# PTD504/handwritten-math-ocr-api

Hardware: NVIDIA B200
Metric: images_per_sec (higher is better)
Workload: dtype fp16

## Files before the change

handwritten_math_ocr_api_b200/_lib.py:

```python
from __future__ import annotations

import ctypes as C
import os

HERE = os.path.dirname(os.path.abspath(__file__))
LIB_PATH = os.path.join(HERE, "libhmocr.so")


class HmocrConfig(C.Structure):
    _fields_ = [(n, C.c_int32) for n in ("vocab_size", "d_model", "nhead", "dim_feedforward", "num_layers",
                                         "max_seq_len", "sos_id", "eos_id", "pad_id", "encoder_arch",
                                         "enc_num_layers")]


_p, _i, _i64p, _fp = C.c_void_p, C.c_int, C.POINTER(C.c_int64), C.c_void_p

SIGNATURES = {
    "hmocr_last_error": (C.c_char_p, []),
    "hmocr_version": (C.c_char_p, []),
    "hmocr_launch_count": (C.c_int64, []),
    "hmocr_create": (_i, [C.POINTER(HmocrConfig), C.POINTER(_p)]),
    "hmocr_destroy": (None, [_p]),
    "hmocr_load_weight": (_i, [_p, C.c_char_p, _p, _i64p, _i, _i]),
    "hmocr_finalize_weights": (_i, [_p]),
    "hmocr_set_option": (_i, [_p, C.c_char_p, _i]),
    "hmocr_decode_max_clusters": (_i, [C.POINTER(C.c_int)]),
    "hmocr_set_pos_table": (_i, [_p, _p, _i, _i, _p]),
    "hmocr_workspace_bytes": (_i, [_p, _i, _i, _i, C.POINTER(C.c_size_t)]),
    "hmocr_set_workspace": (_i, [_p, _p, C.c_size_t, _p]),
    "hmocr_read_trace": (_i, [_p, _i64p, _i]),
    "hmocr_encode": (_i, [_p, _p, _i, _p, _p]),
    "hmocr_decoder_forward": (_i, [_p, _p, _p, _i, _i, _p, _p]),
    "hmocr_generate": (_i, [_p, _p, _i, _i, _i, _p, _p, _p, _p, _p]),
    "hmocr_generate_from_memory": (_i, [_p, _p, _i, _i, _i, _p, _p, _p, _p, _p]),
    "hmocr_generate_nbest": (_i, [_p, _p, _i, _i, _i, _i, _i, _p, _p, _p, _p, _p]),
    "hmocr_generate_host": (_i, [_p, _p, _i, _i, _i, _p, _p, _p, _p, _p]),
    "hmocr_preprocess_u8": (_i, [_p, _p, _i, _p, _p]),
    "hmocr_pack_tokens": (_i, [_p, _p, _i, _i, _p, _p, _p]),
    "hmocr_preprocess_image_u8": (_i, [_p, _p, _i, _i, _i, _p, _p]),
    "hmocr_preprocess_cv2_u8": (_i, [_p, _p, _i, _i, _p, _p]),
    "hmocr_generate_host_u8": (_i, [_p, _p, _i, _i, _i, _p, _p, _p, _p, _p]),
    "hmocr_last_decode_steps": (_i, [_p, C.POINTER(C.c_int32)]),
    "hmocr_last_timings": (_i, [_p, C.POINTER(C.c_float), C.POINTER(C.c_float)]),
    "hmocr_gemm_f16": (_i, [_p, _i, _i, _i, _p, _i, _p, _i, _p, _i, _p, _i, _p, _i, _p, _p, _i, _p]),
    "hmocr_swin_mlp": (_i, [_p, _i, _i, _p, _p, _p, _p, _p, _p]),
    "hmocr_layernorm": (_i, [_p, _i, _i, _p, _p, _p, _p, _p]),
    "hmocr_patch_embed": (_i, [_p, _i, _p, _p, _p, _p, _p, _p]),
    "hmocr_patch_merge_ln": (_i, [_p, _i, _i, _i, _i, _p, _p, _p, _p]),
    "hmocr_window_attention": (_i, [_p, _p, _p, _i, _i, _i, _i, _i, _i, _p, _p]),
    "hmocr_self_attention": (_i, [_p, _i, _i, _i, _i, _p, _p]),
}

_lib = None


def load() -> C.CDLL:
    global _lib
    if _lib is None:
        if not os.path.exists(LIB_PATH):
            raise RuntimeError(
                f"{LIB_PATH} is missing: build it with `python -m handwritten_math_ocr_api_b200.build` "
                "(there is no CPU or PyTorch fallback)")
        lib = C.CDLL(LIB_PATH)
        for name, (res, args) in SIGNATURES.items():
            fn = getattr(lib, name)
            fn.restype, fn.argtypes = res, args
        _lib = lib
    return _lib


def check(rc: int, what: str) -> None:
    if rc != 0:
        msg = load().hmocr_last_error()
        raise RuntimeError(f"{what} failed ({rc}): {msg.decode() if msg else 'unknown error'}")
```

handwritten_math_ocr_api_b200/csrc/engine.cu:

```cuda
#include <stdarg.h>
#include <string.h>

#include <map>
#include <string>
#include <vector>

#include "decode_persistent.cuh"
#include "gemm.cuh"
#include "hmocr.h"
#include "kernels.cuh"

#include <nvtx3/nvToolsExt.h>

#define HM_API extern "C" __attribute__((visibility("default")))

namespace hmocr {

thread_local long g_launch_count = 0;
static thread_local char g_err[1024] = "";

void set_error(const char* fmt, ...) {
  va_list ap;
  va_start(ap, fmt);
  vsnprintf(g_err, sizeof(g_err), fmt, ap);
  va_end(ap);
}

namespace {

inline void nvtx_push(const char* name) { nvtxRangePushA(name); }
inline void nvtx_pop() { nvtxRangePop(); }

constexpr int IMG_H = 96, IMG_W = 320, SWIN_OUT = 768;
constexpr int RES18_MEM = 10, SWIN_MEM = 30;
constexpr int RES18_C[4] = {64, 128, 256, 512};
constexpr int RES18_STRIDE[4] = {1, 2, 2, 2};
constexpr int DEPTHS[4] = {2, 2, 6, 2};
constexpr int HEADS[4] = {3, 6, 12, 24};
constexpr int STEP_CHUNK = 8;

struct HostTensor {
  std::vector<float> f;
  std::vector<int64_t> i;
  std::vector<int64_t> shape;
};

struct Lin {
  h16* w = nullptr;
  float* b = nullptr;
  int n = 0, k = 0;
};
struct Norm { float* g = nullptr; float* b = nullptr; };
struct SwinBlock { Norm n1, n2; Lin qkv, proj, fc1, fc2; float* rel_bias = nullptr; };
struct Merge { Norm norm; Lin red; };
struct DecLayer { Lin sa_in, sa_out, ca_q, ca_out, l1, l2; Norm n1, n2, n3; };
struct EncLayer { Lin in_proj, out_proj, l1, l2; Norm n1, n2; };
struct ResBlock { Lin conv1, conv2, down; bool has_down = false; };

struct Buf {
  void* p = nullptr;
  size_t cap = 0;
};

}
}

using namespace hmocr;

struct hmocr_engine {
  hmocr_config cfg;
  int device = 0;
  int vpad = 0;
  std::map<std::string, HostTensor> host;
  bool finalized = false;

  uint8_t* arena = nullptr;
  size_t arena_cap = 0, arena_used = 0;
  float *pe_w = nullptr, *pe_b = nullptr;
  Norm pe_norm;
  SwinBlock blocks[12];
  Merge merges[3];
  Lin proj;
  float *emb = nullptr, *pos = nullptr;
  std::vector<DecLayer> layers;
  int mem_len = SWIN_MEM;
  float *r18_w1 = nullptr, *r18_b1 = nullptr;
  ResBlock r18_blocks[8];
  Lin r18_proj;
  std::vector<EncLayer> enc_layers;
  float* pos_table = nullptr;
  bool pos_table_set = false;
  Lin ca_kv;
  Lin fc;
  uint8_t* dp_wstream = nullptr;
  float* dp_lnparams = nullptr;
  int dp_fc_tiles = 0, dp_chunks_per_step = 0;
  int decode_impl = 0;
  int steps_per_launch = 0;
  int trace_step = -1;
  int conv_impl = 0;
  int mlp_fused = 1;

  std::map<std::string, Buf> ws;
  uint64_t ws_epoch = 0;
  uint8_t* ext_ws = nullptr;
  size_t ext_cap = 0, ext_used = 0;
  cudaStream_t cur_stream = nullptr;
  bool planning = false;
  std::map<std::string, size_t> plan;
  std::map<std::string, size_t> planned;

  struct StepGraph { cudaGraphExec_t exec = nullptr; uint64_t epoch = 0; };
  std::map<long long, StepGraph> graphs;
  struct EncGraph { cudaGraphExec_t exec = nullptr; uint64_t epoch = 0; bool warm = false; long launches = 0; };
  std::map<int, EncGraph> enc_graphs;
  int encoder_graph = 1;
  cudaStream_t cap_stream = nullptr;
  cudaEvent_t ev[4] = {nullptr, nullptr, nullptr, nullptr};
  cudaEvent_t poll_ev[2] = {nullptr, nullptr};
  DecodeState* pinned_state = nullptr;
  int last_poll_slot = -1;
  float last_enc_ms = 0.f, last_dec_ms = 0.f;
  bool timings_pending = false;
};

namespace hmocr {
namespace {

constexpr size_t WS_ALIGN = 256;
inline size_t ws_round(size_t b) { return (b + WS_ALIGN - 1) / WS_ALIGN * WS_ALIGN; }
inline bool ws_pool_exempt(const char* name) { return name[0] == 'p' && name[1] == 'p' && name[2] == '.'; }

template <class T>
int ws_get(hmocr_engine* e, const char* name, size_t count, T** out) {
  const size_t bytes = ws_round(count * sizeof(T) + 1);
  if (e->planning) {
    size_t& need = e->plan[name];
    if (need < bytes) need = bytes;
    *out = reinterpret_cast<T*>(WS_ALIGN);
    return 0;
  }
  Buf& b = e->ws[name];
  if (b.cap < bytes) {
    if (e->ext_ws != nullptr && !ws_pool_exempt(name)) {
      const size_t off = ws_round(e->ext_used);
      auto pl = e->planned.find(name);
      const size_t bytes_now = bytes;
      const size_t bytes = (pl != e->planned.end() && pl->second > bytes_now) ? pl->second : bytes_now;
      HM_CHECK(off + bytes <= e->ext_cap,
               "caller-owned workspace too small for '%s' (%zu + %zu > %zu bytes): size it with hmocr_workspace_bytes for "
               "the largest (batch, max_len, beam) you call with", name, off, bytes, e->ext_cap);
      b.p = e->ext_ws + off;
      b.cap = bytes;
      e->ext_used = off + bytes;
    } else {
      if (b.p != nullptr) {
        HM_CUDA(cudaFreeAsync(b.p, e->cur_stream));
        b.p = nullptr;
        b.cap = 0;
      }
      const size_t want = ws_round(bytes + bytes / 8);
      HM_CUDA(cudaMallocAsync(&b.p, want, e->cur_stream));
      b.cap = want;
    }
    ++e->ws_epoch;
  }
  *out = reinterpret_cast<T*>(b.p);
  return 0;
}

int arena_alloc(hmocr_engine* e, size_t bytes, void** out) {
  const size_t off = (e->arena_used + 255) & ~size_t(255);
  HM_CHECK(off + bytes <= e->arena_cap, "weight arena overflow (%zu + %zu > %zu)", off, bytes, e->arena_cap);
  *out = e->arena + off;
  e->arena_used = off + bytes;
  return 0;
}

const HostTensor* find(hmocr_engine* e, const std::string& key) {
  auto it = e->host.find(key);
  return it == e->host.end() ? nullptr : &it->second;
}

int need(hmocr_engine* e, const std::string& key, std::vector<int64_t> shape, const HostTensor** out) {
  const HostTensor* t = find(e, key);
  HM_CHECK(t != nullptr, "missing state-dict entry '%s'", key.c_str());
  HM_CHECK(t->shape == shape, "state-dict entry '%s' has the wrong shape", key.c_str());
  HM_CHECK(!t->f.empty(), "state-dict entry '%s' must be float32", key.c_str());
  *out = t;
  return 0;
}

inline h16 host_to_h16(float v) { return __float2half(v > 65504.f ? 65504.f : (v < -65504.f ? -65504.f : v)); }

int upload_f32(hmocr_engine* e, const float* src, size_t n, float** out) {
  void* p;
  HM_TRY(arena_alloc(e, n * sizeof(float), &p));
  HM_CUDA(cudaMemcpy(p, src, n * sizeof(float), cudaMemcpyHostToDevice));
  *out = reinterpret_cast<float*>(p);
  return 0;
}

int upload_vec(hmocr_engine* e, const std::string& key, int64_t n, float** out) {
  const HostTensor* t;
  HM_TRY(need(e, key, {n}, &t));
  return upload_f32(e, t->f.data(), (size_t)n, out);
}

int upload_norm(hmocr_engine* e, const std::string& prefix, int64_t n, Norm* out) {
  HM_TRY(upload_vec(e, prefix + ".weight", n, &out->g));
  return upload_vec(e, prefix + ".bias", n, &out->b);
}

int upload_lin_rows(hmocr_engine* e, const float* w, const float* b, int rows, int k, Lin* out) {
  const int npad = (rows + 31) / 32 * 32;
  std::vector<h16> tmp((size_t)npad * k, host_to_h16(0.f));
  for (size_t i = 0; i < (size_t)rows * k; ++i) tmp[i] = host_to_h16(w[i]);
  void* p;
  HM_TRY(arena_alloc(e, tmp.size() * 2, &p));
  HM_CUDA(cudaMemcpy(p, tmp.data(), tmp.size() * 2, cudaMemcpyHostToDevice));
  out->w = reinterpret_cast<h16*>(p);
  out->n = npad;
  out->k = k;
  out->b = nullptr;
  if (b != nullptr) {
    std::vector<float> bt(npad, 0.f);
    memcpy(bt.data(), b, sizeof(float) * rows);
    HM_TRY(upload_f32(e, bt.data(), npad, &out->b));
  }
  return 0;
}

int upload_lin(hmocr_engine* e, const std::string& prefix, int n, int k, bool bias, Lin* out) {
  const HostTensor *w, *b = nullptr;
  HM_TRY(need(e, prefix + ".weight", {n, k}, &w));
  if (bias) HM_TRY(need(e, prefix + ".bias", {n}, &b));
  return upload_lin_rows(e, w->f.data(), b ? b->f.data() : nullptr, n, k, out);
}

int fold_bn(hmocr_engine* e, const std::string& bn, int cout, std::vector<float>* scale, std::vector<float>* shift) {
  const HostTensor *g, *b, *m, *v;
  HM_TRY(need(e, bn + ".weight", {cout}, &g));
  HM_TRY(need(e, bn + ".bias", {cout}, &b));
  HM_TRY(need(e, bn + ".running_mean", {cout}, &m));
  HM_TRY(need(e, bn + ".running_var", {cout}, &v));
  scale->resize(cout); shift->resize(cout);
  for (int i = 0; i < cout; ++i) {
    const float sc = g->f[i] / sqrtf(v->f[i] + 1e-5f);
    (*scale)[i] = sc;
    (*shift)[i] = b->f[i] - m->f[i] * sc;
  }
  return 0;
}

int upload_conv(hmocr_engine* e, const std::string& conv, const std::string& bn, int cout, int cin, int k, Lin* out) {
  const HostTensor* w;
  HM_TRY(need(e, conv + ".weight", {cout, cin, k, k}, &w));
  std::vector<float> scale, shift;
  HM_TRY(fold_bn(e, bn, cout, &scale, &shift));
  std::vector<float> m((size_t)cout * k * k * cin);
  for (int o = 0; o < cout; ++o)
    for (int ci = 0; ci < cin; ++ci)
      for (int ky = 0; ky < k; ++ky)
        for (int kx = 0; kx < k; ++kx)
          m[(size_t)o * k * k * cin + (size_t)(ky * k + kx) * cin + ci] =
              w->f[(((size_t)o * cin + ci) * k + ky) * k + kx] * scale[o];
  return upload_lin_rows(e, m.data(), shift.data(), cout, k * k * cin, out);
}

int load_res18_weights(hmocr_engine* e) {
  const hmocr_config& c = e->cfg;
  const int d = c.d_model, ff = c.dim_feedforward;
  const std::string f = "encoder.features.";
  {
    const HostTensor* w;
    HM_TRY(need(e, f + "0.weight", {64, 1, 7, 7}, &w));
    std::vector<float> scale, shift;
    HM_TRY(fold_bn(e, f + "1", 64, &scale, &shift));
    std::vector<float> w1(64 * 49);
    for (int o = 0; o < 64; ++o)
      for (int i = 0; i < 49; ++i) w1[o * 49 + i] = w->f[o * 49 + i] * scale[o];
    HM_TRY(upload_f32(e, w1.data(), w1.size(), &e->r18_w1));
    HM_TRY(upload_f32(e, shift.data(), shift.size(), &e->r18_b1));
  }
  int cin = 64;
  for (int sidx = 0; sidx < 4; ++sidx) {
    const int cout = RES18_C[sidx];
    for (int j = 0; j < 2; ++j) {
      const std::string p = f + std::to_string(4 + sidx) + "." + std::to_string(j) + ".";
      ResBlock& rb = e->r18_blocks[sidx * 2 + j];
      HM_TRY(upload_conv(e, p + "conv1", p + "bn1", cout, j == 0 ? cin : cout, 3, &rb.conv1));
      HM_TRY(upload_conv(e, p + "conv2", p + "bn2", cout, cout, 3, &rb.conv2));
      rb.has_down = find(e, p + "downsample.0.weight") != nullptr;
      if (rb.has_down) HM_TRY(upload_conv(e, p + "downsample.0", p + "downsample.1", cout, cin, 1, &rb.down));
    }
    cin = cout;
  }
  HM_TRY(upload_lin(e, "encoder.projection", d, 512, true, &e->r18_proj));
  const int enc_layers = c.enc_num_layers > 0 ? c.enc_num_layers : c.num_layers;
  HM_CHECK(find(e, "encoder.transformer_encoder.layers." + std::to_string(enc_layers) + ".linear1.weight") == nullptr,
           "checkpoint has more than %d TransformerEncoder layers: set hmocr_config.enc_num_layers "
           "(config.res18trans_num_encoder_layers)", enc_layers);
  e->enc_layers.resize(enc_layers);
  for (int l = 0; l < enc_layers; ++l) {
    const std::string p = "encoder.transformer_encoder.layers." + std::to_string(l) + ".";
    EncLayer& L = e->enc_layers[l];
    const HostTensor *w, *b;
    HM_TRY(need(e, p + "self_attn.in_proj_weight", {3 * d, d}, &w));
    HM_TRY(need(e, p + "self_attn.in_proj_bias", {3 * d}, &b));
    HM_TRY(upload_lin_rows(e, w->f.data(), b->f.data(), 3 * d, d, &L.in_proj));
    HM_TRY(upload_lin(e, p + "self_attn.out_proj", d, d, true, &L.out_proj));
    HM_TRY(upload_lin(e, p + "linear1", ff, d, true, &L.l1));
    HM_TRY(upload_lin(e, p + "linear2", d, ff, true, &L.l2));
    HM_TRY(upload_norm(e, p + "norm1", d, &L.n1));
    HM_TRY(upload_norm(e, p + "norm2", d, &L.n2));
  }
  void* pt;
  HM_TRY(arena_alloc(e, sizeof(float) * RES18_MEM * d, &pt));
  e->pos_table = static_cast<float*>(pt);
  return 0;
}

int run_lin(cudaStream_t st, const h16* a, int lda, int M, const Lin& l, GemmEpilogue epi) {
  epi.bias = l.b;
  return gemm_f16(st, a, lda, M, l.k, l.w, l.n, epi);
}

int encode_impl(hmocr_engine* e, const float* images, int B, float* enc32, h16* enc16, cudaStream_t st) {
  const size_t tok1 = (size_t)B * 24 * 80;
  float *xa, *xb;
  h16 *xn, *qkv, *ctx, *hid;
  HM_TRY(ws_get(e, "enc.xa", tok1 * 96, &xa));
  HM_TRY(ws_get(e, "enc.xb", tok1 * 96 / 2, &xb));
  HM_TRY(ws_get(e, "enc.xn", tok1 * 96, &xn));
  HM_TRY(ws_get(e, "enc.qkv", tok1 * 288, &qkv));
  HM_TRY(ws_get(e, "enc.ctx", tok1 * 96, &ctx));
  HM_TRY(ws_get(e, "enc.hid", tok1 * 384, &hid));
  if (e->planning) return 0;

  HM_TRY(patch_embed(st, images, B, e->pe_w, e->pe_b, e->pe_norm.g, e->pe_norm.b, xa));
  int H = 24, W = 80, C = 96, blk = 0;
  float* x = xa;
  float* other = xb;
  for (int s = 0; s < 4; ++s) {
    const int rows = B * H * W;
    for (int j = 0; j < DEPTHS[s]; ++j, ++blk) {
      const SwinBlock& sb = e->blocks[blk];
      HM_TRY(layernorm(st, x, rows, C, sb.n1.g, sb.n1.b, xn, nullptr));
      GemmEpilogue eq;
      eq.out_f16 = qkv; eq.ld16 = 3 * C;
      HM_TRY(run_lin(st, xn, C, rows, sb.qkv, eq));
      HM_TRY(window_attention(st, qkv, sb.qkv.b, sb.rel_bias, B, H, W, C, HEADS[s], (j & 1) ? 3 : 0, ctx));
      GemmEpilogue ep;
      ep.residual = x; ep.ldr = C; ep.out_f32 = x; ep.ld32 = C;
      HM_TRY(run_lin(st, ctx, C, rows, sb.proj, ep));
      HM_TRY(layernorm(st, x, rows, C, sb.n2.g, sb.n2.b, xn, nullptr));
      if (e->mlp_fused && swin_mlp_supported(C)) {
        HM_TRY(swin_mlp(st, xn, rows, C, sb.fc1.w, sb.fc1.b, sb.fc2.w, sb.fc2.b, x));
      } else {
        GemmEpilogue e1;
        e1.act = 1; e1.out_f16 = hid; e1.ld16 = 4 * C;
        HM_TRY(run_lin(st, xn, C, rows, sb.fc1, e1));
        GemmEpilogue e2;
        e2.residual = x; e2.ldr = C; e2.out_f32 = x; e2.ld32 = C;
        HM_TRY(run_lin(st, hid, 4 * C, rows, sb.fc2, e2));
      }
    }
    if (s < 3) {
      const Merge& m = e->merges[s];
      HM_TRY(patch_merge_ln(st, x, B, H, W, C, m.norm.g, m.norm.b, xn));
      GemmEpilogue em;
      em.out_f32 = other; em.ld32 = 2 * C;
      HM_TRY(run_lin(st, xn, 4 * C, rows / 4, m.red, em));
      float* t = x; x = other; other = t;
      H /= 2; W /= 2; C *= 2;
    }
  }
  const int rows = B * e->mem_len;
  HM_TRY(f32_to_f16(st, x, (size_t)rows * SWIN_OUT, xn));
  GemmEpilogue eo;
  eo.out_f32 = enc32; eo.ld32 = e->cfg.d_model;
  eo.out_f16 = enc16; eo.ld16 = e->cfg.d_model;
  HM_TRY(run_lin(st, xn, SWIN_OUT, rows, e->proj, eo));
  return 0;
}

int conv_gemm(hmocr_engine* e, cudaStream_t st, const h16* x16, int B, int H, int W, int C, int k, int stride,
              const Lin& w, h16* col, GemmEpilogue epi) {
  const int pad = (k == 3) ? 1 : 0;
  const int Ho = (H + 2 * pad - k) / stride + 1, Wo = (W + 2 * pad - k) / stride + 1;
  int tw, th, tn;
  if (e->conv_impl == 0 && C % 64 == 0 && w.n % 64 == 0 && conv_tiling(Ho, Wo, &tw, &th, &tn)) {
    epi.bias = w.b;
    return gemm_conv_f16(st, x16, B, H, W, C, k, stride, pad, w.w, w.n, epi);
  }
  HM_TRY(im2col(st, x16, B, H, W, C, k, stride, pad, col));
  return run_lin(st, col, k * k * C, B * Ho * Wo, w, epi);
}

int encode_res18_impl(hmocr_engine* e, const float* images, int B, float* enc32, h16* enc16, cudaStream_t st) {
  const int d = e->cfg.d_model, ff = e->cfg.dim_feedforward, nh = e->cfg.nhead;
  HM_CHECK(e->planning || e->pos_table_set, "ResNet-18 variant: call hmocr_set_pos_table first - the reference draws a fresh "
                             "nn.Embedding(10, d_model) table on every encoder call (src/model_res18trans.py:57-59)");
  HM_CHECK(B <= 256, "ResNet-18 variant: the encoder attends ACROSS the batch (SURVEY.md D7); batch %d > 256 unsupported", B);
  const size_t m1 = (size_t)B * 24 * 80;
  h16 *stem, *xa16, *xb16, *h16b, *col;
  float *xa32, *xb32, *ds32;
  HM_TRY(ws_get(e, "r18.stem", (size_t)B * 48 * 160 * 64, &stem));
  HM_TRY(ws_get(e, "r18.xa16", m1 * 64, &xa16));
  HM_TRY(ws_get(e, "r18.xb16", m1 * 64, &xb16));
  HM_TRY(ws_get(e, "r18.h16", m1 * 64, &h16b));
  HM_TRY(ws_get(e, "r18.xa32", m1 * 64, &xa32));
  HM_TRY(ws_get(e, "r18.xb32", m1 * 64, &xb32));
  HM_TRY(ws_get(e, "r18.ds32", m1 * 64 / 2, &ds32));
  HM_TRY(ws_get(e, "r18.col", m1 * 576, &col));
  const int S = RES18_MEM, rows = B * S;
  h16 *pool16, *z16, *qkv, *ctx, *hid;
  float *q32, *z32;
  HM_TRY(ws_get(e, "r18.pool16", (size_t)rows * 512, &pool16));
  HM_TRY(ws_get(e, "r18.q32", (size_t)rows * d, &q32));
  HM_TRY(ws_get(e, "r18.z32", (size_t)rows * d, &z32));
  HM_TRY(ws_get(e, "r18.z16", (size_t)rows * d, &z16));
  HM_TRY(ws_get(e, "r18.qkv", (size_t)rows * 3 * d, &qkv));
  HM_TRY(ws_get(e, "r18.ctx", (size_t)rows * d, &ctx));
  HM_TRY(ws_get(e, "r18.hid", (size_t)rows * ff, &hid));
  if (e->planning) return 0;
  HM_TRY(conv7x7_bn_relu(st, images, B, e->r18_w1, e->r18_b1, stem));
  HM_TRY(maxpool3x3s2(st, stem, B, 48, 160, 64, xa16, xa32));
  int H = 24, W = 80, C = 64;
  h16 *x16 = xa16, *y16 = xb16;
  float *x32 = xa32, *y32 = xb32;
  for (int sidx = 0; sidx < 4; ++sidx) {
    for (int j = 0; j < 2; ++j) {
      const ResBlock& rb = e->r18_blocks[sidx * 2 + j];
      const int cout = RES18_C[sidx], stride = (j == 0) ? RES18_STRIDE[sidx] : 1;
      const int Ho = H / stride, Wo = W / stride, M = B * Ho * Wo;
      GemmEpilogue e1;
      e1.act = 2; e1.out_f16 = h16b; e1.ld16 = cout;
      HM_TRY(conv_gemm(e, st, x16, B, H, W, C, 3, stride, rb.conv1, col, e1));
      const float* identity = x32;
      if (rb.has_down) {
        GemmEpilogue ed;
        ed.out_f32 = ds32; ed.ld32 = cout;
        HM_TRY(conv_gemm(e, st, x16, B, H, W, C, 1, stride, rb.down, col, ed));
        identity = ds32;
      }
      GemmEpilogue e2;
      e2.act = 3; e2.residual = identity; e2.ldr = cout; e2.out_f32 = y32; e2.ld32 = cout; e2.out_f16 = y16; e2.ld16 = cout;
      HM_TRY(conv_gemm(e, st, h16b, B, Ho, Wo, cout, 3, 1, rb.conv2, col, e2));
      (void)M;
      h16* t16 = x16; x16 = y16; y16 = t16;
      float* t32 = x32; x32 = y32; y32 = t32;
      H = Ho; W = Wo; C = cout;
    }
  }
  HM_TRY(avgpool_h(st, x32, B, H, W, C, pool16));
  GemmEpilogue ep;
  ep.out_f32 = q32; ep.ld32 = d;
  HM_TRY(run_lin(st, pool16, 512, rows, e->r18_proj, ep));
  HM_TRY(add_pos_permute(st, q32, e->pos_table, B, S, d, z32, z16));
  for (size_t l = 0; l < e->enc_layers.size(); ++l) {
    const EncLayer& L = e->enc_layers[l];
    GemmEpilogue ei;
    ei.out_f16 = qkv; ei.ld16 = 3 * d;
    HM_TRY(run_lin(st, z16, d, rows, L.in_proj, ei));
    HM_TRY(mha_prefill_self(st, qkv, S, B, nh, ctx, false));
    GemmEpilogue e1;
    e1.residual = z32; e1.ldr = d; e1.out_f32 = z32; e1.ld32 = d; e1.out_f16 = z16; e1.ld16 = d;
    e1.ln_gamma = L.n1.g; e1.ln_beta = L.n1.b;
    HM_TRY(run_lin(st, ctx, d, rows, L.out_proj, e1));
    GemmEpilogue ef;
    ef.act = 2; ef.out_f16 = hid; ef.ld16 = ff;
    HM_TRY(run_lin(st, z16, d, rows, L.l1, ef));
    GemmEpilogue e2;
    e2.residual = z32; e2.ldr = d; e2.out_f32 = z32; e2.ld32 = d; e2.out_f16 = z16; e2.ld16 = d;
    e2.ln_gamma = L.n2.g; e2.ln_beta = L.n2.b;
    HM_TRY(run_lin(st, hid, ff, rows, L.l2, e2));
  }
  return permute_back(st, z32, B, S, d, enc32, enc16);
}

int project_memory(hmocr_engine* e, const h16* enc16, int B, h16* memkv, cudaStream_t st) {
  GemmEpilogue ek;
  ek.out_f16 = memkv; ek.ld16 = e->ca_kv.n;
  return run_lin(st, enc16, e->cfg.d_model, B * e->mem_len, e->ca_kv, ek);
}

struct DecBufs {
  float* x32;
  h16 *x16, *qkv, *q, *ctx, *hid;
  float* logits;
};

int dec_bufs(hmocr_engine* e, const char* tag, size_t rows, DecBufs* b) {
  const int d = e->cfg.d_model, ff = e->cfg.dim_feedforward;
  std::string t(tag);
  HM_TRY(ws_get(e, (t + ".x32").c_str(), rows * d, &b->x32));
  HM_TRY(ws_get(e, (t + ".x16").c_str(), rows * d, &b->x16));
  HM_TRY(ws_get(e, (t + ".qkv").c_str(), rows * 3 * d, &b->qkv));
  HM_TRY(ws_get(e, (t + ".q").c_str(), rows * d, &b->q));
  HM_TRY(ws_get(e, (t + ".ctx").c_str(), rows * d, &b->ctx));
  HM_TRY(ws_get(e, (t + ".hid").c_str(), rows * ff, &b->hid));
  HM_TRY(ws_get(e, (t + ".logits").c_str(), rows * e->vpad, &b->logits));
  return 0;
}

int layer_tail(hmocr_engine* e, const DecLayer& L, int l, const DecBufs& b, int rows, const h16* memkv,
               const int* mem_row, int T, cudaStream_t st) {
  const int d = e->cfg.d_model, ff = e->cfg.dim_feedforward, nh = e->cfg.nhead;
  GemmEpilogue e1;
  e1.residual = b.x32; e1.ldr = d; e1.out_f32 = b.x32; e1.ld32 = d; e1.out_f16 = b.x16; e1.ld16 = d;
  e1.ln_gamma = L.n1.g; e1.ln_beta = L.n1.b;
  HM_TRY(run_lin(st, b.ctx, d, rows, L.sa_out, e1));
  GemmEpilogue eq;
  eq.out_f16 = b.q; eq.ld16 = d;
  HM_TRY(run_lin(st, b.x16, d, rows, L.ca_q, eq));
  if (T > 0)
    HM_TRY(mha_prefill_cross(st, b.q, memkv, e->ca_kv.n, l * 2 * d, l * 2 * d + d, rows / T, T, e->mem_len, nh, b.ctx));
  else
    HM_TRY(cross_attn_step(st, b.q, memkv, e->ca_kv.n, l * 2 * d, l * 2 * d + d, mem_row, rows, e->mem_len, nh, b.ctx));
  GemmEpilogue e2;
  e2.residual = b.x32; e2.ldr = d; e2.out_f32 = b.x32; e2.ld32 = d; e2.out_f16 = b.x16; e2.ld16 = d;
  e2.ln_gamma = L.n2.g; e2.ln_beta = L.n2.b;
  HM_TRY(run_lin(st, b.ctx, d, rows, L.ca_out, e2));
  GemmEpilogue ef;
  ef.act = 2; ef.out_f16 = b.hid; ef.ld16 = ff;
  HM_TRY(run_lin(st, b.x16, d, rows, L.l1, ef));
  GemmEpilogue e3;
  e3.residual = b.x32; e3.ldr = d; e3.out_f32 = b.x32; e3.ld32 = d; e3.out_f16 = b.x16; e3.ld16 = d;
  e3.ln_gamma = L.n3.g; e3.ln_beta = L.n3.b;
  HM_TRY(run_lin(st, b.hid, ff, rows, L.l2, e3));
  return 0;
}

int decoder_forward_impl(hmocr_engine* e, const float* enc32, const int64_t* tgt, int B, int T, float* logits,
                         cudaStream_t st) {
  const int d = e->cfg.d_model, nh = e->cfg.nhead;
  const int rows = B * T;
  h16 *enc16, *memkv;
  HM_TRY(ws_get(e, "tf.enc16", (size_t)B * e->mem_len * d, &enc16));
  HM_TRY(ws_get(e, "tf.memkv", (size_t)B * e->mem_len * e->ca_kv.n, &memkv));
  DecBufs b;
  HM_TRY(dec_bufs(e, "tf", rows, &b));
  if (e->planning) return 0;
  HM_TRY(f32_to_f16(st, enc32, (size_t)B * e->mem_len * d, enc16));
  HM_TRY(project_memory(e, enc16, B, memkv, st));
  HM_TRY(embed_tokens(st, tgt, T, B, T, e->emb, e->pos, d, e->cfg.vocab_size, b.x32, b.x16));
  for (int l = 0; l < e->cfg.num_layers; ++l) {
    const DecLayer& L = e->layers[l];
    GemmEpilogue ei;
    ei.out_f16 = b.qkv; ei.ld16 = 3 * d;
    HM_TRY(run_lin(st, b.x16, d, rows, L.sa_in, ei));
    HM_TRY(mha_prefill_self(st, b.qkv, B, T, nh, b.ctx));
    HM_TRY(layer_tail(e, L, l, b, rows, memkv, nullptr, T, st));
  }
  GemmEpilogue eo;
  eo.out_f32 = b.logits; eo.ld32 = e->vpad;
  HM_TRY(run_lin(st, b.x16, d, rows, e->fc, eo));
  HM_TRY(copy_logits(st, b.logits, e->vpad, rows, e->cfg.vocab_size, logits));
  return 0;
}

struct GenBufs {
  DecBufs b;
  h16 *kcache, *vcache;
  DecodeState* state;
  uint8_t* finished;
  int tmax;
};

int enqueue_step(hmocr_engine* e, const GenBufs& g, int rows, const h16* memkv, int64_t* tokens,
                 float* logprob, int max_len, cudaStream_t st) {
  const int d = e->cfg.d_model, nh = e->cfg.nhead;
  const size_t layer_stride = (size_t)rows * nh * g.tmax * 32;
  for (int l = 0; l < e->cfg.num_layers; ++l) {
    const DecLayer& L = e->layers[l];
    GemmEpilogue ei;
    ei.out_f16 = g.b.qkv; ei.ld16 = 3 * d;
    HM_TRY(run_lin(st, g.b.x16, d, rows, L.sa_in, ei));
    HM_TRY(self_attn_step(st, g.state, g.b.qkv, g.kcache + l * layer_stride, g.vcache + l * layer_stride, rows, nh,
                          g.tmax, g.b.ctx));
    HM_TRY(layer_tail(e, L, l, g.b, rows, memkv, nullptr, 0, st));
  }
  GemmEpilogue eo;
  eo.out_f32 = g.b.logits; eo.ld32 = e->vpad;
  HM_TRY(run_lin(st, g.b.x16, d, rows, e->fc, eo));
  HM_TRY(greedy_select(st, g.state, g.b.logits, e->vpad, e->cfg.vocab_size, rows, tokens, max_len + 1, logprob,
                       max_len, e->cfg.eos_id, g.finished, e->emb, e->pos, d, e->cfg.max_seq_len, g.b.x32, g.b.x16));
  HM_TRY(advance_step(st, g.state));
  return 0;
}

int generate_persistent(hmocr_engine* e, const h16* enc16, int B, int max_len, int beam, int64_t* tokens,
                        float* logprob, int32_t* steps, float* score, cudaStream_t st, int n_best);

int generate_from_memory_impl(hmocr_engine* e, const h16* enc16, int B, int max_len, int beam,
                              int64_t* tokens, float* logprob, int32_t* steps, float* score, cudaStream_t st,
                              int n_best = 0) {
  HM_CHECK(max_len >= 1 && max_len <= e->cfg.max_seq_len,
           "max_len=%d outside [1, %d] (size of pos_encoder, src/model_swin.py:54)", max_len, e->cfg.max_seq_len);
  HM_CHECK(beam >= 1 && beam <= DP_MAX_BEAM, "beam=%d outside [1, %d]", beam, DP_MAX_BEAM);
  HM_CHECK(beam <= e->cfg.vocab_size, "beam=%d exceeds vocab_size=%d", beam, e->cfg.vocab_size);
  if (e->decode_impl == 0 || n_best > 0)
    return generate_persistent(e, enc16, B, max_len, beam, tokens, logprob, steps, score, st, n_best);
  HM_CHECK(beam == 1, "the step-graph decode (decode_impl=1) is greedy only; beam=%d needs decode_impl=0", beam);
  const int d = e->cfg.d_model, nh = e->cfg.nhead, L = e->cfg.num_layers;
  const int rows = B;
  h16* memkv;
  HM_TRY(ws_get(e, "gen.memkv", (size_t)B * e->mem_len * e->ca_kv.n, &memkv));
  GenBufs g;
  g.tmax = e->cfg.max_seq_len;
  HM_TRY(dec_bufs(e, "gen", rows, &g.b));
  const size_t cache_elems = (size_t)L * rows * nh * g.tmax * 32;
  HM_TRY(ws_get(e, "gen.kcache", cache_elems, &g.kcache));
  HM_TRY(ws_get(e, "gen.vcache", cache_elems, &g.vcache));
  HM_TRY(ws_get(e, "gen.state", 1, &g.state));
  HM_TRY(ws_get(e, "gen.finished", rows, &g.finished));
  int64_t* tok_ws;
  float* lp_ws;
  HM_TRY(ws_get(e, "gen.tokens", (size_t)rows * (g.tmax + 1), &tok_ws));
  HM_TRY(ws_get(e, "gen.logprob", (size_t)rows * g.tmax, &lp_ws));
  if (e->planning) return 0;

  HM_TRY(project_memory(e, enc16, B, memkv, st));
  HM_TRY(init_decode(st, g.state, tok_ws, max_len + 1, rows, e->cfg.sos_id, e->cfg.pad_id, g.finished, lp_ws, max_len));
  HM_TRY(embed_tokens(st, tok_ws, max_len + 1, rows, 1, e->emb, e->pos, d, e->cfg.vocab_size, g.b.x32, g.b.x16));

  const long long key = (long long)rows * 1024 + max_len;
  hmocr_engine::StepGraph& sg = e->graphs[key];
  if (sg.exec == nullptr || sg.epoch != e->ws_epoch) {
    if (sg.exec != nullptr) { cudaGraphExecDestroy(sg.exec); sg.exec = nullptr; }
    cudaGraph_t graph = nullptr;
    HM_CUDA(cudaStreamBeginCapture(e->cap_stream, cudaStreamCaptureModeThreadLocal));
    const long launches_before = g_launch_count;
    int rc = enqueue_step(e, g, rows, memkv, tok_ws, lp_ws, max_len, e->cap_stream);
    g_launch_count = launches_before;
    cudaError_t ce = cudaStreamEndCapture(e->cap_stream, &graph);
    if (rc != 0) { if (graph) cudaGraphDestroy(graph); return rc; }
    HM_CUDA(ce);
    ce = cudaGraphInstantiate(&sg.exec, graph, 0);
    cudaGraphDestroy(graph);
    HM_CUDA(ce);
    sg.epoch = e->ws_epoch;
  }
  size_t nodes_per_step = 8 * (size_t)L + 3;
  int launched_steps = 0, poll_idx = 0;
  bool done = false;
  for (int s0 = 0; s0 < max_len && !done; s0 += STEP_CHUNK, ++poll_idx) {
    const int n = (max_len - s0 < STEP_CHUNK) ? (max_len - s0) : STEP_CHUNK;
    for (int i = 0; i < n; ++i) {
      HM_CUDA(cudaGraphLaunch(sg.exec, st));
      g_launch_count += (long)nodes_per_step;
    }
    launched_steps += n;
    const int slot = poll_idx & 1;
    HM_CUDA(cudaMemcpyAsync(&e->pinned_state[slot], g.state, sizeof(DecodeState), cudaMemcpyDeviceToHost, st));
    HM_CUDA(cudaEventRecord(e->poll_ev[slot], st));
    if (poll_idx >= 1) {
      const int prev = (poll_idx - 1) & 1;
      HM_CUDA(cudaEventSynchronize(e->poll_ev[prev]));
      if (e->pinned_state[prev].steps_executed > 0) done = true;
    }
  }
  (void)launched_steps;
  HM_TRY(finalize_decode(st, g.state, tok_ws, max_len + 1, rows, max_len, e->cfg.pad_id, lp_ws, steps));
// ... 461 lines not shown
  }

  HM_TRY(need(e, "decoder.embedding.weight", {V, d}, &t));
  HM_TRY(upload_f32(e, t->f.data(), (size_t)V * d, &e->emb));
  HM_TRY(need(e, "decoder.pos_encoder.weight", {c.max_seq_len, d}, &t));
  HM_TRY(upload_f32(e, t->f.data(), (size_t)c.max_seq_len * d, &e->pos));
  std::vector<float> kvw((size_t)c.num_layers * 2 * d * d), kvb((size_t)c.num_layers * 2 * d);
  for (int l = 0; l < c.num_layers; ++l) {
    const std::string p = "decoder.decoder.layers." + std::to_string(l) + ".";
    DecLayer& L = e->layers[l];
    const HostTensor *w, *b;
    HM_TRY(need(e, p + "self_attn.in_proj_weight", {3 * d, d}, &w));
    HM_TRY(need(e, p + "self_attn.in_proj_bias", {3 * d}, &b));
    HM_TRY(upload_lin_rows(e, w->f.data(), b->f.data(), 3 * d, d, &L.sa_in));
    HM_TRY(upload_lin(e, p + "self_attn.out_proj", d, d, true, &L.sa_out));
    HM_TRY(need(e, p + "multihead_attn.in_proj_weight", {3 * d, d}, &w));
    HM_TRY(need(e, p + "multihead_attn.in_proj_bias", {3 * d}, &b));
    HM_TRY(upload_lin_rows(e, w->f.data(), b->f.data(), d, d, &L.ca_q));
    memcpy(&kvw[(size_t)l * 2 * d * d], w->f.data() + (size_t)d * d, sizeof(float) * 2 * d * d);
    memcpy(&kvb[(size_t)l * 2 * d], b->f.data() + d, sizeof(float) * 2 * d);
    HM_TRY(upload_lin(e, p + "multihead_attn.out_proj", d, d, true, &L.ca_out));
    HM_TRY(upload_lin(e, p + "linear1", ff, d, true, &L.l1));
    HM_TRY(upload_lin(e, p + "linear2", d, ff, true, &L.l2));
    HM_TRY(upload_norm(e, p + "norm1", d, &L.n1));
    HM_TRY(upload_norm(e, p + "norm2", d, &L.n2));
    HM_TRY(upload_norm(e, p + "norm3", d, &L.n3));
  }
  HM_TRY(upload_lin_rows(e, kvw.data(), kvb.data(), c.num_layers * 2 * d, d, &e->ca_kv));
  {
    const HostTensor *w, *b;
    HM_TRY(need(e, "decoder.fc_out.weight", {V, d}, &w));
    HM_TRY(need(e, "decoder.fc_out.bias", {V}, &b));
    std::vector<float> wp((size_t)e->vpad * d, 0.f), bp(e->vpad, 0.f);
    memcpy(wp.data(), w->f.data(), sizeof(float) * (size_t)V * d);
    memcpy(bp.data(), b->f.data(), sizeof(float) * V);
    HM_TRY(upload_lin_rows(e, wp.data(), bp.data(), e->vpad, d, &e->fc));
  }
  HM_TRY(pack_decode_operands(e));
  HM_TRY(decode_persistent_init());
  e->host.clear();
  e->finalized = true;
  return 0;
}

HM_API int hmocr_set_pos_table(hmocr_engine* e, const float* pos_host, int rows, int d, void* stream) {
  HM_CHECK(e != nullptr && pos_host != nullptr, "hmocr_set_pos_table: null argument");
  HM_CHECK(e->finalized && e->cfg.encoder_arch == 1, "hmocr_set_pos_table: only for a loaded ResNet-18 variant engine");
  HM_CHECK(rows == RES18_MEM && d == e->cfg.d_model, "positional table must be [%d, %d]", RES18_MEM, e->cfg.d_model);
  HM_CUDA(cudaSetDevice(e->device));
  HM_CUDA(cudaMemcpyAsync(e->pos_table, pos_host, sizeof(float) * rows * d, cudaMemcpyHostToDevice,
                          static_cast<cudaStream_t>(stream)));
  e->pos_table_set = true;
  return 0;
}

HM_API int hmocr_workspace_bytes(hmocr_engine* e, int batch, int max_len, int beam, size_t* bytes) {
  HM_CHECK(e != nullptr && bytes != nullptr, "hmocr_workspace_bytes: null argument");
  HM_CHECK(e->finalized, "hmocr_workspace_bytes: load the weights first (buffer sizes depend on the checkpoint's vocabulary)");
  HM_CHECK(batch >= 1 && max_len >= 1 && beam >= -DP_MAX_BEAM, "hmocr_workspace_bytes: bad shape batch=%d max_len=%d beam=%d", batch, max_len, beam);
  return plan_workspace(e, batch, max_len, beam, bytes);
}

HM_API int hmocr_set_workspace(hmocr_engine* e, void* workspace_dev, size_t bytes, void* stream) {
  HM_CHECK(e != nullptr, "hmocr_set_workspace: null engine");
  HM_CHECK(workspace_dev == nullptr || (reinterpret_cast<uintptr_t>(workspace_dev) % WS_ALIGN == 0 && bytes >= WS_ALIGN),
           "hmocr_set_workspace: the buffer must be %zu-byte aligned and non-empty", WS_ALIGN);
  HM_CUDA(cudaSetDevice(e->device));
  cudaStream_t st = static_cast<cudaStream_t>(stream);
  for (auto& kv : e->ws) {
    uint8_t* p = static_cast<uint8_t*>(kv.second.p);
    const bool in_pool = e->ext_ws != nullptr && p >= e->ext_ws && p < e->ext_ws + e->ext_cap;
    if (p != nullptr && !in_pool) HM_CUDA(cudaFreeAsync(p, st));
  }
  e->ws.clear();
  e->ext_ws = static_cast<uint8_t*>(workspace_dev);
  e->ext_cap = workspace_dev ? bytes : 0;
  e->ext_used = 0;
  ++e->ws_epoch;
  return 0;
}

HM_API int hmocr_decode_max_clusters(int* out) {
  HM_CHECK(out != nullptr, "null argument");
  return decode_persistent_max_clusters(out);
}

HM_API int hmocr_set_option(hmocr_engine* e, const char* name, int value) {
  HM_CHECK(e != nullptr && name != nullptr, "hmocr_set_option: null argument");
  const std::string n(name);
  if (n == "decode_impl") {
    HM_CHECK(value == 0 || value == 1, "decode_impl must be 0 (persistent cluster kernel) or 1 (step graph)");
    e->decode_impl = value;
  } else if (n == "steps_per_launch") {
    HM_CHECK(value >= 0 && value <= 256, "steps_per_launch must be in [0,256] (0 = automatic)");
    e->steps_per_launch = value;
  } else if (n == "trace_step") {
    e->trace_step = value;
  } else if (n == "encoder_graph") {
    HM_CHECK(value == 0 || value == 1, "encoder_graph must be 0 or 1");
    e->encoder_graph = value;
  } else if (n == "conv_impl") {
    HM_CHECK(value == 0 || value == 1, "conv_impl must be 0 (implicit GEMM) or 1 (im2col)");
    e->conv_impl = value;
  } else if (n == "gemm_dbg") {
    gemm_set_debug(value);
  } else if (n == "mlp_fused") {
    HM_CHECK(value == 0 || value == 1, "mlp_fused must be 0 (fc1 and fc2 as two GEMM launches) or 1 (one kernel)");
    if (e->mlp_fused != value) ++e->ws_epoch;
    e->mlp_fused = value;
  } else {
    HM_CHECK(false, "unknown option '%s'", name);
  }
  return 0;
}

HM_API int hmocr_read_trace(hmocr_engine* e, int64_t* out_host, int n) {
  HM_CHECK(e != nullptr && out_host != nullptr && n >= 1 && n <= 1024, "hmocr_read_trace: bad argument");
  auto it = e->ws.find("gen.trace");
  HM_CHECK(it != e->ws.end() && it->second.p != nullptr, "no trace recorded (set option trace_step first)");
  HM_CUDA(cudaMemcpy(out_host, it->second.p, sizeof(int64_t) * n, cudaMemcpyDeviceToHost));
  return 0;
}

HM_API int hmocr_encode(hmocr_engine* e, const float* images, int B, float* enc_out, void* stream) {
  HM_TRY(check_ready(e, B, stream));
  HM_CHECK(images != nullptr && enc_out != nullptr, "hmocr_encode: null buffer");
  h16* enc16;
  HM_TRY(ws_get(e, "enc.out16", (size_t)B * e->mem_len * e->cfg.d_model, &enc16));
  return e->cfg.encoder_arch == 1 ? encode_res18_impl(e, images, B, enc_out, enc16, static_cast<cudaStream_t>(stream))
                                  : encode_impl(e, images, B, enc_out, enc16, static_cast<cudaStream_t>(stream));
}

HM_API int hmocr_decoder_forward(hmocr_engine* e, const float* enc_out, const int64_t* tgt, int B, int T,
                                 float* logits, void* stream) {
  HM_TRY(check_ready(e, B, stream));
  HM_CHECK(enc_out != nullptr && tgt != nullptr && logits != nullptr, "hmocr_decoder_forward: null buffer");
  HM_CHECK(T >= 1 && T <= e->cfg.max_seq_len, "T=%d outside [1,%d] (tgt_mask / pos_encoder size)", T,
           e->cfg.max_seq_len);
  return decoder_forward_impl(e, enc_out, tgt, B, T, logits, static_cast<cudaStream_t>(stream));
}

HM_API int hmocr_generate(hmocr_engine* e, const float* images, int B, int max_len, int beam, int64_t* tokens,
                          float* logprob, int32_t* steps, float* score, void* stream) {
  HM_TRY(check_ready(e, B, stream));
  HM_CHECK(images != nullptr && tokens != nullptr, "hmocr_generate: null buffer");
  return generate_impl(e, images, B, max_len, beam, tokens, logprob, steps, score, static_cast<cudaStream_t>(stream));
}

HM_API int hmocr_generate_from_memory(hmocr_engine* e, const float* enc_out, int B, int max_len, int beam,
                                      int64_t* tokens, float* logprob, int32_t* steps, float* score, void* stream) {
  HM_TRY(check_ready(e, B, stream));
  HM_CHECK(enc_out != nullptr && tokens != nullptr, "hmocr_generate_from_memory: null buffer");
  return generate_from_enc32(e, enc_out, B, max_len, beam, tokens, logprob, steps, score,
                             static_cast<cudaStream_t>(stream), 0);
}

HM_API int hmocr_generate_nbest(hmocr_engine* e, const float* input, int input_is_memory, int B, int max_len, int beam,
                                int n_best, int64_t* tokens, float* logprob, float* score, int32_t* steps, void* stream) {
  HM_TRY(check_ready(e, B, stream));
  HM_CHECK(beam >= 1 && beam <= DP_MAX_BEAM, "hmocr_generate_nbest: beam=%d outside [1, %d]", beam, DP_MAX_BEAM);
  HM_CHECK(n_best >= 1 && n_best <= beam, "hmocr_generate_nbest: n_best=%d outside [1, beam=%d]", n_best, beam);
  HM_CHECK(input != nullptr && tokens != nullptr, "hmocr_generate_nbest: null buffer");
  cudaStream_t st = static_cast<cudaStream_t>(stream);
  if (input_is_memory) return generate_from_enc32(e, input, B, max_len, beam, tokens, logprob, steps, score, st, n_best);
  return generate_impl(e, input, B, max_len, beam, tokens, logprob, steps, score, st, n_best);
}

HM_API int hmocr_generate_host(hmocr_engine* e, const float* images_host, int B, int max_len, int beam,
                               int64_t* tokens_host, float* logprob_host, int32_t* steps_host, float* score_host,
                               void* stream) {
  HM_TRY(check_ready(e, B, stream));
  HM_CHECK(images_host != nullptr && tokens_host != nullptr, "hmocr_generate_host: null buffer");
  cudaStream_t st = static_cast<cudaStream_t>(stream);
  float *img_d, *lp_d, *score_d;
  int64_t* tok_d;
  int32_t* steps_d;
  const size_t img_n = (size_t)B * IMG_H * IMG_W;
  HM_TRY(ws_get(e, "host.images", img_n, &img_d));
  HM_TRY(ws_get(e, "host.tokens", (size_t)B * (max_len + 1), &tok_d));
  HM_TRY(ws_get(e, "host.logprob", (size_t)B * max_len, &lp_d));
  HM_TRY(ws_get(e, "host.steps", 1, &steps_d));
  HM_TRY(ws_get(e, "host.score", B, &score_d));
  HM_CUDA(cudaMemcpyAsync(img_d, images_host, img_n * sizeof(float), cudaMemcpyHostToDevice, st));
  HM_TRY(generate_impl(e, img_d, B, max_len, beam, tok_d, logprob_host ? lp_d : nullptr, steps_d,
                       score_host ? score_d : nullptr, st));
  HM_CUDA(cudaMemcpyAsync(tokens_host, tok_d, sizeof(int64_t) * B * (max_len + 1), cudaMemcpyDeviceToHost, st));
  if (logprob_host) HM_CUDA(cudaMemcpyAsync(logprob_host, lp_d, sizeof(float) * B * max_len, cudaMemcpyDeviceToHost, st));
  if (steps_host) HM_CUDA(cudaMemcpyAsync(steps_host, steps_d, sizeof(int32_t), cudaMemcpyDeviceToHost, st));
  if (score_host) HM_CUDA(cudaMemcpyAsync(score_host, score_d, sizeof(float) * B, cudaMemcpyDeviceToHost, st));
  HM_CUDA(cudaStreamSynchronize(st));
  return 0;
}

HM_API int hmocr_preprocess_image_u8(hmocr_engine* e, const uint8_t* image_host, int channels, int height, int width,
                                     float* image_dev, void* stream) {
  HM_CHECK(e != nullptr && image_host != nullptr && image_dev != nullptr, "hmocr_preprocess_image_u8: null argument");
  HM_CHECK(channels == 1 || channels == 3, "hmocr_preprocess_image_u8: channels must be 1 (mode L) or 3 (mode RGB), got %d", channels);
  HM_CHECK(height >= 1 && width >= 1 && height <= 16384 && width <= 16384, "hmocr_preprocess_image_u8: bad size %dx%d", height, width);
  HM_CUDA(cudaSetDevice(e->device));
  cudaStream_t st = static_cast<cudaStream_t>(stream);
  e->cur_stream = st;
  uint8_t *src, *mid;
  int* tables;
  const size_t bytes = (size_t)height * width * channels;
  HM_TRY(ws_get(e, "pp.src", bytes, &src));
  HM_TRY(ws_get(e, "pp.mid", (size_t)height * IMG_W, &mid));
  HM_TRY(ws_get(e, "pp.tables", preprocess_table_ints(height, width, IMG_H, IMG_W), &tables));
  HM_CUDA(cudaMemcpyAsync(src, image_host, bytes, cudaMemcpyHostToDevice, st));
  return preprocess_image(st, src, channels, height, width, IMG_H, IMG_W, tables, mid, image_dev);
}

HM_API int hmocr_preprocess_cv2_u8(hmocr_engine* e, const uint8_t* gray_host, int height, int width, float* image_dev,
                                   void* stream) {
  HM_CHECK(e != nullptr && gray_host != nullptr && image_dev != nullptr, "hmocr_preprocess_cv2_u8: null argument");
  HM_CHECK(height >= 1 && width >= 1 && height <= 16384 && width <= 16384, "hmocr_preprocess_cv2_u8: bad size %dx%d", height, width);
  HM_CUDA(cudaSetDevice(e->device));
  cudaStream_t st = static_cast<cudaStream_t>(stream);
  e->cur_stream = st;
  uint8_t* src;
  int* tables;
  const size_t bytes = (size_t)height * width;
  HM_TRY(ws_get(e, "pp.src", bytes, &src));
  HM_TRY(ws_get(e, "pp.tables", (size_t)4 * (IMG_H + IMG_W) + preprocess_table_ints(height, width, IMG_H, IMG_W), &tables));
  HM_CUDA(cudaMemcpyAsync(src, gray_host, bytes, cudaMemcpyHostToDevice, st));
  return preprocess_gray_cv2(st, src, height, width, IMG_H, IMG_W, tables, image_dev);
}

HM_API int hmocr_pack_tokens(hmocr_engine* e, const int64_t* tokens_dev, int rows, int ld_tok, int32_t* lengths_dev,
                             int32_t* packed_dev, void* stream) {
  HM_CHECK(e != nullptr && tokens_dev != nullptr && lengths_dev != nullptr && packed_dev != nullptr, "hmocr_pack_tokens: null argument");
  HM_CHECK(rows >= 1 && ld_tok >= 1, "hmocr_pack_tokens: bad shape rows=%d ld=%d", rows, ld_tok);
  HM_CUDA(cudaSetDevice(e->device));
  return pack_tokens(static_cast<cudaStream_t>(stream), tokens_dev, rows, ld_tok, e->cfg.sos_id, e->cfg.eos_id, e->cfg.pad_id,
                     lengths_dev, packed_dev);
}

HM_API int hmocr_preprocess_u8(hmocr_engine* e, const uint8_t* images_u8_dev, int B, float* images_dev, void* stream) {
  HM_CHECK(e != nullptr && images_u8_dev != nullptr && images_dev != nullptr && B >= 1, "hmocr_preprocess_u8: bad argument");
  HM_CUDA(cudaSetDevice(e->device));
  return preprocess_u8(static_cast<cudaStream_t>(stream), images_u8_dev, (size_t)B * IMG_H * IMG_W, images_dev);
}

HM_API int hmocr_generate_host_u8(hmocr_engine* e, const uint8_t* images_u8_host, int B, int max_len, int beam,
                                  int64_t* tokens_host, float* logprob_host, int32_t* steps_host, float* score_host,
                                  void* stream) {
  HM_TRY(check_ready(e, B, stream));
  HM_CHECK(images_u8_host != nullptr && tokens_host != nullptr, "hmocr_generate_host_u8: null buffer");
  cudaStream_t st = static_cast<cudaStream_t>(stream);
  uint8_t* u8_d;
  float *img_d, *lp_d, *score_d;
  int64_t* tok_d;
  int32_t* steps_d;
  const size_t img_n = (size_t)B * IMG_H * IMG_W;
  HM_TRY(ws_get(e, "host.images_u8", img_n, &u8_d));
  HM_TRY(ws_get(e, "host.images", img_n, &img_d));
  HM_TRY(ws_get(e, "host.tokens", (size_t)B * (max_len + 1), &tok_d));
  HM_TRY(ws_get(e, "host.logprob", (size_t)B * max_len, &lp_d));
  HM_TRY(ws_get(e, "host.steps", 1, &steps_d));
  HM_TRY(ws_get(e, "host.score", B, &score_d));
  HM_CUDA(cudaMemcpyAsync(u8_d, images_u8_host, img_n, cudaMemcpyHostToDevice, st));
  HM_TRY(preprocess_u8(st, u8_d, img_n, img_d));
  HM_TRY(generate_impl(e, img_d, B, max_len, beam, tok_d, logprob_host ? lp_d : nullptr, steps_d,
                       score_host ? score_d : nullptr, st));
  HM_CUDA(cudaMemcpyAsync(tokens_host, tok_d, sizeof(int64_t) * B * (max_len + 1), cudaMemcpyDeviceToHost, st));
  if (logprob_host) HM_CUDA(cudaMemcpyAsync(logprob_host, lp_d, sizeof(float) * B * max_len, cudaMemcpyDeviceToHost, st));
  if (steps_host) HM_CUDA(cudaMemcpyAsync(steps_host, steps_d, sizeof(int32_t), cudaMemcpyDeviceToHost, st));
  if (score_host) HM_CUDA(cudaMemcpyAsync(score_host, score_d, sizeof(float) * B, cudaMemcpyDeviceToHost, st));
  HM_CUDA(cudaStreamSynchronize(st));
  return 0;
}

HM_API int hmocr_last_decode_steps(hmocr_engine* e, int32_t* steps_run) {
  HM_CHECK(e != nullptr && steps_run != nullptr, "hmocr_last_decode_steps: null argument");
  HM_CHECK(e->last_poll_slot >= 0 && e->pinned_state != nullptr, "no persistent-kernel decode has run on this engine");
  *steps_run = e->pinned_state[e->last_poll_slot].step;
  return 0;
}

HM_API int hmocr_last_timings(hmocr_engine* e, float* encoder_ms, float* decode_ms) {
  HM_CHECK(e != nullptr, "null engine");
  if (e->timings_pending) {
    HM_CUDA(cudaEventSynchronize(e->ev[2]));
    HM_CUDA(cudaEventElapsedTime(&e->last_enc_ms, e->ev[0], e->ev[1]));
    HM_CUDA(cudaEventElapsedTime(&e->last_dec_ms, e->ev[1], e->ev[2]));
    e->timings_pending = false;
  }
  if (encoder_ms) *encoder_ms = e->last_enc_ms;
  if (decode_ms) *decode_ms = e->last_dec_ms;
  return 0;
}

HM_API int hmocr_gemm_f16(const void* a, int lda, int M, int K, const void* w, int N, const float* bias, int act,
                           const float* residual, int ldr, float* out_f32, int ld32, void* out_f16, int ld16,
                           const float* ln_gamma, const float* ln_beta, int force_bn, void* stream) {
  GemmEpilogue epi;
  epi.bias = bias; epi.act = act; epi.residual = residual; epi.ldr = ldr;
  epi.out_f32 = out_f32; epi.ld32 = ld32;
  epi.out_f16 = static_cast<h16*>(out_f16); epi.ld16 = ld16;
  epi.ln_gamma = ln_gamma; epi.ln_beta = ln_beta;
  return gemm_f16(static_cast<cudaStream_t>(stream), static_cast<const h16*>(a), lda, M, K,
                   static_cast<const h16*>(w), N, epi, force_bn);
}

HM_API int hmocr_swin_mlp(const void* xn, int M, int C, const void* w1, const float* b1, const void* w2, const float* b2,
                          float* x, void* stream) {
  HM_CHECK(xn != nullptr && w1 != nullptr && w2 != nullptr && x != nullptr, "null buffer");
  return swin_mlp(static_cast<cudaStream_t>(stream), static_cast<const h16*>(xn), M, C, static_cast<const h16*>(w1), b1,
                  static_cast<const h16*>(w2), b2, x);
}

HM_API int hmocr_layernorm(const float* x, int rows, int C, const float* gamma, const float* beta, void* out_f16,
                           float* out_f32, void* stream) {
  return layernorm(static_cast<cudaStream_t>(stream), x, rows, C, gamma, beta, static_cast<h16*>(out_f16),
                   out_f32);
}

HM_API int hmocr_patch_embed(const float* images, int B, const float* w, const float* b, const float* g,
                             const float* beta, float* x, void* stream) {
  return patch_embed(static_cast<cudaStream_t>(stream), images, B, w, b, g, beta, x);
}

HM_API int hmocr_patch_merge_ln(const float* x, int B, int H, int W, int C, const float* gamma, const float* beta,
                                void* out_f16, void* stream) {
  return patch_merge_ln(static_cast<cudaStream_t>(stream), x, B, H, W, C, gamma, beta,
                        static_cast<h16*>(out_f16));
}

HM_API int hmocr_self_attention(const void* qkv, int B, int T, int nhead, int causal, void* ctx, void* stream) {
  HM_CHECK(qkv != nullptr && ctx != nullptr, "null buffer");
  HM_CHECK(B >= 1 && T >= 1 && nhead >= 1, "bad shape B=%d T=%d nhead=%d", B, T, nhead);
  return mha_prefill_self(static_cast<cudaStream_t>(stream), static_cast<const h16*>(qkv), B, T, nhead,
                          static_cast<h16*>(ctx), causal != 0);
}

HM_API int hmocr_window_attention(const void* qkv, const float* qkv_bias, const float* rel_bias, int B, int H, int W,
                                  int C, int heads, int shift, void* ctx, void* stream) {
  return window_attention(static_cast<cudaStream_t>(stream), static_cast<const h16*>(qkv), qkv_bias,
                          rel_bias, B, H, W, C, heads, shift, static_cast<h16*>(ctx));
}
```

handwritten_math_ocr_api_b200/csrc/gemm.cu:

```cuda
#include "gemm.cuh"

#include <map>
#include <mutex>
#include <tuple>

namespace hmocr {
namespace {

constexpr int BM = 128;
constexpr int BK = 64;
constexpr int EPI_WARPS = 16;
constexpr int GROUP_WARPS = 8;
constexpr int NUM_THREADS = 32 * (2 + EPI_WARPS);
constexpr int EPI_WARP_BYTES = 4096 + 128;

template <int BN>
struct Cfg {
  static constexpr int A_BYTES = BM * BK * 2;
  static constexpr int B_BYTES = BN * BK * 2;
  static constexpr int STAGE_BYTES = A_BYTES + B_BYTES;
  static constexpr int EPI_STAGE_BYTES = EPI_WARPS * EPI_WARP_BYTES;
  static constexpr int STAGES_RAW = (156 * 1024) / STAGE_BYTES;
  static constexpr int STAGES = STAGES_RAW > 8 ? 8 : STAGES_RAW;
  static constexpr int TMEM_COLS = (2 * BN <= 128) ? 128 : ((2 * BN <= 256) ? 256 : 512);
  static constexpr int BAR_BYTES = 256;
  static constexpr int SMEM_BYTES = STAGES * STAGE_BYTES + 1024 + BAR_BYTES + EPI_STAGE_BYTES;
};

enum EpiMode { EPI_GENERAL = 0, EPI_F16 = 1, EPI_LN = 2 };

struct ConvGeom {
  int tw, th, tn, tiles_w, tiles_h, Ho, Wo, B, stride, pad, ksize, cin_blocks, rows_valid;
};
__device__ __forceinline__ int conv_pixel(const ConvGeom& g, int mi, int r) {
  if (r >= g.rows_valid) return -1;
  const int tile_w = mi % g.tiles_w, t2 = mi / g.tiles_w, tile_h = t2 % g.tiles_h, tile_n = t2 / g.tiles_h;
  const int w = r % g.tw, r2 = r / g.tw, h = r2 % g.th, n = tile_n * g.tn + r2 / g.th;
  if (n >= g.B) return -1;
  return (n * g.Ho + tile_h * g.th + h) * g.Wo + tile_w * g.tw + w;
}

struct GemmParams {
  int M, N, K;
  int num_n_tiles, num_tiles;
  int mode;
  ConvGeom cg;
  int dbg;
  GemmEpilogue epi;
};
int g_gemm_dbg = 0;

__device__ __forceinline__ uint64_t make_smem_desc(uint32_t saddr) {
  uint64_t d = 0;
  d |= static_cast<uint64_t>((saddr & 0x3FFFF) >> 4);
  d |= static_cast<uint64_t>(1) << 16;
  d |= static_cast<uint64_t>(1024 >> 4) << 32;
  d |= static_cast<uint64_t>(1) << 46;
  d |= static_cast<uint64_t>(2) << 61;
  return d;
}

template <int BN>
__device__ __forceinline__ constexpr uint32_t make_idesc() {
  return (1u << 4)
         | (0u << 7)
         | (0u << 10)
         | (uint32_t(BN >> 3) << 17)
         | (uint32_t(BM >> 4) << 24);
}

__device__ __forceinline__ void release_accumulator(bool last_chunk, uint32_t release_bar) {
  tc_fence_before();
  __syncwarp();
  if (last_chunk && (threadIdx.x & 31) == 0) mbar_arrive_cluster(release_bar);
}

template <int BN, int ACT, bool CONV>
__device__ __forceinline__ void epilogue_f16(const GemmEpilogue& e, uint32_t taddr, uint32_t st_addr, int m_base,
                                             int M, int n0, int c_first, int dbg, uint32_t release_bar,
                                             const ConvGeom& cg, int mi, int rq) {
  const int lane = threadIdx.x & 31;
  const uint32_t bias_addr = st_addr + 4096;
  const int srow = lane >> 2, sq = lane & 3;
  const uint32_t wr_addr = st_addr + lane * 64, wr_sw = (lane >> 1) & 3;
  const uint32_t rd_addr = st_addr + srow * 64 + ((sq ^ ((srow >> 1) & 3)) << 4);
  h16* out = e.out_f16 + (size_t)(m_base + srow) * e.ld16 + n0 + sq * 8;
  const size_t out_step = (size_t)8 * e.ld16;
  const int rows_left = (dbg & 1) ? 0 : M - m_base - srow;
  int pix[4];
  if (CONV) {
#pragma unroll
    for (int it = 0; it < 4; ++it) pix[it] = (dbg & 1) ? -1 : conv_pixel(cg, mi, rq + it * 8 + srow);
  }
#pragma unroll 1
  for (int c = c_first; c < BN / 32; c += 2) {
    const float b = e.bias != nullptr ? __ldg(e.bias + n0 + c * 32 + lane) : 0.0f;
    __syncwarp();
    asm volatile("st.shared.f32 [%0], %1;" ::"r"(bias_addr + lane * 4), "f"(b) : "memory");
    uint32_t r[32];
    tmem_ld32(taddr + c * 32, r);
    release_accumulator(c + 2 >= BN / 32, release_bar);
    if ((dbg & 4) && r[0] != 0x12345678u) continue;
    uint32_t h[16];
#pragma unroll
    for (int q = 0; q < 8; ++q) {
      uint64_t b01, b23;
      asm volatile("ld.shared.v2.b64 {%0, %1}, [%2];" : "=l"(b01), "=l"(b23) : "r"(bias_addr + q * 16));
      float v0, v1, v2, v3;
      upk2(add2(pk2(__uint_as_float(r[4 * q]), __uint_as_float(r[4 * q + 1])), b01), v0, v1);
      upk2(add2(pk2(__uint_as_float(r[4 * q + 2]), __uint_as_float(r[4 * q + 3])), b23), v2, v3);
      if (ACT == 1) { gelu_erf2(v0, v1); gelu_erf2(v2, v3); }
      if (ACT == 2) { v0 = fmaxf(v0, 0.f); v1 = fmaxf(v1, 0.f); v2 = fmaxf(v2, 0.f); v3 = fmaxf(v3, 0.f); }
      h[2 * q] = pack16(v0, v1);
      h[2 * q + 1] = pack16(v2, v3);
    }
#pragma unroll
    for (int q = 0; q < 4; ++q)
      asm volatile("st.shared.v4.b32 [%0], {%1, %2, %3, %4};" ::"r"(wr_addr + ((q ^ wr_sw) << 4)), "r"(h[4 * q]),
                   "r"(h[4 * q + 1]), "r"(h[4 * q + 2]), "r"(h[4 * q + 3])
                   : "memory");
    __syncwarp();
#pragma unroll
    for (int it = 0; it < 4; ++it) {
      uint4 v;
      asm volatile("ld.shared.v4.b32 {%0, %1, %2, %3}, [%4];"
                   : "=r"(v.x), "=r"(v.y), "=r"(v.z), "=r"(v.w)
                   : "r"(rd_addr + it * 512));
      if (CONV) {
        if (pix[it] >= 0) *reinterpret_cast<uint4*>(e.out_f16 + (size_t)pix[it] * e.ld16 + n0 + sq * 8 + c * 32) = v;
      } else {
        if (it * 8 < rows_left) *reinterpret_cast<uint4*>(out + it * out_step + c * 32) = v;
      }
    }
  }
}

template <int BN, bool RES, bool CONV>
__device__ __forceinline__ void epilogue_general(const GemmEpilogue& e, uint32_t taddr, uint32_t st_addr, int m_base,
                                                 int M, int n0, int c_first, int dbg, uint32_t release_bar,
                                                 const ConvGeom& cg, int mi, int rq) {
  const int lane = threadIdx.x & 31;
  const int rr = lane >> 3, cg4 = lane & 7;
  const float lo_pre = e.act == 2 ? 0.0f : -INFINITY, lo_post = e.act == 3 ? 0.0f : -INFINITY;
  const int rows_left = M - m_base - rr;
  const int rows_store = (dbg & 1) ? 0 : rows_left;
  const uint32_t wr_addr = st_addr + lane * 128, wr_sw = lane & 7;
  const uint32_t rd_addr = st_addr + rr * 128;
  int pix[8];
  if (CONV) {
#pragma unroll
    for (int it = 0; it < 8; ++it) pix[it] = conv_pixel(cg, mi, rq + it * 4 + rr);
  }
#pragma unroll 1
  for (int c = c_first; c < BN / 32; c += 2) {
    const int col = n0 + c * 32 + cg4 * 4;
    float4 res[8];
    if (RES) {
      const float* rp = e.residual + (size_t)(m_base + rr) * e.ldr + col;
#pragma unroll
      for (int it = 0; it < 8; ++it) {
        if (CONV)
          res[it] = pix[it] >= 0 ? __ldcs(reinterpret_cast<const float4*>(e.residual + (size_t)pix[it] * e.ldr + col))
                                 : make_float4(0.f, 0.f, 0.f, 0.f);
        else
          res[it] = (it * 4 < rows_left) ? __ldcs(reinterpret_cast<const float4*>(rp + (size_t)it * 4 * e.ldr))
                                         : make_float4(0.f, 0.f, 0.f, 0.f);
      }
    }
    float4 bias = make_float4(0.f, 0.f, 0.f, 0.f);
    if (e.bias != nullptr) bias = __ldg(reinterpret_cast<const float4*>(e.bias + col));
    uint32_t r[32];
    tmem_ld32(taddr + c * 32, r);
    release_accumulator(c + 2 >= BN / 32, release_bar);
    if ((dbg & 4) && r[0] != 0x12345678u) continue;
#pragma unroll
    for (int q = 0; q < 8; ++q)
      asm volatile("st.shared.v4.b32 [%0], {%1, %2, %3, %4};" ::"r"(wr_addr + ((q ^ wr_sw) << 4)), "r"(r[4 * q]),
                   "r"(r[4 * q + 1]), "r"(r[4 * q + 2]), "r"(r[4 * q + 3])
                   : "memory");
    __syncwarp();
    float* o32 = e.out_f32 != nullptr ? e.out_f32 + (size_t)(m_base + rr) * e.ld32 + col : nullptr;
    h16* o16 = e.out_f16 != nullptr ? e.out_f16 + (size_t)(m_base + rr) * e.ld16 + col : nullptr;
#pragma unroll
    for (int it = 0; it < 8; ++it) {
      float4 v;
      asm volatile("ld.shared.v4.f32 {%0, %1, %2, %3}, [%4];"
                   : "=f"(v.x), "=f"(v.y), "=f"(v.z), "=f"(v.w)
                   : "r"(rd_addr + it * 512 + ((cg4 ^ ((it * 4 + rr) & 7)) << 4)));
      v.x += bias.x; v.y += bias.y; v.z += bias.z; v.w += bias.w;
      if (e.act == 1) { v.x = gelu_erf(v.x); v.y = gelu_erf(v.y); v.z = gelu_erf(v.z); v.w = gelu_erf(v.w); }
      v.x = fmaxf(v.x, lo_pre); v.y = fmaxf(v.y, lo_pre); v.z = fmaxf(v.z, lo_pre); v.w = fmaxf(v.w, lo_pre);
      if (RES) { v.x += res[it].x; v.y += res[it].y; v.z += res[it].z; v.w += res[it].w; }
      v.x = fmaxf(v.x, lo_post); v.y = fmaxf(v.y, lo_post); v.z = fmaxf(v.z, lo_post); v.w = fmaxf(v.w, lo_post);
      if (CONV) {
        if (pix[it] >= 0 && !(dbg & 1)) {
          if (e.out_f32 != nullptr) *reinterpret_cast<float4*>(e.out_f32 + (size_t)pix[it] * e.ld32 + col) = v;
          if (e.out_f16 != nullptr)
            *reinterpret_cast<uint2*>(e.out_f16 + (size_t)pix[it] * e.ld16 + col) = make_uint2(pack16(v.x, v.y), pack16(v.z, v.w));
        }
      } else if (it * 4 < rows_store) {
        if (o32 != nullptr) *reinterpret_cast<float4*>(o32 + (size_t)it * 4 * e.ld32) = v;
        if (o16 != nullptr)
          *reinterpret_cast<uint2*>(o16 + (size_t)it * 4 * e.ld16) = make_uint2(pack16(v.x, v.y), pack16(v.z, v.w));
      }
    }
  }
}

template <int BN>
__device__ __forceinline__ void epilogue_ln(const GemmEpilogue& e, uint32_t taddr, int row, bool row_ok, int n0) {
  float sum = 0.0f;
#pragma unroll 1
  for (int c = 0; c < BN / 32; ++c) {
    uint32_t r[32];
    tmem_ld32(taddr + c * 32, r);
    const int col = n0 + c * 32;
    float v[32];
#pragma unroll
    for (int j = 0; j < 32; ++j) v[j] = __uint_as_float(r[j]);
    if (e.bias != nullptr) {
#pragma unroll
      for (int j = 0; j < 32; ++j) v[j] += __ldg(e.bias + col + j);
    }
    if (e.act == 1) {
#pragma unroll
      for (int j = 0; j < 32; ++j) v[j] = gelu_erf(v[j]);
    } else if (e.act == 2) {
#pragma unroll
      for (int j = 0; j < 32; ++j) v[j] = fmaxf(v[j], 0.0f);
    }
    if (row_ok && e.residual != nullptr) {
      const float4* r4 = reinterpret_cast<const float4*>(e.residual + (size_t)row * e.ldr + col);
#pragma unroll
      for (int q = 0; q < 8; ++q) {
        float4 x = r4[q];
        v[4 * q + 0] += x.x; v[4 * q + 1] += x.y; v[4 * q + 2] += x.z; v[4 * q + 3] += x.w;
      }
    }
#pragma unroll
    for (int j = 0; j < 32; ++j) { sum += v[j]; r[j] = __float_as_uint(v[j]); }
    tmem_st32(taddr + c * 32, r);
  }
  const float mean = sum * (1.0f / BN);
  float sq = 0.0f;
#pragma unroll 1
  for (int c = 0; c < BN / 32; ++c) {
    uint32_t r[32];
    tmem_ld32(taddr + c * 32, r);
#pragma unroll
    for (int j = 0; j < 32; ++j) { float d = __uint_as_float(r[j]) - mean; sq += d * d; }
  }
  const float rstd = rsqrtf(sq * (1.0f / BN) + 1e-5f);
#pragma unroll 1
  for (int c = 0; c < BN / 32; ++c) {
    uint32_t r[32];
    tmem_ld32(taddr + c * 32, r);
    const int col = n0 + c * 32;
    float v[32];
#pragma unroll
    for (int j = 0; j < 32; ++j)
      v[j] = (__uint_as_float(r[j]) - mean) * rstd * __ldg(e.ln_gamma + col + j) + __ldg(e.ln_beta + col + j);
    if (row_ok) {
      if (e.out_f32 != nullptr) {
        float4* o = reinterpret_cast<float4*>(e.out_f32 + (size_t)row * e.ld32 + col);
#pragma unroll
        for (int q = 0; q < 8; ++q) o[q] = make_float4(v[4 * q], v[4 * q + 1], v[4 * q + 2], v[4 * q + 3]);
      }
      if (e.out_f16 != nullptr) {
        uint4* o = reinterpret_cast<uint4*>(e.out_f16 + (size_t)row * e.ld16 + col);
#pragma unroll
        for (int q = 0; q < 4; ++q)
          o[q] = make_uint4(pack16(v[8 * q], v[8 * q + 1]), pack16(v[8 * q + 2], v[8 * q + 3]),
                            pack16(v[8 * q + 4], v[8 * q + 5]), pack16(v[8 * q + 6], v[8 * q + 7]));
      }
    }
  }
}

template <int BN, bool CONV>
__global__ void __launch_bounds__(NUM_THREADS, 1)
gemm_tcgen05_kernel(const __grid_constant__ CUtensorMap tmA, const __grid_constant__ CUtensorMap tmB,
                    const GemmParams p) {
  using C = Cfg<BN>;
  extern __shared__ uint8_t smem_raw[];
  const uint32_t raw_addr = smem_u32(smem_raw);
  uint8_t* smem = smem_raw + ((1024u - (raw_addr & 1023u)) & 1023u);

  uint64_t* full_bar = reinterpret_cast<uint64_t*>(smem + C::STAGES * C::STAGE_BYTES);
  uint64_t* empty_bar = full_bar + C::STAGES;
  uint64_t* tfull_bar = empty_bar + C::STAGES;
  uint64_t* tempty_bar = tfull_bar + 2;
  uint32_t* tmem_slot = reinterpret_cast<uint32_t*>(tempty_bar + 2);
  const uint32_t epi_stage = smem_u32(smem + C::STAGES * C::STAGE_BYTES + C::BAR_BYTES);

  const int warp = threadIdx.x >> 5;
  const int lane = threadIdx.x & 31;
  pdl_launch_dependents();

  if (warp == 0 && lane == 0) {
    tma_prefetch_desc(&tmA);
    tma_prefetch_desc(&tmB);
    for (int s = 0; s < C::STAGES; ++s) {
      mbar_init(&full_bar[s], 1);
      mbar_init(&empty_bar[s], 1);
    }
    for (int a = 0; a < 2; ++a) {
      mbar_init(&tfull_bar[a], 1);
      mbar_init(&tempty_bar[a], GROUP_WARPS);
    }
    fence_barrier_init();
  }
  if (warp == 1) tmem_alloc(tmem_slot, C::TMEM_COLS);
  tc_fence_before();
  __syncthreads();
  tc_fence_after();
  const uint32_t tmem_base = *tmem_slot;
  const int num_kb = (p.K + BK - 1) / BK;
  pdl_wait();

  if (warp == 0) {
    if (lane == 0) {
      int s = 0;
      uint32_t ph = 0;
      for (int t = blockIdx.x; t < p.num_tiles; t += gridDim.x) {
        const int m0 = (t / p.num_n_tiles) * BM;
        const int n0 = (t % p.num_n_tiles) * BN;
        int cw = 0, chh = 0, cn = 0;
        if (CONV) {
          const int mi = t / p.num_n_tiles;
          const int tile_w = mi % p.cg.tiles_w, t2 = mi / p.cg.tiles_w;
          cw = tile_w * p.cg.tw * p.cg.stride - p.cg.pad;
          chh = (t2 % p.cg.tiles_h) * p.cg.th * p.cg.stride - p.cg.pad;
          cn = (t2 / p.cg.tiles_h) * p.cg.tn;
        }
        for (int kb = 0; kb < num_kb; ++kb) {
          mbar_wait(&empty_bar[s], ph ^ 1u);
          uint8_t* st = smem + s * C::STAGE_BYTES;
          if (CONV) {
            mbar_expect_tx(&full_bar[s], p.cg.rows_valid * (BK * 2) + C::B_BYTES);
            const int tap = kb / p.cg.cin_blocks, cb = kb - tap * p.cg.cin_blocks;
            const int kh = tap / p.cg.ksize, kw = tap - kh * p.cg.ksize;
            tma_load_4d(st, &tmA, &full_bar[s], cb * BK, cw + kw, chh + kh, cn);
          } else {
            mbar_expect_tx(&full_bar[s], C::STAGE_BYTES);
            tma_load_2d(st, &tmA, &full_bar[s], kb * BK, m0);
          }
          tma_load_2d(st + C::A_BYTES, &tmB, &full_bar[s], kb * BK, n0);
          if (++s == C::STAGES) { s = 0; ph ^= 1u; }
        }
      }
    }
  } else if (warp == 1) {
    if (lane == 0) {
      constexpr uint32_t idesc = make_idesc<BN>();
      int s = 0;
      uint32_t ph = 0;
      int it = 0;
      for (int t = blockIdx.x; t < p.num_tiles; t += gridDim.x, ++it) {
        const int a = it & 1;
        const uint32_t aph = (it >> 1) & 1;
        mbar_wait_backoff(&tempty_bar[a], aph ^ 1u);
        tc_fence_after();
        const uint32_t d_tmem = tmem_base + a * BN;
        for (int kb = 0; kb < num_kb; ++kb) {
          mbar_wait(&full_bar[s], ph);
          tc_fence_after();
          const uint32_t abase = smem_u32(smem + s * C::STAGE_BYTES);
          const uint32_t bbase = abase + C::A_BYTES;
#pragma unroll
          for (int k = 0; k < BK / 16; ++k) {
            umma_f16(d_tmem, make_smem_desc(abase + k * 32), make_smem_desc(bbase + k * 32), idesc,
                      (kb | k) != 0 ? 1u : 0u);
          }
          umma_commit(&empty_bar[s]);
          if (++s == C::STAGES) { s = 0; ph ^= 1u; }
        }
        umma_commit(&tfull_bar[a]);
      }
    }
  } else {
    const int quarter = warp & 3;
    const int ew = warp - 2;
    const int group = ew >> 3;
    const int half = (ew >> 2) & 1;
    const uint32_t st_addr = epi_stage + ew * EPI_WARP_BYTES;
    const uint32_t taddr = tmem_base + (uint32_t(quarter * 32) << 16) + group * BN;
    const bool has_res = p.epi.residual != nullptr && !(p.dbg & 2);
    int it = group;
    for (int t = blockIdx.x + group * gridDim.x; t < p.num_tiles; t += 2 * gridDim.x, it += 2) {
      const uint32_t aph = (it >> 1) & 1;
      const int m0 = (t / p.num_n_tiles) * BM;
      const int n0 = (t % p.num_n_tiles) * BN;
      mbar_wait_backoff(&tfull_bar[group], aph);
      tc_fence_after();
      const int mb = m0 + quarter * 32;
      const int mi = t / p.num_n_tiles, rq = quarter * 32;
      if (p.mode == EPI_LN) {
        const int row = mb + lane;
        if (half == 0) epilogue_ln<BN>(p.epi, taddr, row, row < p.M, n0);
      } else if (p.mode == EPI_F16) {
        if (p.epi.act == 1) epilogue_f16<BN, 1, CONV>(p.epi, taddr, st_addr, mb, p.M, n0, half, p.dbg, smem_u32(&tempty_bar[group]), p.cg, mi, rq);
        else if (p.epi.act == 2) epilogue_f16<BN, 2, CONV>(p.epi, taddr, st_addr, mb, p.M, n0, half, p.dbg, smem_u32(&tempty_bar[group]), p.cg, mi, rq);
        else epilogue_f16<BN, 0, CONV>(p.epi, taddr, st_addr, mb, p.M, n0, half, p.dbg, smem_u32(&tempty_bar[group]), p.cg, mi, rq);
      } else {
        if (has_res) epilogue_general<BN, true, CONV>(p.epi, taddr, st_addr, mb, p.M, n0, half, p.dbg, smem_u32(&tempty_bar[group]), p.cg, mi, rq);
        else epilogue_general<BN, false, CONV>(p.epi, taddr, st_addr, mb, p.M, n0, half, p.dbg, smem_u32(&tempty_bar[group]), p.cg, mi, rq);
      }
      if (p.mode == EPI_LN) {
        tc_fence_before();
        __syncwarp();
        if (lane == 0) mbar_arrive(&tempty_bar[group]);
      }
    }
  }

  tc_fence_before();
  __syncthreads();
  if (warp == 1) {
    __syncwarp();
    tmem_dealloc(tmem_base, C::TMEM_COLS);
  }
}

template <int BN>
struct Cfg2 {
  static constexpr int A_BYTES = BM * BK * 2;
  static constexpr int B_BYTES = (BN / 2) * BK * 2;
  static constexpr int STAGE_BYTES = A_BYTES + B_BYTES;
  static constexpr int EPI_STAGE_BYTES = EPI_WARPS * EPI_WARP_BYTES;
  static constexpr int STAGES_RAW = (156 * 1024) / STAGE_BYTES;
  static constexpr int STAGES = STAGES_RAW > 8 ? 8 : STAGES_RAW;
  static constexpr int TMEM_COLS = (2 * BN <= 128) ? 128 : ((2 * BN <= 256) ? 256 : 512);
  static constexpr int BAR_BYTES = 256;
  static constexpr int SMEM_BYTES = STAGES * STAGE_BYTES + 1024 + BAR_BYTES + EPI_STAGE_BYTES;
};

template <int BN>
__global__ void __launch_bounds__(NUM_THREADS, 1)
gemm2_tcgen05_kernel(const __grid_constant__ CUtensorMap tmA, const __grid_constant__ CUtensorMap tmB,
                     const GemmParams p) {
  using C = Cfg2<BN>;
  extern __shared__ uint8_t smem_raw[];
  const uint32_t raw_addr = smem_u32(smem_raw);
  uint8_t* smem = smem_raw + ((1024u - (raw_addr & 1023u)) & 1023u);

  uint64_t* full_bar = reinterpret_cast<uint64_t*>(smem + C::STAGES * C::STAGE_BYTES);
  uint64_t* empty_bar = full_bar + C::STAGES;
  uint64_t* tfull_bar = empty_bar + C::STAGES;
  uint64_t* tempty_bar = tfull_bar + 2;
  uint32_t* tmem_slot = reinterpret_cast<uint32_t*>(tempty_bar + 2);
  const uint32_t epi_stage = smem_u32(smem + C::STAGES * C::STAGE_BYTES + C::BAR_BYTES);

  const int warp = threadIdx.x >> 5;
  const int lane = threadIdx.x & 31;
  const uint32_t rank = cta_rank_in_cluster();
  const int pair = blockIdx.x >> 1, npairs = gridDim.x >> 1;
  pdl_launch_dependents();

  if (warp == 0 && lane == 0) {
    tma_prefetch_desc(&tmA);
    tma_prefetch_desc(&tmB);
    for (int s = 0; s < C::STAGES; ++s) {
      mbar_init(&full_bar[s], 1);
      mbar_init(&empty_bar[s], 1);
    }
    for (int a = 0; a < 2; ++a) {
      mbar_init(&tfull_bar[a], 1);
      mbar_init(&tempty_bar[a], 2 * GROUP_WARPS);
    }
    fence_barrier_init();
  }
  cluster_barrier();
  if (warp == 1) tmem_alloc2(tmem_slot, C::TMEM_COLS);
  tc_fence_before();
  __syncthreads();
  cluster_barrier();
  tc_fence_after();
  const uint32_t tmem_base = *tmem_slot;
  const int num_kb = (p.K + BK - 1) / BK;
  pdl_wait();

  if (warp == 0) {
    if (lane == 0) {
      int s = 0;
      uint32_t ph = 0;
      for (int t = pair; t < p.num_tiles; t += npairs) {
        const int m0 = (t / p.num_n_tiles) * (2 * BM) + rank * BM;
        const int n0 = (t % p.num_n_tiles) * BN + rank * (BN / 2);
        for (int kb = 0; kb < num_kb; ++kb) {
          mbar_wait(&empty_bar[s], ph ^ 1u);
          if (rank == 0) mbar_expect_tx(&full_bar[s], 2 * C::STAGE_BYTES);
          uint8_t* st = smem + s * C::STAGE_BYTES;
          tma2_load_2d(st, &tmA, &full_bar[s], kb * BK, m0);
          tma2_load_2d(st + C::A_BYTES, &tmB, &full_bar[s], kb * BK, n0);
          if (++s == C::STAGES) { s = 0; ph ^= 1u; }
        }
      }
    }
  } else if (warp == 1) {
    if (lane == 0 && rank == 0) {
      constexpr uint32_t idesc = (1u << 4) | (uint32_t(BN >> 3) << 17) | (uint32_t((2 * BM) >> 4) << 24);
      int s = 0;
      uint32_t ph = 0;
      int it = 0;
      for (int t = pair; t < p.num_tiles; t += npairs, ++it) {
        const int a = it & 1;
        const uint32_t aph = (it >> 1) & 1;
        mbar_wait_backoff(&tempty_bar[a], aph ^ 1u);
        tc_fence_after();
        const uint32_t d_tmem = tmem_base + a * BN;
        for (int kb = 0; kb < num_kb; ++kb) {
          mbar_wait(&full_bar[s], ph);
          tc_fence_after();
          const uint32_t abase = smem_u32(smem + s * C::STAGE_BYTES);
          const uint32_t bbase = abase + C::A_BYTES;
#pragma unroll
          for (int k = 0; k < BK / 16; ++k) {
            umma2_f16(d_tmem, make_smem_desc(abase + k * 32), make_smem_desc(bbase + k * 32), idesc,
                      (kb | k) != 0 ? 1u : 0u);
          }
          umma2_commit(&empty_bar[s]);
          if (++s == C::STAGES) { s = 0; ph ^= 1u; }
        }
        umma2_commit(&tfull_bar[a]);
      }
    }
  } else {
    const int quarter = warp & 3;
    const int ew = warp - 2;
    const int group = ew >> 3;
    const int half = (ew >> 2) & 1;
    const uint32_t st_addr = epi_stage + ew * EPI_WARP_BYTES;
    const uint32_t taddr = tmem_base + (uint32_t(quarter * 32) << 16) + group * BN;
    const bool has_res = p.epi.residual != nullptr && !(p.dbg & 2);
    const uint32_t release = smem_u32(&tempty_bar[group]) & PEER_BIT_MASK;
    int it = group;
    for (int t = pair + group * npairs; t < p.num_tiles; t += 2 * npairs, it += 2) {
      const uint32_t aph = (it >> 1) & 1;
      const int m0 = (t / p.num_n_tiles) * (2 * BM) + rank * BM;
      const int n0 = (t % p.num_n_tiles) * BN;
      mbar_wait_backoff(&tfull_bar[group], aph);
      tc_fence_after();
      const int mb = m0 + quarter * 32;
      if (p.mode == EPI_F16) {
        if (p.epi.act == 1) epilogue_f16<BN, 1, false>(p.epi, taddr, st_addr, mb, p.M, n0, half, p.dbg, release, p.cg, 0, 0);
        else if (p.epi.act == 2) epilogue_f16<BN, 2, false>(p.epi, taddr, st_addr, mb, p.M, n0, half, p.dbg, release, p.cg, 0, 0);
        else epilogue_f16<BN, 0, false>(p.epi, taddr, st_addr, mb, p.M, n0, half, p.dbg, release, p.cg, 0, 0);
      } else {
        if (has_res) epilogue_general<BN, true, false>(p.epi, taddr, st_addr, mb, p.M, n0, half, p.dbg, release, p.cg, 0, 0);
        else epilogue_general<BN, false, false>(p.epi, taddr, st_addr, mb, p.M, n0, half, p.dbg, release, p.cg, 0, 0);
      }
    }
  }

  tc_fence_before();
  __syncthreads();
  cluster_barrier();
  if (warp == 1) {
    __syncwarp();
    tmem_dealloc2(tmem_base, C::TMEM_COLS);
  }
}

typedef CUresult (*EncodeTiledFn)(CUtensorMap*, CUtensorMapDataType, cuuint32_t, void*, const cuuint64_t*,
                                  const cuuint64_t*, const cuuint32_t*, const cuuint32_t*, CUtensorMapInterleave,
                                  CUtensorMapSwizzle, CUtensorMapL2promotion, CUtensorMapFloatOOBfill);
EncodeTiledFn g_encode = nullptr;
int g_sms[HM_MAX_DEVICES] = {};
int num_sms() {
  int dev = 0;
  cudaGetDevice(&dev);
  return (dev >= 0 && dev < HM_MAX_DEVICES && g_sms[dev] > 0) ? g_sms[dev] : 148;
}
std::mutex g_mu;
std::map<std::tuple<const void*, int, int, int, int>, CUtensorMap> g_maps;

int get_tensor_map(const void* ptr, int rows, int cols, int ld, int box_rows, CUtensorMap* out) {
  auto key = std::make_tuple(ptr, rows, cols, ld, box_rows);
  std::lock_guard<std::mutex> lk(g_mu);
  auto it = g_maps.find(key);
  if (it != g_maps.end()) {
    *out = it->second;
    return 0;
  }
  alignas(64) CUtensorMap m;
  cuuint64_t dims[2] = {(cuuint64_t)cols, (cuuint64_t)rows};
  cuuint64_t strides[1] = {(cuuint64_t)ld * 2};
  cuuint32_t box[2] = {(cuuint32_t)BK, (cuuint32_t)box_rows};
  cuuint32_t estr[2] = {1, 1};
  CUresult r = g_encode(&m, CU_TENSOR_MAP_DATA_TYPE_FLOAT16, 2, const_cast<void*>(ptr), dims, strides, box, estr,
                        CU_TENSOR_MAP_INTERLEAVE_NONE, CU_TENSOR_MAP_SWIZZLE_128B, CU_TENSOR_MAP_L2_PROMOTION_L2_256B,
                        CU_TENSOR_MAP_FLOAT_OOB_FILL_NONE);
  HM_CHECK(r == CUDA_SUCCESS, "cuTensorMapEncodeTiled failed (%d) ptr=%p rows=%d cols=%d ld=%d box_rows=%d", (int)r,
           ptr, rows, cols, ld, box_rows);
  if (g_maps.size() > 4096) g_maps.clear();
  g_maps[key] = m;
  *out = m;
  return 0;
}

template <int BN>
int launch(cudaStream_t stream, const h16* A, int lda, int M, int K, const h16* W, int N,
           const GemmEpilogue& epi) {
  using C = Cfg<BN>;
  alignas(64) CUtensorMap tmA, tmB;
  HM_TRY(get_tensor_map(A, M, K, lda, BM, &tmA));
  HM_TRY(get_tensor_map(W, N, K, K, BN, &tmB));
  GemmParams p;
  p.M = M; p.N = N; p.K = K;
  p.num_n_tiles = N / BN;
  p.num_tiles = ceil_div(M, BM) * p.num_n_tiles;
  p.epi = epi;
  p.dbg = g_gemm_dbg;
  p.mode = epi.ln_gamma != nullptr ? EPI_LN
           : (epi.out_f32 == nullptr && epi.residual == nullptr && epi.act != 3) ? EPI_F16 : EPI_GENERAL;
  const int grid = p.num_tiles < num_sms() ? p.num_tiles : num_sms();
  HM_CUDA(launch_pdl(gemm_tcgen05_kernel<BN, false>, dim3(grid), dim3(NUM_THREADS), C::SMEM_BYTES, stream, tmA, tmB, p));
  HM_LAUNCHED();
  return 0;
}

std::map<std::tuple<const void*, int, int, int, int, int, int, int, int>, CUtensorMap> g_maps4;
int get_tensor_map_nhwc(const void* ptr, int B, int H, int W, int C, int tw, int th, int tn, int stride, CUtensorMap* out) {
  auto key = std::make_tuple(ptr, B, H, W, C, tw, th, tn, stride);
  std::lock_guard<std::mutex> lk(g_mu);
  auto it = g_maps4.find(key);
  if (it != g_maps4.end()) {
    *out = it->second;
    return 0;
  }
  alignas(64) CUtensorMap m;
  cuuint64_t dims[4] = {(cuuint64_t)C, (cuuint64_t)W, (cuuint64_t)H, (cuuint64_t)B};
  cuuint64_t strides[3] = {(cuuint64_t)C * 2, (cuuint64_t)W * C * 2, (cuuint64_t)H * W * C * 2};
  cuuint32_t box[4] = {(cuuint32_t)BK, (cuuint32_t)(tw * stride), (cuuint32_t)(th * stride), (cuuint32_t)tn};
  cuuint32_t estr[4] = {1, (cuuint32_t)stride, (cuuint32_t)stride, 1};
  CUresult r = g_encode(&m, CU_TENSOR_MAP_DATA_TYPE_FLOAT16, 4, const_cast<void*>(ptr), dims, strides, box, estr,
                        CU_TENSOR_MAP_INTERLEAVE_NONE, CU_TENSOR_MAP_SWIZZLE_128B, CU_TENSOR_MAP_L2_PROMOTION_L2_256B,
                        CU_TENSOR_MAP_FLOAT_OOB_FILL_NONE);
  HM_CHECK(r == CUDA_SUCCESS, "cuTensorMapEncodeTiled (NHWC) failed (%d) B=%d H=%d W=%d C=%d box=%dx%dx%d stride=%d", (int)r,
           B, H, W, C, tw, th, tn, stride);
  if (g_maps4.size() > 1024) g_maps4.clear();
  g_maps4[key] = m;
  *out = m;
  return 0;
}

template <int BN>
int launch_conv(cudaStream_t stream, const CUtensorMap& tmA, const h16* Wt, int N, int K, const ConvGeom& cg, int m_tiles,
                const GemmEpilogue& epi) {
  using C = Cfg<BN>;
  alignas(64) CUtensorMap tmB;
  HM_TRY(get_tensor_map(Wt, N, K, K, BN, &tmB));
  GemmParams p;
  p.M = m_tiles * BM; p.N = N; p.K = K;
  p.num_n_tiles = N / BN;
  p.num_tiles = m_tiles * p.num_n_tiles;
  p.epi = epi;
  p.dbg = g_gemm_dbg;
  p.mode = (epi.out_f32 == nullptr && epi.residual == nullptr && epi.act != 3) ? EPI_F16 : EPI_GENERAL;
  p.cg = cg;
  const int grid = p.num_tiles < num_sms() ? p.num_tiles : num_sms();
  HM_CUDA(launch_pdl(gemm_tcgen05_kernel<BN, true>, dim3(grid), dim3(NUM_THREADS), C::SMEM_BYTES, stream, tmA, tmB, p));
  HM_LAUNCHED();
  return 0;
}

template <int BN>
int launch2(cudaStream_t stream, const h16* A, int lda, int M, int K, const h16* W, int N, const GemmEpilogue& epi) {
  using C = Cfg2<BN>;
  alignas(64) CUtensorMap tmA, tmB;
  HM_TRY(get_tensor_map(A, M, K, lda, BM, &tmA));
  HM_TRY(get_tensor_map(W, N, K, K, BN / 2, &tmB));
  GemmParams p;
  p.M = M; p.N = N; p.K = K;
  p.num_n_tiles = N / BN;
  p.num_tiles = ceil_div(M, 2 * BM) * p.num_n_tiles;
  p.epi = epi;
  p.dbg = g_gemm_dbg;
  p.mode = (epi.out_f32 == nullptr && epi.residual == nullptr && epi.act != 3) ? EPI_F16 : EPI_GENERAL;
  p.cg = ConvGeom{};
  int pairs = num_sms() / 2;
  if (p.num_tiles < pairs) pairs = p.num_tiles;
  cudaLaunchConfig_t cfg = {};
  cfg.gridDim = dim3(2 * pairs);
  cfg.blockDim = dim3(NUM_THREADS);
  cfg.dynamicSmemBytes = C::SMEM_BYTES;
  cfg.stream = stream;
  cudaLaunchAttribute attr[2];
  attr[0].id = cudaLaunchAttributeClusterDimension;
  attr[0].val.clusterDim.x = 2; attr[0].val.clusterDim.y = 1; attr[0].val.clusterDim.z = 1;
  attr[1].id = cudaLaunchAttributeProgrammaticStreamSerialization;
  attr[1].val.programmaticStreamSerializationAllowed = 1;
  cfg.attrs = attr;
  cfg.numAttrs = 2;
  HM_CUDA(cudaLaunchKernelEx(&cfg, gemm2_tcgen05_kernel<BN>, tmA, tmB, p));
  HM_LAUNCHED();
  return 0;
}

}

bool conv_tiling(int Ho, int Wo, int* tw, int* th, int* tn) {
  if (Ho * Wo <= BM) {
    *tw = Wo; *th = Ho; *tn = BM / (Ho * Wo);
    if (*tn > 256) *tn = 256;
    return (*tw) * (*th) * (*tn) * 4 >= BM * 3;
  }
  *tn = 1;
  int best_tw = 0, best_th = 0;
  for (int w = 1; w <= Wo && w <= BM; ++w) {
    if (Wo % w != 0) continue;
    for (int h = 1; h <= Ho && w * h <= BM; ++h) {
      if (Ho % h != 0) continue;
      if (w * h > best_tw * best_th) { best_tw = w; best_th = h; }
    }
  }
  *tw = best_tw; *th = best_th;
  return best_tw * best_th * 4 >= BM * 3 && best_tw <= 256 && best_th <= 256;
}

int gemm_conv_f16(cudaStream_t stream, const h16* x, int B, int H, int W, int Cin, int ksize, int stride, int pad,
                  const h16* Wt, int N, const GemmEpilogue& epi) {
  HM_TRY(gemm_init());
  const int Ho = (H + 2 * pad - ksize) / stride + 1, Wo = (W + 2 * pad - ksize) / stride + 1;
  ConvGeom cg;
  HM_CHECK(conv_tiling(Ho, Wo, &cg.tw, &cg.th, &cg.tn), "conv: no tile box for a %dx%d output", Ho, Wo);
  HM_CHECK(Cin % BK == 0, "conv: input channels %d must be a multiple of %d", Cin, BK);
  HM_CHECK(cg.tw * stride <= 256 && cg.th * stride <= 256, "conv: tile box too large for TMA");
  HM_CHECK(epi.ln_gamma == nullptr, "conv: fused LayerNorm is not supported");
  HM_CHECK(epi.out_f32 != nullptr || epi.out_f16 != nullptr, "conv: no output");
  cg.tiles_w = Wo / cg.tw; cg.tiles_h = Ho / cg.th;
  cg.Ho = Ho; cg.Wo = Wo; cg.B = B; cg.stride = stride; cg.pad = pad; cg.ksize = ksize;
  cg.cin_blocks = Cin / BK; cg.rows_valid = cg.tw * cg.th * cg.tn;
  const int m_tiles = cg.tiles_w * cg.tiles_h * ceil_div(B, cg.tn);
  const int K = ksize * ksize * Cin;
  alignas(64) CUtensorMap tmA;
  HM_TRY(get_tensor_map_nhwc(x, B, H, W, Cin, cg.tw, cg.th, cg.tn, stride, &tmA));
  int bn = 0;
  const int cands[3] = {256, 128, 64};
  for (int i = 0; i < 3; ++i) {
    if (N % cands[i] != 0) continue;
    bn = cands[i];
    if (m_tiles * (N / cands[i]) >= num_sms()) break;
  }
  HM_CHECK(bn != 0, "conv: output channels %d must be a multiple of 64", N);
  switch (bn) {
    case 64: return launch_conv<64>(stream, tmA, Wt, N, K, cg, m_tiles, epi);
    case 128: return launch_conv<128>(stream, tmA, Wt, N, K, cg, m_tiles, epi);
    default: return launch_conv<256>(stream, tmA, Wt, N, K, cg, m_tiles, epi);
  }
}

void gemm_set_debug(int v) { g_gemm_dbg = v; }
int gemm_tensor_map(const void* ptr, int rows, int cols, int ld, int box_rows, CUtensorMap* out) {
  return get_tensor_map(ptr, rows, cols, ld, box_rows, out);
}
int gemm_num_sms() { return num_sms(); }

int gemm_init() {
  std::lock_guard<std::mutex> lk(g_mu);
  int cur = 0;
  HM_CUDA(cudaGetDevice(&cur));
  HM_CHECK(cur >= 0 && cur < HM_MAX_DEVICES, "device index %d", cur);
  if (g_sms[cur] > 0) return 0;
  void* fn = nullptr;
  cudaDriverEntryPointQueryResult q;
  HM_CUDA(cudaGetDriverEntryPoint("cuTensorMapEncodeTiled", &fn, cudaEnableDefault, &q));
  HM_CHECK(fn != nullptr && q == cudaDriverEntryPointSuccess, "cuTensorMapEncodeTiled not available in this driver");
  const int dev = cur;
  cudaDeviceProp prop;
  HM_CUDA(cudaGetDeviceProperties(&prop, dev));
  HM_CHECK(prop.major == 10, "libhmocr is built for sm_100a only; device is sm_%d%d (no fallback path)", prop.major,
           prop.minor);
  HM_CUDA(cudaFuncSetAttribute(gemm_tcgen05_kernel<64, false>, cudaFuncAttributeMaxDynamicSharedMemorySize, Cfg<64>::SMEM_BYTES));
  HM_CUDA(cudaFuncSetAttribute(gemm_tcgen05_kernel<96, false>, cudaFuncAttributeMaxDynamicSharedMemorySize, Cfg<96>::SMEM_BYTES));
  HM_CUDA(cudaFuncSetAttribute(gemm_tcgen05_kernel<128, false>, cudaFuncAttributeMaxDynamicSharedMemorySize, Cfg<128>::SMEM_BYTES));
  HM_CUDA(cudaFuncSetAttribute(gemm_tcgen05_kernel<192, false>, cudaFuncAttributeMaxDynamicSharedMemorySize, Cfg<192>::SMEM_BYTES));
  HM_CUDA(cudaFuncSetAttribute(gemm_tcgen05_kernel<256, false>, cudaFuncAttributeMaxDynamicSharedMemorySize, Cfg<256>::SMEM_BYTES));
  HM_CUDA(cudaFuncSetAttribute(gemm2_tcgen05_kernel<192>, cudaFuncAttributeMaxDynamicSharedMemorySize, Cfg2<192>::SMEM_BYTES));
  HM_CUDA(cudaFuncSetAttribute(gemm2_tcgen05_kernel<256>, cudaFuncAttributeMaxDynamicSharedMemorySize, Cfg2<256>::SMEM_BYTES));
  HM_CUDA(cudaFuncSetAttribute(gemm_tcgen05_kernel<64, true>, cudaFuncAttributeMaxDynamicSharedMemorySize, Cfg<64>::SMEM_BYTES));
  HM_CUDA(cudaFuncSetAttribute(gemm_tcgen05_kernel<128, true>, cudaFuncAttributeMaxDynamicSharedMemorySize, Cfg<128>::SMEM_BYTES));
  HM_CUDA(cudaFuncSetAttribute(gemm_tcgen05_kernel<256, true>, cudaFuncAttributeMaxDynamicSharedMemorySize, Cfg<256>::SMEM_BYTES));
  g_encode = reinterpret_cast<EncodeTiledFn>(fn);
  g_sms[dev] = prop.multiProcessorCount;
  return 0;
}

int gemm_f16(cudaStream_t stream, const h16* A, int lda, int M, int K, const h16* W, int N,
              const GemmEpilogue& epi, int force_bn) {
  HM_TRY(gemm_init());
  HM_CHECK(M > 0 && N > 0 && K > 0, "gemm: empty problem M=%d N=%d K=%d", M, N, K);
  HM_CHECK(N % 32 == 0, "gemm: N=%d must be a multiple of 32 (pad the weight)", N);
  HM_CHECK(K % 8 == 0 && lda % 8 == 0, "gemm: K=%d and lda=%d must be multiples of 8", K, lda);
  HM_CHECK((reinterpret_cast<uintptr_t>(A) & 15) == 0 && (reinterpret_cast<uintptr_t>(W) & 15) == 0,
           "gemm: operands must be 16-byte aligned");
  HM_CHECK(epi.out_f32 != nullptr || epi.out_f16 != nullptr, "gemm: no output");
  HM_CHECK(epi.out_f32 == nullptr || epi.ld32 % 4 == 0, "gemm: ld32 must be a multiple of 4");
  HM_CHECK(epi.out_f16 == nullptr || epi.ld16 % 8 == 0, "gemm: ld16 must be a multiple of 8");
  HM_CHECK(epi.residual == nullptr || epi.ldr % 4 == 0, "gemm: ldr must be a multiple of 4");
  int bn = force_bn;
  if (epi.ln_gamma != nullptr) {
    HM_CHECK(N == 64 || N == 96 || N == 128 || N == 192 || N == 256,
             "gemm: fused LayerNorm needs N in {64,96,128,192,256}, got %d", N);
    HM_CHECK(epi.ln_beta != nullptr, "gemm: ln_beta missing");
    bn = N;
  }
  if (bn == 0) {
    const int cands[5] = {256, 192, 128, 96, 64};
    const int mt = ceil_div(M, BM);
    int smallest = 0;
    for (int i = 0; i < 5; ++i) {
      if (N % cands[i] != 0) continue;
      smallest = cands[i];
      if (bn == 0 && mt * (N / cands[i]) >= num_sms()) bn = cands[i];
    }
    if (bn == 0) bn = smallest;
    HM_CHECK(bn != 0, "gemm: N=%d is not a multiple of 64 or 96", N);
  }
  if (force_bn == 0 && epi.ln_gamma == nullptr && K >= 1024 && N % 192 == 0 && M >= 4 * BM)
    return launch2<192>(stream, A, lda, M, K, W, N, epi);
  if (force_bn == 2192 || force_bn == 2256) {
    bn = force_bn - 2000;
    HM_CHECK(N % bn == 0 && epi.ln_gamma == nullptr, "gemm: pair kernel needs N %% %d == 0 and no fused LayerNorm", bn);
    return bn == 192 ? launch2<192>(stream, A, lda, M, K, W, N, epi) : launch2<256>(stream, A, lda, M, K, W, N, epi);
  }
  HM_CHECK(N % bn == 0, "gemm: N=%d not divisible by tile width %d", N, bn);
  switch (bn) {
    case 64: return launch<64>(stream, A, lda, M, K, W, N, epi);
    case 96: return launch<96>(stream, A, lda, M, K, W, N, epi);
    case 128: return launch<128>(stream, A, lda, M, K, W, N, epi);
    case 192: return launch<192>(stream, A, lda, M, K, W, N, epi);
    case 256: return launch<256>(stream, A, lda, M, K, W, N, epi);
  }
  HM_CHECK(false, "gemm: unsupported tile width %d", bn);
  return -2;
}

}
```

handwritten_math_ocr_api_b200/csrc/gemm.cuh:

```cuda
#pragma once
#include "common.cuh"

namespace hmocr {

struct GemmEpilogue {
  const float* bias = nullptr;
  int act = 0;
  const float* residual = nullptr;
  int ldr = 0;
  float* out_f32 = nullptr;
  int ld32 = 0;
  h16* out_f16 = nullptr;
  int ld16 = 0;
  const float* ln_gamma = nullptr;
  const float* ln_beta = nullptr;
};

int gemm_f16(cudaStream_t stream, const h16* A, int lda, int M, int K, const h16* W,
              int N, const GemmEpilogue& epi, int force_bn = 0);

bool conv_tiling(int Ho, int Wo, int* tw, int* th, int* tn);
int gemm_conv_f16(cudaStream_t stream, const h16* x, int B, int H, int W, int Cin, int ksize, int stride, int pad,
                  const h16* Wt, int N, const GemmEpilogue& epi);

int gemm_init();
int gemm_tensor_map(const void* ptr, int rows, int cols, int ld, int box_rows, CUtensorMap* out);
int gemm_num_sms();
void gemm_set_debug(int v);

}
```

handwritten_math_ocr_api_b200/csrc/kernels.cuh:

```cuda
#pragma once
#include "common.cuh"

namespace hmocr {

int layernorm(cudaStream_t st, const float* x, int rows, int C, const float* gamma, const float* beta,
              h16* out16, float* out32);
int patch_merge_ln(cudaStream_t st, const float* x, int B, int H, int W, int Cin, const float* gamma,
                   const float* beta, h16* out16);
int patch_embed(cudaStream_t st, const float* images, int B, const float* w, const float* b, const float* g,
                const float* beta, float* x);
int window_attention(cudaStream_t st, const h16* qkv, const float* qkv_bias, const float* rel_bias, int B,
                     int H, int W, int C, int heads, int shift, h16* ctx);

bool swin_mlp_supported(int C);
int swin_mlp(cudaStream_t st, const h16* xn, int M, int C, const h16* w1, const float* b1, const h16* w2,
             const float* b2, float* x);

struct DecodeState {
  int step;
  int finished_count;
  int steps_executed;
  int last_eos;
};

int embed_tokens(cudaStream_t st, const int64_t* tok, int ld_tok, int B, int T, const float* emb, const float* pos,
                 int d, int vocab, float* x32, h16* x16);

int mha_prefill_self(cudaStream_t st, const h16* qkv16, int B, int T, int nhead, h16* ctx16, bool causal = true);
int mha_full_mma(cudaStream_t st, const h16* qkv, int B, int T, int nhead, h16* ctx);
int mha_prefill_cross(cudaStream_t st, const h16* q16, const h16* memkv, int ld_mem, int koff,
                      int voff, int B, int T, int S, int nhead, h16* ctx16);

int self_attn_step(cudaStream_t st, const DecodeState* state, const h16* qkv16, h16* kcache,
                   h16* vcache, int rows, int nhead, int tmax, h16* ctx16);
int cross_attn_step(cudaStream_t st, const h16* q16, const h16* memkv, int ld_mem, int koff,
                    int voff, const int* mem_row, int rows, int S, int nhead, h16* ctx16);

int greedy_select(cudaStream_t st, DecodeState* state, const float* logits, int ld, int n_valid, int rows,
                  int64_t* tokens, int ld_tok, float* logprob, int max_len, int eos, uint8_t* finished,
                  const float* emb, const float* pos, int d, int max_pos, float* x32, h16* x16);
int advance_step(cudaStream_t st, DecodeState* state);
int pack_tokens(cudaStream_t st, const int64_t* tokens, int rows, int ld_tok, int sos, int eos, int pad, int32_t* lengths,
                int32_t* packed);
int init_decode(cudaStream_t st, DecodeState* state, int64_t* tokens, int ld_tok, int rows, int sos, int pad,
                uint8_t* finished, float* logprob, int max_len);
int finalize_decode(cudaStream_t st, const DecodeState* state, int64_t* tokens, int ld_tok, int rows, int max_len,
                    int pad, float* logprob, int32_t* steps_out);

int conv7x7_bn_relu(cudaStream_t st, const float* images, int B, const float* w, const float* bias, h16* out);
int maxpool3x3s2(cudaStream_t st, const h16* in, int B, int H, int W, int C, h16* out16, float* out32);
int im2col(cudaStream_t st, const h16* in, int B, int H, int W, int C, int k, int stride, int pad, h16* out);
int avgpool_h(cudaStream_t st, const float* in, int B, int H, int W, int C, h16* out);
int add_pos_permute(cudaStream_t st, const float* x, const float* pos, int B, int S, int d, float* o32, h16* o16);
int permute_back(cudaStream_t st, const float* x, int B, int S, int d, float* o32, h16* o16);

int preprocess_u8(cudaStream_t st, const uint8_t* in, size_t pixels, float* out);
int preprocess_gray_cv2(cudaStream_t st, const uint8_t* src_dev, int H, int W, int out_h, int out_w, int* tables_dev,
                        float* out_dev);
size_t preprocess_table_ints(int H, int W, int out_h, int out_w);
int preprocess_image(cudaStream_t st, const uint8_t* src_dev, int channels, int H, int W, int out_h, int out_w,
                     int* tables_dev, uint8_t* mid_dev, float* out_dev);

int copy_logits(cudaStream_t st, const float* src, int ld, int rows, int n_valid, float* dst);
int f32_to_f16(cudaStream_t st, const float* src, size_t n, h16* dst);

}
```

handwritten_math_ocr_api_b200/csrc/swin_kernels.cu:

```cuda
#include "kernels.cuh"

namespace hmocr {
namespace {

constexpr float LN_EPS = 1e-5f;

constexpr int LN_MAXV = 12;

struct RowSrc {
  const float* x;
  int C;
  __device__ __forceinline__ const float4* vec(int row, int idx) const {
    return reinterpret_cast<const float4*>(x + (size_t)row * C) + idx;
  }
};

struct MergeSrc {
  const float* x;
  int H, W, Cin;
  __device__ __forceinline__ const float4* vec(int row, int idx) const {
    const int Ho = H >> 1, Wo = W >> 1;
    const int j = row % Wo, i = (row / Wo) % Ho, b = row / (Wo * Ho);
    const int per = Cin >> 2;
    const int seg = idx / per, within = idx - seg * per;
    const int r = 2 * i + (seg & 1), c = 2 * j + (seg >> 1);
    return reinterpret_cast<const float4*>(x + ((size_t)(b * H + r) * W + c) * Cin) + within;
  }
};

template <class Src>
__global__ void __launch_bounds__(256) layernorm_kernel(Src src, int rows, int C, const float* __restrict__ gamma,
                                                        const float* __restrict__ beta,
                                                        h16* __restrict__ out16, float* __restrict__ out32) {
  const int lane = threadIdx.x & 31;
  const int row = blockIdx.x * (blockDim.x >> 5) + (threadIdx.x >> 5);
  if (row >= rows) return;
  const int nvec = C >> 2;
  float4 v[LN_MAXV];
  float sum = 0.f;
#pragma unroll
  for (int i = 0; i < LN_MAXV; ++i) {
    const int idx = lane + 32 * i;
    if (idx < nvec) {
      v[i] = *src.vec(row, idx);
      sum += v[i].x + v[i].y + v[i].z + v[i].w;
    }
  }
  const float mean = warp_sum(sum) / C;
  float sq = 0.f;
#pragma unroll
  for (int i = 0; i < LN_MAXV; ++i) {
    const int idx = lane + 32 * i;
    if (idx < nvec) {
      float a = v[i].x - mean, b = v[i].y - mean, c = v[i].z - mean, d = v[i].w - mean;
      sq += a * a + b * b + c * c + d * d;
    }
  }
  const float rstd = rsqrtf(warp_sum(sq) / C + LN_EPS);
#pragma unroll
  for (int i = 0; i < LN_MAXV; ++i) {
    const int idx = lane + 32 * i;
    if (idx < nvec) {
      const float4 g = __ldg(reinterpret_cast<const float4*>(gamma) + idx);
      const float4 b = __ldg(reinterpret_cast<const float4*>(beta) + idx);
      float4 y;
      y.x = (v[i].x - mean) * rstd * g.x + b.x;
      y.y = (v[i].y - mean) * rstd * g.y + b.y;
      y.z = (v[i].z - mean) * rstd * g.z + b.z;
      y.w = (v[i].w - mean) * rstd * g.w + b.w;
      if (out16 != nullptr)
        reinterpret_cast<uint2*>(out16 + (size_t)row * C)[idx] = make_uint2(pack16(y.x, y.y), pack16(y.z, y.w));
      if (out32 != nullptr) reinterpret_cast<float4*>(out32 + (size_t)row * C)[idx] = y;
    }
  }
}

template <int C, int V, bool MERGE>
__global__ void __launch_bounds__(256) layernorm_c_kernel(const float* __restrict__ x, int rows, int H, int W,
                                                          const float* __restrict__ gamma, const float* __restrict__ beta,
                                                          h16* __restrict__ out16, float* __restrict__ out32) {
  constexpr int G = C / (4 * V), RPW = 32 / G;
  static_assert(G >= 1 && G <= 32 && (G & (G - 1)) == 0 && G * 4 * V == C, "bad LayerNorm geometry");
  constexpr bool PARAMS_IN_REGS = V <= 3;
  const int lane = threadIdx.x & 31, g = lane % G, sub = lane / G;
  const int warps_total = gridDim.x * (blockDim.x >> 5);
  pdl_launch_dependents();
  float4 gr[PARAMS_IN_REGS ? V : 1], br[PARAMS_IN_REGS ? V : 1];
  if (PARAMS_IN_REGS) {
#pragma unroll
    for (int i = 0; i < V; ++i) {
      gr[i] = __ldg(reinterpret_cast<const float4*>(gamma) + g + G * i);
      br[i] = __ldg(reinterpret_cast<const float4*>(beta) + g + G * i);
    }
  }
  pdl_wait();
  for (int row0 = (blockIdx.x * (blockDim.x >> 5) + (threadIdx.x >> 5)) * RPW; row0 < rows; row0 += warps_total * RPW) {
    const int row = row0 + sub;
    const bool ok = row < rows;
    float4 v[V];
    float sum = 0.f;
    size_t base00 = 0;
    if (MERGE) {
      const int Ho = H >> 1, Wo = W >> 1, rr = ok ? row : 0;
      const int j = rr % Wo, i = (rr / Wo) % Ho, b = rr / (Wo * Ho);
      base00 = ((size_t)(b * H + 2 * i) * W + 2 * j) * (C / 4);
    }
#pragma unroll
    for (int i = 0; i < V; ++i) {
      const int idx = g + G * i;
      const float4* p;
      if (MERGE) {
        constexpr int per = C / 16;
        const int sgm = idx / per;
        p = reinterpret_cast<const float4*>(x + base00 + (size_t)((sgm & 1) * W + (sgm >> 1)) * (C / 4)) + (idx - sgm * per);
      } else {
        p = reinterpret_cast<const float4*>(x + (size_t)row * C) + idx;
      }
      v[i] = ok ? __ldcs(p) : make_float4(0.f, 0.f, 0.f, 0.f);
      sum += (v[i].x + v[i].y) + (v[i].z + v[i].w);
    }
#pragma unroll
    for (int o = G / 2; o > 0; o >>= 1) sum += __shfl_xor_sync(0xffffffffu, sum, o);
    const float mean = sum * (1.0f / C);
    float sq = 0.f;
#pragma unroll
    for (int i = 0; i < V; ++i) {
      v[i].x -= mean; v[i].y -= mean; v[i].z -= mean; v[i].w -= mean;
      sq += (v[i].x * v[i].x + v[i].y * v[i].y) + (v[i].z * v[i].z + v[i].w * v[i].w);
    }
#pragma unroll
    for (int o = G / 2; o > 0; o >>= 1) sq += __shfl_xor_sync(0xffffffffu, sq, o);
    const float rstd = rsqrtf(sq * (1.0f / C) + LN_EPS);
    if (!ok) continue;
#pragma unroll
    for (int i = 0; i < V; ++i) {
      const int idx = g + G * i;
      float4 gg, bb;
      if (PARAMS_IN_REGS) { gg = gr[i]; bb = br[i]; }
      else {
        gg = __ldg(reinterpret_cast<const float4*>(gamma) + idx);
        bb = __ldg(reinterpret_cast<const float4*>(beta) + idx);
      }
      float4 y;
      y.x = v[i].x * rstd * gg.x + bb.x; y.y = v[i].y * rstd * gg.y + bb.y;
      y.z = v[i].z * rstd * gg.z + bb.z; y.w = v[i].w * rstd * gg.w + bb.w;
      if (out16 != nullptr)
        reinterpret_cast<uint2*>(out16 + (size_t)row * C)[idx] = make_uint2(pack16(y.x, y.y), pack16(y.z, y.w));
      if (out32 != nullptr) reinterpret_cast<float4*>(out32 + (size_t)row * C)[idx] = y;
    }
  }
}

template <int C, int V, bool MERGE>
int launch_ln_c(cudaStream_t st, const float* x, int rows, int H, int W, const float* gamma, const float* beta,
                h16* out16, float* out32) {
  constexpr int RPW = 32 / (C / (4 * V));
  int blocks = ceil_div(rows, 8 * RPW);
  if (blocks > 148 * 8) blocks = 148 * 8;
  HM_CUDA(launch_pdl(layernorm_c_kernel<C, V, MERGE>, dim3(blocks), dim3(256), 0, st, x, rows, H, W, gamma, beta, out16, out32));
  HM_LAUNCHED();
  return 0;
}

constexpr int PE_WARPS = 4, PE_PITCH = 100;
struct PatchSmem {
  float wT[16][96];
  float bias[96], g[96], beta[96];
  float tile[PE_WARPS][32][PE_PITCH];
};

__global__ void __launch_bounds__(PE_WARPS * 32, 3) patch_embed_kernel(const float* __restrict__ img, int ntok,
                                                                      const float* __restrict__ w,
                                                                      const float* __restrict__ bias,
                                                                      const float* __restrict__ g,
                                                                      const float* __restrict__ beta,
                                                                      float* __restrict__ x) {
  extern __shared__ __align__(16) uint8_t pe_raw[];
  PatchSmem& s = *reinterpret_cast<PatchSmem*>(pe_raw);
  const int lane = threadIdx.x & 31, warp = threadIdx.x >> 5;
  pdl_launch_dependents();
  for (int i = threadIdx.x; i < 96 * 16; i += PE_WARPS * 32) s.wT[i & 15][i >> 4] = __ldg(w + i);
  for (int i = threadIdx.x; i < 96; i += PE_WARPS * 32) {
    s.bias[i] = __ldg(bias + i);
    s.g[i] = __ldg(g + i);
    s.beta[i] = __ldg(beta + i);
  }
  __syncthreads();
  pdl_wait();
  const uint32_t w_addr = smem_u32(&s.wT[0][0]), b_addr = smem_u32(&s.bias[0]);
  float(*tile)[PE_PITCH] = s.tile[warp];
  const int groups = ntok >> 5;
  for (int grp = blockIdx.x * PE_WARPS + warp; grp < groups; grp += gridDim.x * PE_WARPS) {
    const int tok = grp * 32 + lane;
    const int b = tok / 1920, rem = tok - b * 1920, ty = rem / 80, tx = rem - ty * 80;
    const float* base = img + ((size_t)b * 96 + ty * 4) * 320 + tx * 4;
    float px[16];
#pragma unroll
    for (int r = 0; r < 4; ++r) {
      const float4 v = __ldg(reinterpret_cast<const float4*>(base + r * 320));
      px[4 * r] = v.x; px[4 * r + 1] = v.y; px[4 * r + 2] = v.z; px[4 * r + 3] = v.w;
    }
    uint64_t acc[48];
#pragma unroll
    for (int c = 0; c < 24; ++c)
      asm volatile("ld.shared.v2.b64 {%0, %1}, [%2];" : "=l"(acc[2 * c]), "=l"(acc[2 * c + 1]) : "r"(b_addr + c * 16));
#pragma unroll
    for (int k = 0; k < 16; ++k) {
      const uint64_t pk = pk2(px[k], px[k]);
#pragma unroll
      for (int c = 0; c < 24; ++c) {
        uint64_t w0, w1;
        asm volatile("ld.shared.v2.b64 {%0, %1}, [%2];" : "=l"(w0), "=l"(w1) : "r"(w_addr + (k * 96 + c * 4) * 4));
        acc[2 * c] = fma2(pk, w0, acc[2 * c]);
        acc[2 * c + 1] = fma2(pk, w1, acc[2 * c + 1]);
      }
    }
    float o[96];
#pragma unroll
    for (int c = 0; c < 48; ++c) upk2(acc[c], o[2 * c], o[2 * c + 1]);
    float sum = 0.f;
#pragma unroll
    for (int c = 0; c < 96; ++c) sum += o[c];
    const float mean = sum * (1.0f / 96.0f);
    float sq = 0.f;
#pragma unroll
    for (int c = 0; c < 96; ++c) { o[c] -= mean; sq = fmaf(o[c], o[c], sq); }
    const float rstd = rsqrtf(sq * (1.0f / 96.0f) + LN_EPS);
    __syncwarp();
#pragma unroll
    for (int c = 0; c < 24; ++c) {
      const float4 gg = *reinterpret_cast<const float4*>(&s.g[4 * c]);
      const float4 bb = *reinterpret_cast<const float4*>(&s.beta[4 * c]);
      *reinterpret_cast<float4*>(&tile[lane][4 * c]) =
          make_float4(fmaf(o[4 * c] * rstd, gg.x, bb.x), fmaf(o[4 * c + 1] * rstd, gg.y, bb.y),
                      fmaf(o[4 * c + 2] * rstd, gg.z, bb.z), fmaf(o[4 * c + 3] * rstd, gg.w, bb.w));
    }
    __syncwarp();
    float* xo = x + (size_t)grp * 32 * 96;
#pragma unroll
    for (int it = 0; it < 24; ++it) {
      const int f = it * 128 + lane * 4, tk = f / 96, ch = f - tk * 96;
      *reinterpret_cast<float4*>(xo + f) = *reinterpret_cast<const float4*>(&tile[tk][ch]);
    }
  }
}

}

int layernorm(cudaStream_t st, const float* x, int rows, int C, const float* gamma, const float* beta,
              h16* out16, float* out32) {
  HM_CHECK(C % 4 == 0 && C <= LN_MAXV * 128, "layernorm: C=%d unsupported (multiple of 4, <= %d)", C, LN_MAXV * 128);
  HM_CHECK(rows > 0, "layernorm: empty input");
  switch (C) {
    case 96: return launch_ln_c<96, 3, false>(st, x, rows, 0, 0, gamma, beta, out16, out32);
    case 192: return launch_ln_c<192, 3, false>(st, x, rows, 0, 0, gamma, beta, out16, out32);
    case 384: return launch_ln_c<384, 3, false>(st, x, rows, 0, 0, gamma, beta, out16, out32);
    case 768: return launch_ln_c<768, 6, false>(st, x, rows, 0, 0, gamma, beta, out16, out32);
    default: break;
  }
  RowSrc src{x, C};
  layernorm_kernel<RowSrc><<<ceil_div(rows, 8), 256, 0, st>>>(src, rows, C, gamma, beta, out16, out32);
  HM_LAUNCHED();
  return 0;
}

int patch_merge_ln(cudaStream_t st, const float* x, int B, int H, int W, int Cin, const float* gamma,
                   const float* beta, h16* out16) {
  HM_CHECK(H % 2 == 0 && W % 2 == 0, "patch_merge: odd grid %dx%d (the reference pads; never hit at 96x320)", H, W);
  HM_CHECK(Cin % 4 == 0 && 4 * Cin <= LN_MAXV * 128, "patch_merge: C=%d unsupported", Cin);
  const int rows = B * (H / 2) * (W / 2);
  switch (Cin) {
    case 96: return launch_ln_c<384, 3, true>(st, x, rows, H, W, gamma, beta, out16, nullptr);
    case 192: return launch_ln_c<768, 6, true>(st, x, rows, H, W, gamma, beta, out16, nullptr);
    case 384: return launch_ln_c<1536, 12, true>(st, x, rows, H, W, gamma, beta, out16, nullptr);
    default: break;
  }
  MergeSrc src{x, H, W, Cin};
  layernorm_kernel<MergeSrc><<<ceil_div(rows, 8), 256, 0, st>>>(src, rows, 4 * Cin, gamma, beta, out16, nullptr);
  HM_LAUNCHED();
  return 0;
}

int patch_embed(cudaStream_t st, const float* images, int B, const float* w, const float* b, const float* g,
                const float* beta, float* x) {
  const int ntok = B * 24 * 80;
  HM_DEVICE_ONCE(HM_CUDA(cudaFuncSetAttribute(patch_embed_kernel, cudaFuncAttributeMaxDynamicSharedMemorySize, (int)sizeof(PatchSmem))));
  int blocks = ceil_div(ntok / 32, PE_WARPS);
  if (blocks > 148 * 3) blocks = 148 * 3;
  HM_CUDA(launch_pdl(patch_embed_kernel, dim3(blocks), dim3(PE_WARPS * 32), sizeof(PatchSmem), st, images, ntok, w, b, g, beta, x));
  HM_LAUNCHED();
  return 0;
}

}
```

handwritten_math_ocr_api_b200/csrc/swin_mlp.cu:

```cuda
#include "gemm.cuh"
#include "kernels.cuh"

namespace hmocr {
namespace {

constexpr int BM = 128, BK = 64, HC = 128;
constexpr int EPI_WARPS = 16;
constexpr int NUM_THREADS = 32 * (2 + EPI_WARPS);

template <int C>
struct MlpCfg {
  static constexpr int KB_A = (C + BK - 1) / BK;
  static constexpr int A_BYTES = KB_A * BM * BK * 2;
  static constexpr int NCH = 4 * C / HC;
  static constexpr int KB_H = HC / BK;
  static constexpr int H_BYTES = BM * HC * 2;
  static constexpr int W1_BOX = HC * BK * 2;
  static constexpr int W2_BOX = C * BK * 2;
  static constexpr int STAGE_BYTES = W1_BOX > W2_BOX ? W1_BOX : W2_BOX;
  static constexpr int STAGES = C == 96 ? 8 : (96 * 1024) / STAGE_BYTES;
  static constexpr int BAR_BYTES = 256;
  static constexpr int BIAS_BYTES = 4 * C * 4;
  static constexpr int SMEM_BYTES = A_BYTES + 2 * H_BYTES + STAGES * STAGE_BYTES + BAR_BYTES + BIAS_BYTES + 1024;
  static constexpr uint32_t ACC2_COL = 2 * HC;
  static_assert(C % 32 == 0 && C <= 256 && (4 * C) % HC == 0, "fused MLP: unsupported width");
  static_assert(ACC2_COL + C <= 512, "TMEM columns");
  static_assert(EPI_WARPS * 4096 <= 2 * H_BYTES, "the final epilogue's staging tiles alias the hidden buffers");
  static_assert(SMEM_BYTES <= 227 * 1024, "shared memory");
};

struct MlpParams {
  int M, num_tiles;
  const float* b1;
  const float* b2;
  float* x;
};

__device__ __forceinline__ uint64_t smem_desc(uint32_t saddr) {
  uint64_t d = 0;
  d |= static_cast<uint64_t>((saddr & 0x3FFFF) >> 4);
  d |= static_cast<uint64_t>(1) << 16;
  d |= static_cast<uint64_t>(1024 >> 4) << 32;
  d |= static_cast<uint64_t>(1) << 46;
  d |= static_cast<uint64_t>(2) << 61;
  return d;
}
__device__ __forceinline__ constexpr uint32_t idesc_f16(int n) {
  return (1u << 4) | (uint32_t(n >> 3) << 17) | (uint32_t(BM >> 4) << 24);
}

template <int C>
__global__ void __launch_bounds__(NUM_THREADS, 1)
swin_mlp_kernel(const __grid_constant__ CUtensorMap tmA, const __grid_constant__ CUtensorMap tmW1,
                const __grid_constant__ CUtensorMap tmW2, const MlpParams p) {
  using G = MlpCfg<C>;
  extern __shared__ uint8_t smem_raw[];
  const uint32_t raw_addr = smem_u32(smem_raw);
  uint8_t* smem = smem_raw + ((1024u - (raw_addr & 1023u)) & 1023u);
  uint8_t* sA = smem;
  uint8_t* sH = sA + G::A_BYTES;
  uint8_t* sW = sH + 2 * G::H_BYTES;
  uint64_t* bars = reinterpret_cast<uint64_t*>(sW + G::STAGES * G::STAGE_BYTES);
  uint64_t* w_full = bars;
  uint64_t* w_empty = w_full + G::STAGES;
  uint64_t* a_full = w_empty + G::STAGES;
  uint64_t* a_empty = a_full + 1;
  uint64_t* acc1_full = a_empty + 1;
  uint64_t* acc1_empty = acc1_full + 2;
  uint64_t* h_ready = acc1_empty + 2;
  uint64_t* h_free = h_ready + 2;
  uint64_t* acc2_full = h_free + 2;
  uint64_t* acc2_empty = acc2_full + 1;
  uint64_t* stg_free = acc2_empty + 1;
  uint32_t* tmem_slot = reinterpret_cast<uint32_t*>(stg_free + 1);
  float* s_b1 = reinterpret_cast<float*>(sW + G::STAGES * G::STAGE_BYTES + G::BAR_BYTES);

  const int warp = threadIdx.x >> 5, lane = threadIdx.x & 31;
  pdl_launch_dependents();
  if (warp == 0 && lane == 0) {
    tma_prefetch_desc(&tmA);
    tma_prefetch_desc(&tmW1);
    tma_prefetch_desc(&tmW2);
    for (int s = 0; s < G::STAGES; ++s) { mbar_init(&w_full[s], 1); mbar_init(&w_empty[s], 1); }
    mbar_init(a_full, 1);
    mbar_init(a_empty, 1);
    for (int b = 0; b < 2; ++b) {
      mbar_init(&acc1_full[b], 1);
      mbar_init(&acc1_empty[b], EPI_WARPS);
      mbar_init(&h_ready[b], EPI_WARPS);
      mbar_init(&h_free[b], 1);
    }
    mbar_init(acc2_full, 1);
    mbar_init(acc2_empty, EPI_WARPS);
    mbar_init(stg_free, EPI_WARPS);
    fence_barrier_init();
  }
  for (int i = threadIdx.x; i < 4 * C; i += NUM_THREADS) s_b1[i] = __ldg(p.b1 + i);
  if (warp == 1) tmem_alloc(tmem_slot, 512);
  tc_fence_before();
  __syncthreads();
  tc_fence_after();
  const uint32_t tmem_base = *tmem_slot;
  pdl_wait();

  if (warp == 0) {
    if (lane == 0) {
      int s = 0;
      uint32_t ph = 0;
      auto push_w1 = [&](int j) {
        for (int kb = 0; kb < G::KB_A; ++kb) {
          mbar_wait(&w_empty[s], ph ^ 1u);
          mbar_expect_tx(&w_full[s], G::W1_BOX);
          tma_load_2d(sW + s * G::STAGE_BYTES, &tmW1, &w_full[s], kb * BK, j * HC);
          if (++s == G::STAGES) { s = 0; ph ^= 1u; }
        }
      };
      auto push_w2 = [&](int j) {
        for (int kb = 0; kb < G::KB_H; ++kb) {
          mbar_wait(&w_empty[s], ph ^ 1u);
          mbar_expect_tx(&w_full[s], G::W2_BOX);
          tma_load_2d(sW + s * G::STAGE_BYTES, &tmW2, &w_full[s], j * HC + kb * BK, 0);
          if (++s == G::STAGES) { s = 0; ph ^= 1u; }
        }
      };
      uint32_t it = 0;
      for (int t = blockIdx.x; t < p.num_tiles; t += gridDim.x, ++it) {
        {
          const int rows = p.M - t * BM < BM ? p.M - t * BM : BM;
          asm volatile("cp.async.bulk.prefetch.L2.global [%0], %1;" ::"l"(reinterpret_cast<uint64_t>(p.x + (size_t)t * BM * C)),
                       "r"(rows * C * 4)
                       : "memory");
        }
        mbar_wait(a_empty, (it & 1u) ^ 1u);
        mbar_expect_tx(a_full, G::A_BYTES);
        for (int kb = 0; kb < G::KB_A; ++kb) tma_load_2d(sA + kb * (BM * BK * 2), &tmA, a_full, kb * BK, t * BM);
        for (int j = 0; j <= G::NCH; ++j) {
          if (j < G::NCH) push_w1(j);
          if (j >= 1) push_w2(j - 1);
        }
      }
    }
  } else if (warp == 1) {
    if (lane == 0) {
      constexpr uint32_t idesc1 = idesc_f16(HC), idesc2 = idesc_f16(C);
      int s = 0;
      uint32_t ph = 0;
      uint32_t n_acc1[2] = {0u, 0u}, n_h[2] = {0u, 0u};
      uint32_t it = 0;
      const uint32_t a_base = smem_u32(sA), h_base = smem_u32(sH);
      for (int t = blockIdx.x; t < p.num_tiles; t += gridDim.x, ++it) {
        mbar_wait_backoff(a_full, it & 1u);
        for (int j = 0; j <= G::NCH; ++j) {
          if (j < G::NCH) {
            const int b = j & 1;
            mbar_wait_backoff(&acc1_empty[b], (n_acc1[b] & 1u) ^ 1u);
            ++n_acc1[b];
            tc_fence_after();
            const uint32_t d_tmem = tmem_base + b * HC;
            for (int kb = 0; kb < G::KB_A; ++kb) {
              mbar_wait(&w_full[s], ph);
              tc_fence_after();
              const uint32_t wb = smem_u32(sW + s * G::STAGE_BYTES);
              const int nks = (C - kb * BK) >= BK ? BK / 16 : (C - kb * BK) / 16;
              for (int k = 0; k < nks; ++k)
                umma_f16(d_tmem, smem_desc(a_base + kb * (BM * BK * 2) + k * 32), smem_desc(wb + k * 32), idesc1,
                         (kb | k) != 0 ? 1u : 0u);
              umma_commit(&w_empty[s]);
              if (++s == G::STAGES) { s = 0; ph ^= 1u; }
            }
            umma_commit(&acc1_full[b]);
            if (j == G::NCH - 1) umma_commit(a_empty);
          }
          if (j >= 1) {
            const int jj = j - 1, b = jj & 1;
            if (jj == 0) mbar_wait_backoff(acc2_empty, (it & 1u) ^ 1u);
            mbar_wait_backoff(&h_ready[b], n_h[b] & 1u);
            ++n_h[b];
            tc_fence_after();
            const uint32_t d_tmem = tmem_base + G::ACC2_COL;
            for (int kb = 0; kb < G::KB_H; ++kb) {
              mbar_wait(&w_full[s], ph);
              tc_fence_after();
              const uint32_t wb = smem_u32(sW + s * G::STAGE_BYTES);
              const uint32_t hb = h_base + b * G::H_BYTES + kb * (BM * BK * 2);
#pragma unroll
              for (int k = 0; k < BK / 16; ++k)
                umma_f16(d_tmem, smem_desc(hb + k * 32), smem_desc(wb + k * 32), idesc2, (jj | kb | k) != 0 ? 1u : 0u);
              umma_commit(&w_empty[s]);
              if (++s == G::STAGES) { s = 0; ph ^= 1u; }
            }
            umma_commit(&h_free[b]);
            if (jj == G::NCH - 1) umma_commit(acc2_full);
          }
        }
      }
    }
  } else {
    const int ew = warp - 2;
    const int quarter = warp & 3;
    const int cgrp = ew >> 2;
    const uint32_t lane_base = tmem_base + (uint32_t(quarter * 32) << 16);
    const int row_in_tile = quarter * 32 + lane;
    uint32_t n_acc1[2] = {0u, 0u}, n_h[2] = {0u, 0u};
    uint32_t it = 0;
    const uint32_t h_row = smem_u32(sH) + (cgrp >> 1) * (BM * BK * 2) + row_in_tile * 128;
    const uint32_t h_sw = row_in_tile & 7, h_c0 = (cgrp & 1) * 4;
    const uint32_t st_addr = smem_u32(sH) + ew * 4096;
    const int rr = lane >> 3, cg4 = lane & 7;
    for (int t = blockIdx.x; t < p.num_tiles; t += gridDim.x, ++it) {
      const int m0 = t * BM;
      for (int j = 0; j < G::NCH; ++j) {
        const int b = j & 1;
        mbar_wait_backoff(&acc1_full[b], n_acc1[b] & 1u);
        ++n_acc1[b];
        tc_fence_after();
        uint32_t r[32];
        tmem_ld32(lane_base + b * HC + cgrp * 32, r);
        tc_fence_before();
        __syncwarp();
        if (lane == 0) mbar_arrive(&acc1_empty[b]);
        const float4* bp = reinterpret_cast<const float4*>(s_b1 + j * HC + cgrp * 32);
        uint32_t h[16];
#pragma unroll
        for (int q = 0; q < 8; ++q) {
          const float4 bb = bp[q];
          float v0, v1, v2, v3;
          upk2(add2(pk2(__uint_as_float(r[4 * q]), __uint_as_float(r[4 * q + 1])), pk2(bb.x, bb.y)), v0, v1);
          upk2(add2(pk2(__uint_as_float(r[4 * q + 2]), __uint_as_float(r[4 * q + 3])), pk2(bb.z, bb.w)), v2, v3);
          gelu_erf2(v0, v1);
          gelu_erf2(v2, v3);
          h[2 * q] = pack16(v0, v1);
          h[2 * q + 1] = pack16(v2, v3);
        }
        mbar_wait_backoff(&h_free[b], (n_h[b] & 1u) ^ 1u);
        ++n_h[b];
        if (j < 2) mbar_wait_backoff(stg_free, (it & 1u) ^ 1u);
        const uint32_t dst = h_row + b * G::H_BYTES;
#pragma unroll
        for (int q = 0; q < 4; ++q)
          asm volatile("st.shared.v4.b32 [%0], {%1, %2, %3, %4};" ::"r"(dst + (((h_c0 + q) ^ h_sw) << 4)), "r"(h[4 * q]),
                       "r"(h[4 * q + 1]), "r"(h[4 * q + 2]), "r"(h[4 * q + 3])
                       : "memory");
        fence_proxy_async();
        __syncwarp();
        if (lane == 0) mbar_arrive(&h_ready[b]);
      }
      const int mb = m0 + quarter * 32;
      const int rows_left = p.M - mb - rr;
      bool first = true;
      for (int c = cgrp; c < C / 32; c += 4) {
        const int col = c * 32 + cg4 * 4;
        float* xp = p.x + (size_t)(mb + rr) * C + col;
        float4 res[8];
#pragma unroll
        for (int i4 = 0; i4 < 8; ++i4)
          res[i4] = (i4 * 4 < rows_left) ? __ldcs(reinterpret_cast<const float4*>(xp + (size_t)i4 * 4 * C))
                                         : make_float4(0.f, 0.f, 0.f, 0.f);
        const float4 bias = __ldg(reinterpret_cast<const float4*>(p.b2 + col));
        if (first) {
          mbar_wait_backoff(acc2_full, it & 1u);
          tc_fence_after();
          first = false;
        }
        uint32_t r[32];
        tmem_ld32(lane_base + G::ACC2_COL + c * 32, r);
#pragma unroll
        for (int q = 0; q < 8; ++q)
          asm volatile("st.shared.v4.b32 [%0], {%1, %2, %3, %4};" ::"r"(st_addr + lane * 128 + ((q ^ (lane & 7)) << 4)),
                       "r"(r[4 * q]), "r"(r[4 * q + 1]), "r"(r[4 * q + 2]), "r"(r[4 * q + 3])
                       : "memory");
        __syncwarp();
#pragma unroll
        for (int i4 = 0; i4 < 8; ++i4) {
          float4 v;
          asm volatile("ld.shared.v4.f32 {%0, %1, %2, %3}, [%4];"
                       : "=f"(v.x), "=f"(v.y), "=f"(v.z), "=f"(v.w)
                       : "r"(st_addr + rr * 128 + i4 * 512 + ((cg4 ^ ((i4 * 4 + rr) & 7)) << 4)));
          v.x += bias.x + res[i4].x; v.y += bias.y + res[i4].y; v.z += bias.z + res[i4].z; v.w += bias.w + res[i4].w;
          if (i4 * 4 < rows_left) *reinterpret_cast<float4*>(xp + (size_t)i4 * 4 * C) = v;
        }
        __syncwarp();
      }
      if (first) {
        mbar_wait_backoff(acc2_full, it & 1u);
        tc_fence_after();
      }
      tc_fence_before();
      __syncwarp();
      if (lane == 0) {
        mbar_arrive(acc2_empty);
        mbar_arrive(stg_free);
      }
    }
  }

  tc_fence_before();
  __syncthreads();
  if (warp == 1) {
    __syncwarp();
    tmem_dealloc(tmem_base, 512);
  }
}

template <int C>
int launch_mlp(cudaStream_t st, const h16* xn, int M, const h16* w1, const float* b1, const h16* w2, const float* b2,
               float* x) {
  using G = MlpCfg<C>;
  HM_DEVICE_ONCE(HM_CUDA(cudaFuncSetAttribute(swin_mlp_kernel<C>, cudaFuncAttributeMaxDynamicSharedMemorySize, G::SMEM_BYTES)));
  alignas(64) CUtensorMap tmA, tmW1, tmW2;
  HM_TRY(gemm_tensor_map(xn, M, C, C, BM, &tmA));
  HM_TRY(gemm_tensor_map(w1, 4 * C, C, C, HC, &tmW1));
  HM_TRY(gemm_tensor_map(w2, C, 4 * C, 4 * C, C, &tmW2));
  MlpParams p;
  p.M = M;
  p.num_tiles = ceil_div(M, BM);
  p.b1 = b1; p.b2 = b2; p.x = x;
  const int sms = gemm_num_sms();
  const int grid = p.num_tiles < sms ? p.num_tiles : sms;
  HM_CUDA(launch_pdl(swin_mlp_kernel<C>, dim3(grid), dim3(NUM_THREADS), G::SMEM_BYTES, st, tmA, tmW1, tmW2, p));
  HM_LAUNCHED();
  return 0;
}

}

bool swin_mlp_supported(int C) { return C == 96 || C == 192; }

int swin_mlp(cudaStream_t st, const h16* xn, int M, int C, const h16* w1, const float* b1, const h16* w2,
             const float* b2, float* x) {
  HM_TRY(gemm_init());
  HM_CHECK(M > 0, "swin_mlp: empty input");
  HM_CHECK(b1 != nullptr && b2 != nullptr, "swin_mlp: biases missing");
  HM_CHECK((reinterpret_cast<uintptr_t>(xn) & 15) == 0 && (reinterpret_cast<uintptr_t>(x) & 15) == 0, "swin_mlp: unaligned operands");
  switch (C) {
    case 96: return launch_mlp<96>(st, xn, M, w1, b1, w2, b2, x);
    case 192: return launch_mlp<192>(st, xn, M, w1, b1, w2, b2, x);
    default: break;
  }
  HM_CHECK(false, "swin_mlp: C=%d unsupported (96, 192)", C);
  return -2;
}

}
```

include/hmocr.h:

```cpp
#ifndef HMOCR_H_
#define HMOCR_H_

#include <stddef.h>
#include <stdint.h>

#ifdef __cplusplus
extern "C" {
#endif

typedef struct hmocr_engine hmocr_engine;

typedef struct hmocr_config {
  int32_t vocab_size;
  int32_t d_model;
  int32_t nhead;
  int32_t dim_feedforward;
  int32_t num_layers;
  int32_t max_seq_len;
  int32_t sos_id, eos_id, pad_id;
  int32_t encoder_arch;
  int32_t enc_num_layers;
} hmocr_config;

enum { HMOCR_F32 = 0, HMOCR_I64 = 1 };

const char* hmocr_last_error(void);
const char* hmocr_version(void);
int64_t hmocr_launch_count(void);

int hmocr_create(const hmocr_config* cfg, hmocr_engine** out);
void hmocr_destroy(hmocr_engine* e);

int hmocr_load_weight(hmocr_engine* e, const char* key, const void* data_host, const int64_t* shape, int ndim,
                      int dtype);
int hmocr_finalize_weights(hmocr_engine* e);

int hmocr_set_option(hmocr_engine* e, const char* name, int value);
int hmocr_read_trace(hmocr_engine* e, int64_t* out_host, int n);

int hmocr_set_pos_table(hmocr_engine* e, const float* pos_host, int rows, int d, void* stream);

int hmocr_workspace_bytes(hmocr_engine* e, int batch, int max_len, int beam, size_t* bytes);
int hmocr_set_workspace(hmocr_engine* e, void* workspace_dev, size_t bytes, void* stream);

int hmocr_decode_max_clusters(int* out);

int hmocr_encode(hmocr_engine* e, const float* images_dev, int batch, float* enc_out_dev, void* stream);

int hmocr_decoder_forward(hmocr_engine* e, const float* enc_out_dev, const int64_t* tgt_dev, int batch, int T,
                          float* logits_dev, void* stream);

int hmocr_generate(hmocr_engine* e, const float* images_dev, int batch, int max_len, int beam, int64_t* tokens_dev,
                   float* logprob_dev, int32_t* steps_dev, float* score_dev, void* stream);

int hmocr_generate_from_memory(hmocr_engine* e, const float* enc_out_dev, int batch, int max_len, int beam,
                               int64_t* tokens_dev, float* logprob_dev, int32_t* steps_dev, float* score_dev,
                               void* stream);

int hmocr_generate_nbest(hmocr_engine* e, const float* input_dev, int input_is_memory, int batch, int max_len, int beam,
                         int n_best, int64_t* tokens_dev, float* logprob_dev, float* score_dev, int32_t* steps_dev,
                         void* stream);

int hmocr_generate_host(hmocr_engine* e, const float* images_host, int batch, int max_len, int beam,
                        int64_t* tokens_host, float* logprob_host, int32_t* steps_host, float* score_host,
                        void* stream);

int hmocr_preprocess_image_u8(hmocr_engine* e, const uint8_t* image_host, int channels, int height, int width,
                              float* image_dev, void* stream);

int hmocr_preprocess_cv2_u8(hmocr_engine* e, const uint8_t* gray_host, int height, int width, float* image_dev,
                            void* stream);

int hmocr_pack_tokens(hmocr_engine* e, const int64_t* tokens_dev, int rows, int ld_tok, int32_t* lengths_dev,
                      int32_t* packed_dev, void* stream);

int hmocr_preprocess_u8(hmocr_engine* e, const uint8_t* images_u8_dev, int batch, float* images_dev, void* stream);

int hmocr_generate_host_u8(hmocr_engine* e, const uint8_t* images_u8_host, int batch, int max_len, int beam,
                           int64_t* tokens_host, float* logprob_host, int32_t* steps_host, float* score_host,
                           void* stream);

int hmocr_last_decode_steps(hmocr_engine* e, int32_t* steps_run);

int hmocr_last_timings(hmocr_engine* e, float* encoder_ms, float* decode_ms);


int hmocr_gemm_f16(const void* a_dev, int lda, int M, int K, const void* w_dev, int N, const float* bias_dev,
                    int act, const float* residual_dev, int ldr, float* out_f32_dev, int ld32, void* out_f16_dev,
                    int ld16, const float* ln_gamma_dev, const float* ln_beta_dev, int force_bn, void* stream);

int hmocr_swin_mlp(const void* xn_dev, int M, int C, const void* w1_dev, const float* b1_dev, const void* w2_dev,
                   const float* b2_dev, float* x_dev, void* stream);

int hmocr_layernorm(const float* x_dev, int rows, int C, const float* gamma_dev, const float* beta_dev,
                    void* out_f16_dev, float* out_f32_dev, void* stream);

int hmocr_patch_embed(const float* images_dev, int batch, const float* conv_w_dev, const float* conv_b_dev,
                      const float* ln_g_dev, const float* ln_b_dev, float* x_dev, void* stream);

int hmocr_patch_merge_ln(const float* x_dev, int batch, int H, int W, int C, const float* gamma_dev,
                         const float* beta_dev, void* out_f16_dev, void* stream);

int hmocr_self_attention(const void* qkv_dev, int B, int T, int nhead, int causal, void* ctx_f16_dev, void* stream);

int hmocr_window_attention(const void* qkv_dev, const float* qkv_bias_dev, const float* rel_bias_dev, int batch,
                           int H, int W, int C, int heads, int shift, void* ctx_f16_dev, void* stream);

#ifdef __cplusplus
}
#endif
#endif
```

Baseline: 13870.

## Fold LayerNorm into QKV GEMM and Swin MLP A-operand producers

Adds a LayerNorm-fused variant of the tcgen05 GEMM. Extra producer warps normalize fp32 rows straight into shared-memory A tiles, double-buffered, with an L2 bulk prefetch and a remapped tile schedule. The swin_mlp kernel gets the same in-kernel LayerNorm path. The encoder's norm1+qkv and norm2+mlp stages now skip the separate layernorm launch and the fp16 xn round trip through global memory. The cost is higher shared-memory use, fewer pipeline stages, and LN work repeated across N-tile splits, which could lower GEMM throughput.

```diff
diff --git a/handwritten_math_ocr_api_b200/_lib.py b/handwritten_math_ocr_api_b200/_lib.py
--- a/handwritten_math_ocr_api_b200/_lib.py
+++ b/handwritten_math_ocr_api_b200/_lib.py
@@ -43,7 +43,9 @@
     "hmocr_last_decode_steps": (_i, [_p, C.POINTER(C.c_int32)]),
     "hmocr_last_timings": (_i, [_p, C.POINTER(C.c_float), C.POINTER(C.c_float)]),
     "hmocr_gemm_f16": (_i, [_p, _i, _i, _i, _p, _i, _p, _i, _p, _i, _p, _i, _p, _i, _p, _p, _i, _p]),
+    "hmocr_gemm_ln_f16": (_i, [_p, _p, _p, _i, _i, _p, _i, _p, _i, _p, _i, _p]),
     "hmocr_swin_mlp": (_i, [_p, _i, _i, _p, _p, _p, _p, _p, _p]),
+    "hmocr_swin_mlp_ln": (_i, [_p, _p, _i, _i, _p, _p, _p, _p, _p, _p]),
     "hmocr_layernorm": (_i, [_p, _i, _i, _p, _p, _p, _p, _p]),
     "hmocr_patch_embed": (_i, [_p, _i, _p, _p, _p, _p, _p, _p]),
     "hmocr_patch_merge_ln": (_i, [_p, _i, _i, _i, _i, _p, _p, _p, _p]),
diff --git a/handwritten_math_ocr_api_b200/csrc/engine.cu b/handwritten_math_ocr_api_b200/csrc/engine.cu
--- a/handwritten_math_ocr_api_b200/csrc/engine.cu
+++ b/handwritten_math_ocr_api_b200/csrc/engine.cu
@@ -326,6 +326,15 @@
   return gemm_f16(st, a, lda, M, l.k, l.w, l.n, epi);
 }
 
+int run_lin_ln(cudaStream_t st, const float* x, const Norm& n, h16* xn, int M, const Lin& l, GemmEpilogue epi) {
+  if (l.k <= 192) {
+    epi.bias = l.b;
+    return gemm_ln_f16(st, x, n.g, n.b, M, l.k, l.w, l.n, epi);
+  }
+  HM_TRY(layernorm(st, x, M, l.k, n.g, n.b, xn, nullptr));
+  return run_lin(st, xn, l.k, M, l, epi);
+}
+
 int encode_impl(hmocr_engine* e, const float* images, int B, float* enc32, h16* enc16, cudaStream_t st) {
   const size_t tok1 = (size_t)B * 24 * 80;
   float *xa, *xb;
@@ -346,21 +355,19 @@
     const int rows = B * H * W;
     for (int j = 0; j < DEPTHS[s]; ++j, ++blk) {
       const SwinBlock& sb = e->blocks[blk];
-      HM_TRY(layernorm(st, x, rows, C, sb.n1.g, sb.n1.b, xn, nullptr));
       GemmEpilogue eq;
       eq.out_f16 = qkv; eq.ld16 = 3 * C;
-      HM_TRY(run_lin(st, xn, C, rows, sb.qkv, eq));
+      HM_TRY(run_lin_ln(st, x, sb.n1, xn, rows, sb.qkv, eq));
       HM_TRY(window_attention(st, qkv, sb.qkv.b, sb.rel_bias, B, H, W, C, HEADS[s], (j & 1) ? 3 : 0, ctx));
       GemmEpilogue ep;
       ep.residual = x; ep.ldr = C; ep.out_f32 = x; ep.ld32 = C;
       HM_TRY(run_lin(st, ctx, C, rows, sb.proj, ep));
-      HM_TRY(layernorm(st, x, rows, C, sb.n2.g, sb.n2.b, xn, nullptr));
       if (e->mlp_fused && swin_mlp_supported(C)) {
-        HM_TRY(swin_mlp(st, xn, rows, C, sb.fc1.w, sb.fc1.b, sb.fc2.w, sb.fc2.b, x));
+        HM_TRY(swin_mlp(st, nullptr, sb.n2.g, sb.n2.b, rows, C, sb.fc1.w, sb.fc1.b, sb.fc2.w, sb.fc2.b, x));
       } else {
         GemmEpilogue e1;
         e1.act = 1; e1.out_f16 = hid; e1.ld16 = 4 * C;
-        HM_TRY(run_lin(st, xn, C, rows, sb.fc1, e1));
+        HM_TRY(run_lin_ln(st, x, sb.n2, xn, rows, sb.fc1, e1));
         GemmEpilogue e2;
         e2.residual = x; e2.ldr = C; e2.out_f32 = x; e2.ld32 = C;
         HM_TRY(run_lin(st, hid, 4 * C, rows, sb.fc2, e2));
@@ -1428,10 +1435,25 @@
                    static_cast<const h16*>(w), N, epi, force_bn);
 }
 
+HM_API int hmocr_gemm_ln_f16(const float* x, const float* ln_gamma, const float* ln_beta, int M, int K, const void* w,
+                             int N, const float* bias, int act, void* out_f16, int ld16, void* stream) {
+  GemmEpilogue epi;
+  epi.bias = bias; epi.act = act;
+  epi.out_f16 = static_cast<h16*>(out_f16); epi.ld16 = ld16;
+  return gemm_ln_f16(static_cast<cudaStream_t>(stream), x, ln_gamma, ln_beta, M, K, static_cast<const h16*>(w), N, epi);
+}
+
 HM_API int hmocr_swin_mlp(const void* xn, int M, int C, const void* w1, const float* b1, const void* w2, const float* b2,
                           float* x, void* stream) {
   HM_CHECK(xn != nullptr && w1 != nullptr && w2 != nullptr && x != nullptr, "null buffer");
-  return swin_mlp(static_cast<cudaStream_t>(stream), static_cast<const h16*>(xn), M, C, static_cast<const h16*>(w1), b1,
+  return swin_mlp(static_cast<cudaStream_t>(stream), static_cast<const h16*>(xn), nullptr, nullptr, M, C,
+                  static_cast<const h16*>(w1), b1, static_cast<const h16*>(w2), b2, x);
+}
+
+HM_API int hmocr_swin_mlp_ln(const float* ln_gamma, const float* ln_beta, int M, int C, const void* w1, const float* b1,
+                             const void* w2, const float* b2, float* x, void* stream) {
+  HM_CHECK(ln_gamma != nullptr && ln_beta != nullptr && w1 != nullptr && w2 != nullptr && x != nullptr, "null buffer");
+  return swin_mlp(static_cast<cudaStream_t>(stream), nullptr, ln_gamma, ln_beta, M, C, static_cast<const h16*>(w1), b1,
                   static_cast<const h16*>(w2), b2, x);
 }
 
diff --git a/handwritten_math_ocr_api_b200/csrc/gemm.cu b/handwritten_math_ocr_api_b200/csrc/gemm.cu
--- a/handwritten_math_ocr_api_b200/csrc/gemm.cu
+++ b/handwritten_math_ocr_api_b200/csrc/gemm.cu
@@ -1,4 +1,5 @@
 #include "gemm.cuh"
+#include "layernorm.cuh"
 
 #include <map>
 #include <mutex>
@@ -13,18 +14,23 @@
 constexpr int GROUP_WARPS = 8;
 constexpr int NUM_THREADS = 32 * (2 + EPI_WARPS);
 constexpr int EPI_WARP_BYTES = 4096 + 128;
-
-template <int BN>
+constexpr int LN_WARPS = 4;
+constexpr int LN_KB = 3;
+constexpr int LN_BN = 96;
+
+template <int BN, bool LNA = false>
 struct Cfg {
   static constexpr int A_BYTES = BM * BK * 2;
   static constexpr int B_BYTES = BN * BK * 2;
-  static constexpr int STAGE_BYTES = A_BYTES + B_BYTES;
+  static constexpr int STAGE_BYTES = (LNA ? 0 : A_BYTES) + B_BYTES;
+  static constexpr int LN_A_BYTES = LNA ? 2 * LN_KB * A_BYTES : 0;
   static constexpr int EPI_STAGE_BYTES = EPI_WARPS * EPI_WARP_BYTES;
-  static constexpr int STAGES_RAW = (156 * 1024) / STAGE_BYTES;
+  static constexpr int STAGES_RAW = (156 * 1024 - LN_A_BYTES) / STAGE_BYTES;
   static constexpr int STAGES = STAGES_RAW > 8 ? 8 : STAGES_RAW;
   static constexpr int TMEM_COLS = (2 * BN <= 128) ? 128 : ((2 * BN <= 256) ? 256 : 512);
   static constexpr int BAR_BYTES = 256;
-  static constexpr int SMEM_BYTES = STAGES * STAGE_BYTES + 1024 + BAR_BYTES + EPI_STAGE_BYTES;
+  static constexpr int SMEM_BYTES = STAGES * STAGE_BYTES + LN_A_BYTES + 1024 + BAR_BYTES + EPI_STAGE_BYTES;
+  static constexpr int THREADS = NUM_THREADS + (LNA ? 32 * LN_WARPS : 0);
 };
 
 enum EpiMode { EPI_GENERAL = 0, EPI_F16 = 1, EPI_LN = 2 };
@@ -43,6 +49,10 @@
 struct GemmParams {
   int M, N, K;
   int num_n_tiles, num_tiles;
+  int num_m_tiles, nsplit;
+  const float* ln_x;
+  const float* ln_g;
+  const float* ln_b;
   int mode;
   ConvGeom cg;
   int dbg;
@@ -277,28 +287,43 @@
   }
 }
 
-template <int BN, bool CONV>
-__global__ void __launch_bounds__(NUM_THREADS, 1)
+template <bool LNA>
+__device__ __forceinline__ bool tile_of(const GemmParams& p, int it, int& t) {
+  if (!LNA) {
+    t = blockIdx.x + it * gridDim.x;
+    return t < p.num_tiles;
+  }
+  const int per_unit = p.num_n_tiles / p.nsplit;
+  const int u = blockIdx.x + (it / per_unit) * gridDim.x;
+  t = (u / p.nsplit) * p.num_n_tiles + u % p.nsplit + (it % per_unit) * p.nsplit;
+  return u < p.num_m_tiles * p.nsplit;
+}
+
+template <int BN, bool CONV, bool LNA = false>
+__global__ void __launch_bounds__(Cfg<BN, LNA>::THREADS, 1)
 gemm_tcgen05_kernel(const __grid_constant__ CUtensorMap tmA, const __grid_constant__ CUtensorMap tmB,
                     const GemmParams p) {
-  using C = Cfg<BN>;
+  using C = Cfg<BN, LNA>;
   extern __shared__ uint8_t smem_raw[];
   const uint32_t raw_addr = smem_u32(smem_raw);
   uint8_t* smem = smem_raw + ((1024u - (raw_addr & 1023u)) & 1023u);
 
-  uint64_t* full_bar = reinterpret_cast<uint64_t*>(smem + C::STAGES * C::STAGE_BYTES);
+  uint8_t* ln_a = smem + C::STAGES * C::STAGE_BYTES;
+  uint64_t* full_bar = reinterpret_cast<uint64_t*>(ln_a + C::LN_A_BYTES);
   uint64_t* empty_bar = full_bar + C::STAGES;
   uint64_t* tfull_bar = empty_bar + C::STAGES;
   uint64_t* tempty_bar = tfull_bar + 2;
-  uint32_t* tmem_slot = reinterpret_cast<uint32_t*>(tempty_bar + 2);
-  const uint32_t epi_stage = smem_u32(smem + C::STAGES * C::STAGE_BYTES + C::BAR_BYTES);
+  uint64_t* afull_bar = tempty_bar + 2;
+  uint64_t* aempty_bar = afull_bar + 2;
+  uint32_t* tmem_slot = reinterpret_cast<uint32_t*>(aempty_bar + 2);
+  const uint32_t epi_stage = smem_u32(ln_a + C::LN_A_BYTES + C::BAR_BYTES);
 
   const int warp = threadIdx.x >> 5;
   const int lane = threadIdx.x & 31;
   pdl_launch_dependents();
 
   if (warp == 0 && lane == 0) {
-    tma_prefetch_desc(&tmA);
+    if (!LNA) tma_prefetch_desc(&tmA);
     tma_prefetch_desc(&tmB);
     for (int s = 0; s < C::STAGES; ++s) {
       mbar_init(&full_bar[s], 1);
@@ -307,10 +332,17 @@
     for (int a = 0; a < 2; ++a) {
       mbar_init(&tfull_bar[a], 1);
       mbar_init(&tempty_bar[a], GROUP_WARPS);
+      mbar_init(&afull_bar[a], LN_WARPS);
+      mbar_init(&aempty_bar[a], 1);
     }
     fence_barrier_init();
   }
   if (warp == 1) tmem_alloc(tmem_slot, C::TMEM_COLS);
+  if (LNA) {
+    for (int i = threadIdx.x; i < C::LN_A_BYTES / 16; i += C::THREADS)
+      *reinterpret_cast<uint4*>(ln_a + i * 16) = make_uint4(0u, 0u, 0u, 0u);
+    fence_proxy_async();
+  }
   tc_fence_before();
   __syncthreads();
   tc_fence_after();
@@ -322,7 +354,8 @@
     if (lane == 0) {
       int s = 0;
       uint32_t ph = 0;
-      for (int t = blockIdx.x; t < p.num_tiles; t += gridDim.x) {
+      int t;
+      for (int it = 0; tile_of<LNA>(p, it, t); ++it) {
         const int m0 = (t / p.num_n_tiles) * BM;
         const int n0 = (t % p.num_n_tiles) * BN;
         int cw = 0, chh = 0, cn = 0;
@@ -341,11 +374,13 @@
             const int tap = kb / p.cg.cin_blocks, cb = kb - tap * p.cg.cin_blocks;
             const int kh = tap / p.cg.ksize, kw = tap - kh * p.cg.ksize;
             tma_load_4d(st, &tmA, &full_bar[s], cb * BK, cw + kw, chh + kh, cn);
-          } else {
+          } else if (!LNA) {
             mbar_expect_tx(&full_bar[s], C::STAGE_BYTES);
             tma_load_2d(st, &tmA, &full_bar[s], kb * BK, m0);
+          } else {
+            mbar_expect_tx(&full_bar[s], C::B_BYTES);
           }
-          tma_load_2d(st + C::A_BYTES, &tmB, &full_bar[s], kb * BK, n0);
+          tma_load_2d(st + (LNA ? 0 : C::A_BYTES), &tmB, &full_bar[s], kb * BK, n0);
           if (++s == C::STAGES) { s = 0; ph ^= 1u; }
         }
       }
@@ -355,18 +390,22 @@
       constexpr uint32_t idesc = make_idesc<BN>();
       int s = 0;
       uint32_t ph = 0;
-      int it = 0;
-      for (int t = blockIdx.x; t < p.num_tiles; t += gridDim.x, ++it) {
+      const int per_unit = LNA ? p.num_n_tiles / p.nsplit : 1;
+      int t;
+      for (int it = 0; tile_of<LNA>(p, it, t); ++it) {
         const int a = it & 1;
         const uint32_t aph = (it >> 1) & 1;
+        const int unit = it / per_unit, ab = unit & 1;
+        if (LNA && it % per_unit == 0) mbar_wait_backoff(&afull_bar[ab], (unit >> 1) & 1);
         mbar_wait_backoff(&tempty_bar[a], aph ^ 1u);
         tc_fence_after();
         const uint32_t d_tmem = tmem_base + a * BN;
         for (int kb = 0; kb < num_kb; ++kb) {
           mbar_wait(&full_bar[s], ph);
           tc_fence_after();
-          const uint32_t abase = smem_u32(smem + s * C::STAGE_BYTES);
-          const uint32_t bbase = abase + C::A_BYTES;
+          const uint32_t sbase = smem_u32(smem + s * C::STAGE_BYTES);
+          const uint32_t abase = LNA ? smem_u32(ln_a) + (ab * LN_KB + kb) * C::A_BYTES : sbase;
+          const uint32_t bbase = LNA ? sbase : sbase + C::A_BYTES;
 #pragma unroll
           for (int k = 0; k < BK / 16; ++k) {
             umma_f16(d_tmem, make_smem_desc(abase + k * 32), make_smem_desc(bbase + k * 32), idesc,
@@ -376,7 +415,34 @@
           if (++s == C::STAGES) { s = 0; ph ^= 1u; }
         }
         umma_commit(&tfull_bar[a]);
-      }
+        if (LNA && it % per_unit == per_unit - 1) umma_commit(&aempty_bar[ab]);
+      }
+    }
+  } else if (LNA && warp >= 2 + EPI_WARPS) {
+    const int w = warp - 2 - EPI_WARPS;
+    const int units = p.num_m_tiles * p.nsplit;
+    auto prefetch = [&](int u) {
+      const int m0 = (u / p.nsplit) * BM, rows = p.M - m0 < BM ? p.M - m0 : BM;
+      asm volatile("cp.async.bulk.prefetch.L2.global [%0], %1;" ::"l"(reinterpret_cast<uint64_t>(p.ln_x + (size_t)m0 * p.K)),
+                   "r"(rows * p.K * 4)
+                   : "memory");
+    };
+    if (w == 0 && lane == 0) {
+      prefetch(blockIdx.x);
+      if (blockIdx.x + gridDim.x < units) prefetch(blockIdx.x + gridDim.x);
+    }
+    int k = 0;
+    for (int u = blockIdx.x; u < units; u += gridDim.x, ++k) {
+      if (w == 0 && lane == 0 && u + 2 * (int)gridDim.x < units) prefetch(u + 2 * gridDim.x);
+      const int ab = k & 1;
+      mbar_wait_backoff(&aempty_bar[ab], ((k >> 1) & 1) ^ 1u);
+      const uint32_t abuf = smem_u32(ln_a) + ab * LN_KB * C::A_BYTES;
+      const int m0 = (u / p.nsplit) * BM;
+      if (p.K == 96) ln_rows_to_tile<96, 32, 4>(p.ln_x, p.M, m0, 32 * w, p.ln_g, p.ln_b, abuf);
+      else ln_rows_to_tile<192, 32, 4>(p.ln_x, p.M, m0, 32 * w, p.ln_g, p.ln_b, abuf);
+      fence_proxy_async();
+      __syncwarp();
+      if (lane == 0) mbar_arrive(&afull_bar[ab]);
     }
   } else {
     const int quarter = warp & 3;
@@ -386,8 +452,8 @@
     const uint32_t st_addr = epi_stage + ew * EPI_WARP_BYTES;
     const uint32_t taddr = tmem_base + (uint32_t(quarter * 32) << 16) + group * BN;
     const bool has_res = p.epi.residual != nullptr && !(p.dbg & 2);
-    int it = group;
-    for (int t = blockIdx.x + group * gridDim.x; t < p.num_tiles; t += 2 * gridDim.x, it += 2) {
+    int t;
+    for (int it = group; tile_of<LNA>(p, it, t); it += 2) {
       const uint32_t aph = (it >> 1) & 1;
       const int m0 = (t / p.num_n_tiles) * BM;
       const int n0 = (t % p.num_n_tiles) * BN;
@@ -395,7 +461,10 @@
       tc_fence_after();
       const int mb = m0 + quarter * 32;
       const int mi = t / p.num_n_tiles, rq = quarter * 32;
-      if (p.mode == EPI_LN) {
+      if (LNA) {
+        if (p.epi.act == 1) epilogue_f16<BN, 1, false>(p.epi, taddr, st_addr, mb, p.M, n0, half, p.dbg, smem_u32(&tempty_bar[group]), p.cg, 0, 0);
+        else epilogue_f16<BN, 0, false>(p.epi, taddr, st_addr, mb, p.M, n0, half, p.dbg, smem_u32(&tempty_bar[group]), p.cg, 0, 0);
+      } else if (p.mode == EPI_LN) {
         const int row = mb + lane;
         if (half == 0) epilogue_ln<BN>(p.epi, taddr, row, row < p.M, n0);
       } else if (p.mode == EPI_F16) {
@@ -616,6 +685,31 @@
            : (epi.out_f32 == nullptr && epi.residual == nullptr && epi.act != 3) ? EPI_F16 : EPI_GENERAL;
   const int grid = p.num_tiles < num_sms() ? p.num_tiles : num_sms();
   HM_CUDA(launch_pdl(gemm_tcgen05_kernel<BN, false>, dim3(grid), dim3(NUM_THREADS), C::SMEM_BYTES, stream, tmA, tmB, p));
+  HM_LAUNCHED();
+  return 0;
+}
+
+int launch_ln(cudaStream_t stream, const float* x, const float* gamma, const float* beta, int M, int K, const h16* W, int N,
+              const GemmEpilogue& epi) {
+  using C = Cfg<LN_BN, true>;
+  alignas(64) CUtensorMap tmB;
+  HM_TRY(get_tensor_map(W, N, K, K, LN_BN, &tmB));
+  GemmParams p;
+  p.M = M; p.N = N; p.K = K;
+  p.num_n_tiles = N / LN_BN;
+  p.num_m_tiles = ceil_div(M, BM);
+  p.num_tiles = p.num_m_tiles * p.num_n_tiles;
+  p.nsplit = 1;
+  for (int d = 1; d <= p.num_n_tiles; ++d)
+    if (p.num_n_tiles % d == 0 && p.num_m_tiles * d <= num_sms()) p.nsplit = d;
+  p.ln_x = x; p.ln_g = gamma; p.ln_b = beta;
+  p.epi = epi;
+  p.dbg = g_gemm_dbg;
+  p.mode = (epi.out_f32 == nullptr && epi.residual == nullptr && epi.act != 3) ? EPI_F16 : EPI_GENERAL;
+  p.cg = ConvGeom{};
+  const int units = p.num_m_tiles * p.nsplit;
+  const int grid = units < num_sms() ? units : num_sms();
+  HM_CUDA(launch_pdl(gemm_tcgen05_kernel<LN_BN, false, true>, dim3(grid), dim3(C::THREADS), C::SMEM_BYTES, stream, tmB, tmB, p));
   HM_LAUNCHED();
   return 0;
 }
@@ -782,6 +876,8 @@
   HM_CUDA(cudaFuncSetAttribute(gemm_tcgen05_kernel<64, true>, cudaFuncAttributeMaxDynamicSharedMemorySize, Cfg<64>::SMEM_BYTES));
   HM_CUDA(cudaFuncSetAttribute(gemm_tcgen05_kernel<128, true>, cudaFuncAttributeMaxDynamicSharedMemorySize, Cfg<128>::SMEM_BYTES));
   HM_CUDA(cudaFuncSetAttribute(gemm_tcgen05_kernel<256, true>, cudaFuncAttributeMaxDynamicSharedMemorySize, Cfg<256>::SMEM_BYTES));
+  HM_CUDA(cudaFuncSetAttribute(gemm_tcgen05_kernel<LN_BN, false, true>, cudaFuncAttributeMaxDynamicSharedMemorySize,
+                               Cfg<LN_BN, true>::SMEM_BYTES));
   g_encode = reinterpret_cast<EncodeTiledFn>(fn);
   g_sms[dev] = prop.multiProcessorCount;
   return 0;
@@ -837,4 +933,20 @@
   return -2;
 }
 
-}
+int gemm_ln_f16(cudaStream_t stream, const float* x, const float* gamma, const float* beta, int M, int K, const h16* W,
+                int N, const GemmEpilogue& epi) {
+  HM_TRY(gemm_init());
+  HM_CHECK(M > 0 && N > 0, "gemm_ln: empty problem M=%d N=%d", M, N);
+  HM_CHECK(K == 96 || K == 192, "gemm_ln: K=%d unsupported (96, 192)", K);
+  HM_CHECK(N % LN_BN == 0, "gemm_ln: N=%d must be a multiple of %d", N, LN_BN);
+  HM_CHECK(x != nullptr && gamma != nullptr && beta != nullptr, "gemm_ln: null LayerNorm input");
+  HM_CHECK(((reinterpret_cast<uintptr_t>(x) | reinterpret_cast<uintptr_t>(gamma) | reinterpret_cast<uintptr_t>(beta) |
+             reinterpret_cast<uintptr_t>(W)) & 15) == 0, "gemm_ln: operands must be 16-byte aligned");
+  HM_CHECK(epi.ln_gamma == nullptr, "gemm_ln: no LayerNorm epilogue on the LayerNorm-fed kernel");
+  HM_CHECK(epi.out_f32 == nullptr && epi.residual == nullptr && epi.out_f16 != nullptr && (epi.act == 0 || epi.act == 1),
+           "gemm_ln: fp16 output with bias and optional GELU only");
+  HM_CHECK(epi.ld16 % 8 == 0, "gemm_ln: ld16 must be a multiple of 8");
+  return launch_ln(stream, x, gamma, beta, M, K, W, N, epi);
+}
+
+}
diff --git a/handwritten_math_ocr_api_b200/csrc/gemm.cuh b/handwritten_math_ocr_api_b200/csrc/gemm.cuh
--- a/handwritten_math_ocr_api_b200/csrc/gemm.cuh
+++ b/handwritten_math_ocr_api_b200/csrc/gemm.cuh
@@ -19,6 +19,9 @@
 int gemm_f16(cudaStream_t stream, const h16* A, int lda, int M, int K, const h16* W,
               int N, const GemmEpilogue& epi, int force_bn = 0);
 
+int gemm_ln_f16(cudaStream_t stream, const float* x, const float* gamma, const float* beta, int M, int K, const h16* W,
+                int N, const GemmEpilogue& epi);
+
 bool conv_tiling(int Ho, int Wo, int* tw, int* th, int* tn);
 int gemm_conv_f16(cudaStream_t stream, const h16* x, int B, int H, int W, int Cin, int ksize, int stride, int pad,
                   const h16* Wt, int N, const GemmEpilogue& epi);
diff --git a/handwritten_math_ocr_api_b200/csrc/kernels.cuh b/handwritten_math_ocr_api_b200/csrc/kernels.cuh
--- a/handwritten_math_ocr_api_b200/csrc/kernels.cuh
+++ b/handwritten_math_ocr_api_b200/csrc/kernels.cuh
@@ -13,8 +13,8 @@
                      int H, int W, int C, int heads, int shift, h16* ctx);
 
 bool swin_mlp_supported(int C);
-int swin_mlp(cudaStream_t st, const h16* xn, int M, int C, const h16* w1, const float* b1, const h16* w2,
-             const float* b2, float* x);
+int swin_mlp(cudaStream_t st, const h16* xn, const float* ln_g, const float* ln_b, int M, int C, const h16* w1,
+             const float* b1, const h16* w2, const float* b2, float* x);
 
 struct DecodeState {
   int step;
diff --git a/handwritten_math_ocr_api_b200/csrc/layernorm.cuh b/handwritten_math_ocr_api_b200/csrc/layernorm.cuh
--- /dev/null
+++ b/handwritten_math_ocr_api_b200/csrc/layernorm.cuh
@@ -0,0 +1,77 @@
+#pragma once
+#include "common.cuh"
+
+namespace hmocr {
+
+constexpr float LN_EPS = 1e-5f;
+
+template <int C, int V>
+struct LnGeom {
+  static constexpr int G = C / (4 * V);
+  static constexpr int RPW = 32 / G;
+  static_assert(G >= 1 && G <= 32 && (G & (G - 1)) == 0 && G * 4 * V == C, "bad LayerNorm geometry");
+};
+
+template <int C, int V>
+__device__ __forceinline__ float ln_center(float4 (&v)[V]) {
+  constexpr int G = LnGeom<C, V>::G;
+  float sum = 0.f;
+#pragma unroll
+  for (int i = 0; i < V; ++i) sum += (v[i].x + v[i].y) + (v[i].z + v[i].w);
+#pragma unroll
+  for (int o = G / 2; o > 0; o >>= 1) sum += __shfl_xor_sync(0xffffffffu, sum, o);
+  const float mean = sum * (1.0f / C);
+  float sq = 0.f;
+#pragma unroll
+  for (int i = 0; i < V; ++i) {
+    v[i].x -= mean; v[i].y -= mean; v[i].z -= mean; v[i].w -= mean;
+    sq += (v[i].x * v[i].x + v[i].y * v[i].y) + (v[i].z * v[i].z + v[i].w * v[i].w);
+  }
+#pragma unroll
+  for (int o = G / 2; o > 0; o >>= 1) sq += __shfl_xor_sync(0xffffffffu, sq, o);
+  return rsqrtf(sq * (1.0f / C) + LN_EPS);
+}
+
+__device__ __forceinline__ float4 ln_scale(const float4& v, float rstd, const float4& g, const float4& b) {
+  return make_float4(__fmaf_rn(__fmul_rn(v.x, rstd), g.x, b.x), __fmaf_rn(__fmul_rn(v.y, rstd), g.y, b.y),
+                     __fmaf_rn(__fmul_rn(v.z, rstd), g.z, b.z), __fmaf_rn(__fmul_rn(v.w, rstd), g.w, b.w));
+}
+
+__device__ __forceinline__ uint2 ln_pack16(const float4& y) { return make_uint2(pack16(y.x, y.y), pack16(y.z, y.w)); }
+
+template <int C, int ROWS, int BATCH>
+__device__ __forceinline__ void ln_rows_to_tile(const float* __restrict__ x, int M, int m0, int r0,
+                                                const float* __restrict__ gamma, const float* __restrict__ beta,
+                                                uint32_t a_base) {
+  constexpr int V = 3, G = LnGeom<C, V>::G, RPW = LnGeom<C, V>::RPW;
+  static_assert(ROWS % (RPW * BATCH) == 0, "rows per call");
+  const int lane = threadIdx.x & 31, g = lane % G, sub = lane / G;
+#pragma unroll 1
+  for (int p0 = 0; p0 < ROWS; p0 += RPW * BATCH) {
+    float4 v[BATCH][V];
+#pragma unroll
+    for (int ps = 0; ps < BATCH; ++ps) {
+      const int row = m0 + r0 + p0 + ps * RPW + sub;
+      const float4* src = reinterpret_cast<const float4*>(x + (size_t)row * C);
+#pragma unroll
+      for (int i = 0; i < V; ++i) v[ps][i] = row < M ? src[g + G * i] : make_float4(0.f, 0.f, 0.f, 0.f);
+    }
+#pragma unroll
+    for (int ps = 0; ps < BATCH; ++ps) {
+      const int r = r0 + p0 + ps * RPW + sub;
+      const bool ok = m0 + r < M;
+      const float rstd = ln_center<C, V>(v[ps]);
+#pragma unroll
+      for (int i = 0; i < V; ++i) {
+        const int idx = g + G * i;
+        const uint2 h = ok ? ln_pack16(ln_scale(v[ps][i], rstd, __ldg(reinterpret_cast<const float4*>(gamma) + idx),
+                                                __ldg(reinterpret_cast<const float4*>(beta) + idx)))
+                           : make_uint2(0u, 0u);
+        const uint32_t addr = a_base + (idx >> 4) * 16384 + r * 128 + ((((idx & 15) >> 1) ^ (r & 7)) << 4) + (idx & 1) * 8;
+        asm volatile("st.shared.v2.b32 [%0], {%1, %2};" ::"r"(addr), "r"(h.x), "r"(h.y) : "memory");
+      }
+    }
+  }
+}
+
+}
diff --git a/handwritten_math_ocr_api_b200/csrc/swin_kernels.cu b/handwritten_math_ocr_api_b200/csrc/swin_kernels.cu
--- a/handwritten_math_ocr_api_b200/csrc/swin_kernels.cu
+++ b/handwritten_math_ocr_api_b200/csrc/swin_kernels.cu
@@ -1,9 +1,8 @@
 #include "kernels.cuh"
+#include "layernorm.cuh"
 
 namespace hmocr {
 namespace {
-
-constexpr float LN_EPS = 1e-5f;
 
 constexpr int LN_MAXV = 12;
 
@@ -79,8 +78,7 @@
 __global__ void __launch_bounds__(256) layernorm_c_kernel(const float* __restrict__ x, int rows, int H, int W,
                                                           const float* __restrict__ gamma, const float* __restrict__ beta,
                                                           h16* __restrict__ out16, float* __restrict__ out32) {
-  constexpr int G = C / (4 * V), RPW = 32 / G;
-  static_assert(G >= 1 && G <= 32 && (G & (G - 1)) == 0 && G * 4 * V == C, "bad LayerNorm geometry");
+  constexpr int G = LnGeom<C, V>::G, RPW = LnGeom<C, V>::RPW;
   constexpr bool PARAMS_IN_REGS = V <= 3;
   const int lane = threadIdx.x & 31, g = lane % G, sub = lane / G;
   const int warps_total = gridDim.x * (blockDim.x >> 5);
@@ -98,7 +96,6 @@
     const int row = row0 + sub;
     const bool ok = row < rows;
     float4 v[V];
-    float sum = 0.f;
     size_t base00 = 0;
     if (MERGE) {
       const int Ho = H >> 1, Wo = W >> 1, rr = ok ? row : 0;
@@ -117,20 +114,8 @@
         p = reinterpret_cast<const float4*>(x + (size_t)row * C) + idx;
       }
       v[i] = ok ? __ldcs(p) : make_float4(0.f, 0.f, 0.f, 0.f);
-      sum += (v[i].x + v[i].y) + (v[i].z + v[i].w);
-    }
-#pragma unroll
-    for (int o = G / 2; o > 0; o >>= 1) sum += __shfl_xor_sync(0xffffffffu, sum, o);
-    const float mean = sum * (1.0f / C);
-    float sq = 0.f;
-#pragma unroll
-    for (int i = 0; i < V; ++i) {
-      v[i].x -= mean; v[i].y -= mean; v[i].z -= mean; v[i].w -= mean;
-      sq += (v[i].x * v[i].x + v[i].y * v[i].y) + (v[i].z * v[i].z + v[i].w * v[i].w);
-    }
-#pragma unroll
-    for (int o = G / 2; o > 0; o >>= 1) sq += __shfl_xor_sync(0xffffffffu, sq, o);
-    const float rstd = rsqrtf(sq * (1.0f / C) + LN_EPS);
+    }
+    const float rstd = ln_center<C, V>(v);
     if (!ok) continue;
 #pragma unroll
     for (int i = 0; i < V; ++i) {
@@ -141,11 +126,8 @@
         gg = __ldg(reinterpret_cast<const float4*>(gamma) + idx);
         bb = __ldg(reinterpret_cast<const float4*>(beta) + idx);
       }
-      float4 y;
-      y.x = v[i].x * rstd * gg.x + bb.x; y.y = v[i].y * rstd * gg.y + bb.y;
-      y.z = v[i].z * rstd * gg.z + bb.z; y.w = v[i].w * rstd * gg.w + bb.w;
-      if (out16 != nullptr)
-        reinterpret_cast<uint2*>(out16 + (size_t)row * C)[idx] = make_uint2(pack16(y.x, y.y), pack16(y.z, y.w));
+      const float4 y = ln_scale(v[i], rstd, gg, bb);
+      if (out16 != nullptr) reinterpret_cast<uint2*>(out16 + (size_t)row * C)[idx] = ln_pack16(y);
       if (out32 != nullptr) reinterpret_cast<float4*>(out32 + (size_t)row * C)[idx] = y;
     }
   }
@@ -154,7 +136,7 @@
 template <int C, int V, bool MERGE>
 int launch_ln_c(cudaStream_t st, const float* x, int rows, int H, int W, const float* gamma, const float* beta,
                 h16* out16, float* out32) {
-  constexpr int RPW = 32 / (C / (4 * V));
+  constexpr int RPW = LnGeom<C, V>::RPW;
   int blocks = ceil_div(rows, 8 * RPW);
   if (blocks > 148 * 8) blocks = 148 * 8;
   HM_CUDA(launch_pdl(layernorm_c_kernel<C, V, MERGE>, dim3(blocks), dim3(256), 0, st, x, rows, H, W, gamma, beta, out16, out32));
diff --git a/handwritten_math_ocr_api_b200/csrc/swin_mlp.cu b/handwritten_math_ocr_api_b200/csrc/swin_mlp.cu
--- a/handwritten_math_ocr_api_b200/csrc/swin_mlp.cu
+++ b/handwritten_math_ocr_api_b200/csrc/swin_mlp.cu
@@ -1,5 +1,6 @@
 #include "gemm.cuh"
 #include "kernels.cuh"
+#include "layernorm.cuh"
 
 namespace hmocr {
 namespace {
@@ -34,6 +35,8 @@
   const float* b1;
   const float* b2;
   float* x;
+  const float* ln_g;
+  const float* ln_b;
 };
 
 __device__ __forceinline__ uint64_t smem_desc(uint32_t saddr) {
@@ -49,7 +52,7 @@
   return (1u << 4) | (uint32_t(n >> 3) << 17) | (uint32_t(BM >> 4) << 24);
 }
 
-template <int C>
+template <int C, bool LNA>
 __global__ void __launch_bounds__(NUM_THREADS, 1)
 swin_mlp_kernel(const __grid_constant__ CUtensorMap tmA, const __grid_constant__ CUtensorMap tmW1,
                 const __grid_constant__ CUtensorMap tmW2, const MlpParams p) {
@@ -78,11 +81,11 @@
   const int warp = threadIdx.x >> 5, lane = threadIdx.x & 31;
   pdl_launch_dependents();
   if (warp == 0 && lane == 0) {
-    tma_prefetch_desc(&tmA);
+    if (!LNA) tma_prefetch_desc(&tmA);
     tma_prefetch_desc(&tmW1);
     tma_prefetch_desc(&tmW2);
     for (int s = 0; s < G::STAGES; ++s) { mbar_init(&w_full[s], 1); mbar_init(&w_empty[s], 1); }
-    mbar_init(a_full, 1);
+    mbar_init(a_full, LNA ? EPI_WARPS : 1);
     mbar_init(a_empty, 1);
     for (int b = 0; b < 2; ++b) {
       mbar_init(&acc1_full[b], 1);
@@ -102,6 +105,12 @@
   tc_fence_after();
   const uint32_t tmem_base = *tmem_slot;
   pdl_wait();
+  auto prefetch_rows = [&](int t) {
+    const int rows = p.M - t * BM < BM ? p.M - t * BM : BM;
+    asm volatile("cp.async.bulk.prefetch.L2.global [%0], %1;" ::"l"(reinterpret_cast<uint64_t>(p.x + (size_t)t * BM * C)),
+                 "r"(rows * C * 4)
+                 : "memory");
+  };
 
   if (warp == 0) {
     if (lane == 0) {
@@ -125,15 +134,13 @@
       };
       uint32_t it = 0;
       for (int t = blockIdx.x; t < p.num_tiles; t += gridDim.x, ++it) {
-        {
-          const int rows = p.M - t * BM < BM ? p.M - t * BM : BM;
-          asm volatile("cp.async.bulk.prefetch.L2.global [%0], %1;" ::"l"(reinterpret_cast<uint64_t>(p.x + (size_t)t * BM * C)),
-                       "r"(rows * C * 4)
-                       : "memory");
-        }
-        mbar_wait(a_empty, (it & 1u) ^ 1u);
-        mbar_expect_tx(a_full, G::A_BYTES);
-        for (int kb = 0; kb < G::KB_A; ++kb) tma_load_2d(sA + kb * (BM * BK * 2), &tmA, a_full, kb * BK, t * BM);
+        if (!LNA) prefetch_rows(t);
+        else if (t + (int)gridDim.x < p.num_tiles) prefetch_rows(t + gridDim.x);
+        if (!LNA) {
+          mbar_wait(a_empty, (it & 1u) ^ 1u);
+          mbar_expect_tx(a_full, G::A_BYTES);
+          for (int kb = 0; kb < G::KB_A; ++kb) tma_load_2d(sA + kb * (BM * BK * 2), &tmA, a_full, kb * BK, t * BM);
+        }
         for (int j = 0; j <= G::NCH; ++j) {
           if (j < G::NCH) push_w1(j);
           if (j >= 1) push_w2(j - 1);
@@ -207,6 +214,13 @@
     const uint32_t h_sw = row_in_tile & 7, h_c0 = (cgrp & 1) * 4;
     const uint32_t st_addr = smem_u32(sH) + ew * 4096;
     const int rr = lane >> 3, cg4 = lane & 7;
+    auto fill_a = [&](int t) {
+      ln_rows_to_tile<C, 8, 2>(p.x, p.M, t * BM, ew * 8, p.ln_g, p.ln_b, smem_u32(sA));
+      fence_proxy_async();
+      __syncwarp();
+      if (lane == 0) mbar_arrive(a_full);
+    };
+    if (LNA) fill_a(blockIdx.x);
     for (int t = blockIdx.x; t < p.num_tiles; t += gridDim.x, ++it) {
       const int m0 = t * BM;
       for (int j = 0; j < G::NCH; ++j) {
@@ -245,6 +259,10 @@
         __syncwarp();
         if (lane == 0) mbar_arrive(&h_ready[b]);
       }
+      if (LNA && t + (int)gridDim.x < p.num_tiles) {
+        mbar_wait_backoff(a_empty, it & 1u);
+        fill_a(t + gridDim.x);
+      }
       const int mb = m0 + quarter * 32;
       const int rows_left = p.M - mb - rr;
       bool first = true;
@@ -302,22 +320,24 @@
   }
 }
 
-template <int C>
-int launch_mlp(cudaStream_t st, const h16* xn, int M, const h16* w1, const float* b1, const h16* w2, const float* b2,
-               float* x) {
+template <int C, bool LNA>
+int launch_mlp(cudaStream_t st, const h16* xn, const float* ln_g, const float* ln_b, int M, const h16* w1,
+               const float* b1, const h16* w2, const float* b2, float* x) {
   using G = MlpCfg<C>;
-  HM_DEVICE_ONCE(HM_CUDA(cudaFuncSetAttribute(swin_mlp_kernel<C>, cudaFuncAttributeMaxDynamicSharedMemorySize, G::SMEM_BYTES)));
+  HM_DEVICE_ONCE(HM_CUDA(cudaFuncSetAttribute(swin_mlp_kernel<C, LNA>, cudaFuncAttributeMaxDynamicSharedMemorySize, G::SMEM_BYTES)));
   alignas(64) CUtensorMap tmA, tmW1, tmW2;
-  HM_TRY(gemm_tensor_map(xn, M, C, C, BM, &tmA));
   HM_TRY(gemm_tensor_map(w1, 4 * C, C, C, HC, &tmW1));
   HM_TRY(gemm_tensor_map(w2, C, 4 * C, 4 * C, C, &tmW2));
+  if (LNA) tmA = tmW1;
+  else HM_TRY(gemm_tensor_map(xn, M, C, C, BM, &tmA));
   MlpParams p;
   p.M = M;
   p.num_tiles = ceil_div(M, BM);
   p.b1 = b1; p.b2 = b2; p.x = x;
+  p.ln_g = ln_g; p.ln_b = ln_b;
   const int sms = gemm_num_sms();
   const int grid = p.num_tiles < sms ? p.num_tiles : sms;
-  HM_CUDA(launch_pdl(swin_mlp_kernel<C>, dim3(grid), dim3(NUM_THREADS), G::SMEM_BYTES, st, tmA, tmW1, tmW2, p));
+  HM_CUDA(launch_pdl(swin_mlp_kernel<C, LNA>, dim3(grid), dim3(NUM_THREADS), G::SMEM_BYTES, st, tmA, tmW1, tmW2, p));
   HM_LAUNCHED();
   return 0;
 }
@@ -326,15 +346,22 @@
 
 bool swin_mlp_supported(int C) { return C == 96 || C == 192; }
 
-int swin_mlp(cudaStream_t st, const h16* xn, int M, int C, const h16* w1, const float* b1, const h16* w2,
-             const float* b2, float* x) {
+int swin_mlp(cudaStream_t st, const h16* xn, const float* ln_g, const float* ln_b, int M, int C, const h16* w1,
+             const float* b1, const h16* w2, const float* b2, float* x) {
   HM_TRY(gemm_init());
   HM_CHECK(M > 0, "swin_mlp: empty input");
   HM_CHECK(b1 != nullptr && b2 != nullptr, "swin_mlp: biases missing");
-  HM_CHECK((reinterpret_cast<uintptr_t>(xn) & 15) == 0 && (reinterpret_cast<uintptr_t>(x) & 15) == 0, "swin_mlp: unaligned operands");
+  HM_CHECK((xn != nullptr) != (ln_g != nullptr), "swin_mlp: give either xn or the LayerNorm parameters");
+  HM_CHECK(xn != nullptr || ln_b != nullptr, "swin_mlp: LayerNorm beta missing");
+  HM_CHECK((reinterpret_cast<uintptr_t>(xn) & 15) == 0 && (reinterpret_cast<uintptr_t>(x) & 15) == 0 &&
+           (reinterpret_cast<uintptr_t>(ln_g) & 15) == 0 && (reinterpret_cast<uintptr_t>(ln_b) & 15) == 0,
+           "swin_mlp: unaligned operands");
+  const bool lna = xn == nullptr;
   switch (C) {
-    case 96: return launch_mlp<96>(st, xn, M, w1, b1, w2, b2, x);
-    case 192: return launch_mlp<192>(st, xn, M, w1, b1, w2, b2, x);
+    case 96: return lna ? launch_mlp<96, true>(st, xn, ln_g, ln_b, M, w1, b1, w2, b2, x)
+                        : launch_mlp<96, false>(st, xn, ln_g, ln_b, M, w1, b1, w2, b2, x);
+    case 192: return lna ? launch_mlp<192, true>(st, xn, ln_g, ln_b, M, w1, b1, w2, b2, x)
+                         : launch_mlp<192, false>(st, xn, ln_g, ln_b, M, w1, b1, w2, b2, x);
     default: break;
   }
   HM_CHECK(false, "swin_mlp: C=%d unsupported (96, 192)", C);
diff --git a/include/hmocr.h b/include/hmocr.h
--- a/include/hmocr.h
+++ b/include/hmocr.h
@@ -89,8 +89,13 @@
                     int act, const float* residual_dev, int ldr, float* out_f32_dev, int ld32, void* out_f16_dev,
                     int ld16, const float* ln_gamma_dev, const float* ln_beta_dev, int force_bn, void* stream);
 
+int hmocr_gemm_ln_f16(const float* x_dev, const float* ln_gamma_dev, const float* ln_beta_dev, int M, int K,
+                      const void* w_dev, int N, const float* bias_dev, int act, void* out_f16_dev, int ld16, void* stream);
+
 int hmocr_swin_mlp(const void* xn_dev, int M, int C, const void* w1_dev, const float* b1_dev, const void* w2_dev,
                    const float* b2_dev, float* x_dev, void* stream);
+int hmocr_swin_mlp_ln(const float* ln_gamma_dev, const float* ln_beta_dev, int M, int C, const void* w1_dev,
+                      const float* b1_dev, const void* w2_dev, const float* b2_dev, float* x_dev, void* stream);
 
 int hmocr_layernorm(const float* x_dev, int rows, int C, const float* gamma_dev, const float* beta_dev,
                     void* out_f16_dev, float* out_f32_dev, void* stream);
diff --git a/profiles/ln_fold_bench.py b/profiles/ln_fold_bench.py
--- /dev/null
+++ b/profiles/ln_fold_bench.py
@@ -0,0 +1,129 @@
+import argparse
+import hashlib
+import json
+import os
+import statistics
+import subprocess
+import sys
+
+ap = argparse.ArgumentParser()
+ap.add_argument("mode", choices=["pairs", "encode"])
+ap.add_argument("--reps", type=int, default=60)
+ap.add_argument("--batch", type=int, default=256)
+ap.add_argument("--root", default=os.path.dirname(os.path.dirname(os.path.abspath(__file__))))
+a = ap.parse_args()
+sys.path.insert(0, os.path.abspath(a.root))
+
+import torch
+
+
+def gpu_line():
+    q = subprocess.run(["nvidia-smi", "--query-gpu=name,power.limit,clocks.sm,clocks.max.sm", "--format=csv,noheader"],
+                       capture_output=True, text=True).stdout.strip().splitlines()
+    return {"gpu": q[0] if q else "unknown", "root": os.path.abspath(a.root)}
+
+
+def timed(fn):
+    s, e = torch.cuda.Event(enable_timing=True), torch.cuda.Event(enable_timing=True)
+    s.record()
+    fn()
+    e.record()
+    e.synchronize()
+    return s.elapsed_time(e) * 1e3
+
+
+def alternate(variants, reps):
+    for f in variants.values():
+        f()
+    torch.cuda.synchronize()
+    t = {k: [] for k in variants}
+    for _ in range(reps):
+        for k, f in variants.items():
+            t[k].append(timed(f))
+    return {k: {"median_us": round(statistics.median(v), 2), "min_us": round(min(v), 2), "max_us": round(max(v), 2)}
+            for k, v in t.items()}
+
+
+def rand(*shape, scale=1.0, seed=0):
+    g = torch.Generator(device="cuda").manual_seed(seed)
+    return torch.randn(*shape, device="cuda", generator=g) * scale
+
+
+def main_pairs():
+    import ctypes as C
+    from handwritten_math_ocr_api_b200 import _lib as L
+    lib = L.load()
+
+    def P(t):
+        return None if t is None else C.c_void_p(t.data_ptr())
+
+    st = C.c_void_p(torch.cuda.current_stream().cuda_stream)
+    B = a.batch
+    for C_, M in ((96, B * 1920), (192, B * 480)):
+        x0 = rand(M, C_, seed=1) * 3 + 0.5
+        g, b = 1 + 0.2 * rand(C_, seed=2), 0.1 * rand(C_, seed=3)
+        w1 = rand(4 * C_, C_, scale=C_ ** -0.5, seed=4).half()
+        w2 = rand(C_, 4 * C_, scale=(4 * C_) ** -0.5, seed=5).half()
+        b1, b2 = 0.3 * rand(4 * C_, seed=6), 0.3 * rand(C_, seed=7)
+        xn = torch.empty(M, C_, dtype=torch.float16, device="cuda")
+        x_pair, x_fused = x0.clone(), x0.clone()
+
+        def pair():
+            L.check(lib.hmocr_layernorm(P(x_pair), M, C_, P(g), P(b), P(xn), None, st), "layernorm")
+            L.check(lib.hmocr_swin_mlp(P(xn), M, C_, P(w1), P(b1), P(w2), P(b2), P(x_pair), st), "swin_mlp")
+
+        def fused():
+            L.check(lib.hmocr_swin_mlp_ln(P(g), P(b), M, C_, P(w1), P(b1), P(w2), P(b2), P(x_fused), st), "swin_mlp_ln")
+
+        res = alternate({"layernorm+swin_mlp": pair, "swin_mlp_ln": fused}, a.reps)
+        same = bool(torch.equal(x_pair, x_fused))
+        print(json.dumps({"shape": f"norm2+mlp C={C_} M={M}", **res, "same_bits": same,
+                          "saved_us": round(res["layernorm+swin_mlp"]["median_us"] - res["swin_mlp_ln"]["median_us"], 2)}),
+              flush=True)
+
+    for C_, M in ((96, B * 1920), (192, B * 480)):
+        N = 3 * C_
+        x = rand(M, C_, seed=8) * 3 + 0.5
+        g, b = 1 + 0.2 * rand(C_, seed=9), 0.1 * rand(C_, seed=10)
+        w = rand(N, C_, scale=C_ ** -0.5, seed=11).half()
+        bias = 0.3 * rand(N, seed=12)
+        xn = torch.empty(M, C_, dtype=torch.float16, device="cuda")
+        o_pair = torch.empty(M, N, dtype=torch.float16, device="cuda")
+        o_fused = torch.empty_like(o_pair)
+
+        def pair():
+            L.check(lib.hmocr_layernorm(P(x), M, C_, P(g), P(b), P(xn), None, st), "layernorm")
+            L.check(lib.hmocr_gemm_f16(P(xn), C_, M, C_, P(w), N, P(bias), 0, None, 0, None, 0, P(o_pair), N, None, None, 0,
+                                       st), "gemm")
+
+        def fused():
+            L.check(lib.hmocr_gemm_ln_f16(P(x), P(g), P(b), M, C_, P(w), N, P(bias), 0, P(o_fused), N, st), "gemm_ln")
+
+        res = alternate({"layernorm+gemm": pair, "gemm_ln": fused}, a.reps)
+        print(json.dumps({"shape": f"norm1+qkv C={C_} M={M} N={N}", **res, "same_bits": bool(torch.equal(o_pair, o_fused)),
+                          "saved_us": round(res["layernorm+gemm"]["median_us"] - res["gemm_ln"]["median_us"], 2)}),
+              flush=True)
+
+
+def main_encode():
+    from handwritten_math_ocr_api_b200 import FormulaRecognitionModel
+    from oracle.arch import ModelConfig
+    from oracle.synth import synth_images, synth_state_dict
+    cfg = ModelConfig()
+    m = FormulaRecognitionModel(cfg.vocab_size, device="cuda:0")
+    m.load_state_dict(synth_state_dict(cfg, seed=0, eos_bias_sigma=0.0))
+    imgs = synth_images(a.batch, seed=1234).cuda()
+    out = m.encoder(imgs)
+    torch.cuda.synchronize()
+    digest = hashlib.sha256(out.cpu().numpy().tobytes()).hexdigest()
+    t = []
+    for _ in range(3):
+        m.encoder(imgs)
+    for _ in range(a.reps):
+        t.append(timed(lambda: m.encoder(imgs)))
+    print(json.dumps({"encode_B": a.batch, "median_us": round(statistics.median(t), 1), "min_us": round(min(t), 1),
+                      "max_us": round(max(t), 1), "sha256": digest}), flush=True)
+
+
+print(json.dumps(gpu_line()), flush=True)
+main_pairs() if a.mode == "pairs" else main_encode()
```

Result: no change. 13830 (median of 6 runs) (-0.3%).
